# VCISwang/STCD

Measured on AMD Instinct MI355X. Metric: image-pairs/sec (256x256 bf16 SiamUnet_diff train), higher is better.
Workload: dtype bf16; 1 GPU; SiamUnet_diff(3,2) 256x256 full training step (fwd + cross_entropy + bwd + AdamW), 16 pairs/GPU, synthetic LEVIR-CD-shaped pairs resident in HBM; global_batch=16, image=256, parallelism=dp1

## Files before the change

include/stcd_hip.h:

```cpp
#ifndef STCD_HIP_H
#define STCD_HIP_H

#include <stdint.h>

#ifdef __cplusplus
extern "C" {
#endif

#define STCD_ABI_VERSION 2

#define STCD_ARCH_DIFF 0
#define STCD_ARCH_CONC 1
#define STCD_ARCH_SUB 2
#define STCD_ARCH_SNUNET 3
#define STCD_ARCH_SEGCD 4
#define STCD_ARCH_SEGCD_R18 5
#define STCD_ARCH_SEGCD_R34 6
#define STCD_ARCH_SEGCD_R101 7
#define STCD_ARCH_SEGCD_R152 8
#define STCD_ARCH_FCEF 9
#define STCD_ARCH_XCONC 10
#define STCD_ARCH_SNUNET_CONC 11
#define STCD_ARCH_SNUNET_CONC_DS 12
#define STCD_ARCH_UNETSEG 16
// ... 168 lines not shown
int stcd_mask_close(const uint8_t* in, int height, int width, int radius, int mask_value, uint8_t* out, void* hip_stream);

typedef struct stcd_conv_geom {
    int32_t n, hi, wi, ci, ldi;
    int32_t hm, wm, in_stride;
    int32_t ho, wo, out_stride, oy0, ox0;
    int32_t co, ldo;
    int32_t ntaps;
    int8_t dy[9], dx[9];
    int8_t pad_[2];
} stcd_conv_geom;

int stcd_op_conv(int dtype, int impl, const stcd_conv_geom* g, const void* in, const float* w, const float* bias,
                 void* out, void* scratch, int64_t scratch_bytes, void* hip_stream);
enum { STCD_CONV_SMALL = 0, STCD_CONV_RES = 1, STCD_CONV_TILE = 2, STCD_CONV_GEMM = 3, STCD_CONV_HALO = 4, STCD_CONV_DMA = 5 };
typedef struct stcd_conv_fused {
    int32_t kernel;
    int32_t groups;
    void* sum_acc;
    int32_t sum_c0, sum_c;
    float sum_scale1, sum_scale2;
    int32_t use_epi, relu;
    const void* gate;
    const void* res;
    int32_t ldg, ldr;
    float alpha, beta;
    const void* bw_y;
    const float* bw_stat;
    const float* bw_mask;
    void* bw_acc;
    int32_t bw_ldy;
    int32_t blocks, tiles_per_group, blocks_per_group, bn_rep;
    int32_t tile_m;
} stcd_conv_fused;
int stcd_op_conv_fused(const stcd_conv_geom* g, stcd_conv_fused* f, const void* in, const float* w, const float* bias, void* out,
                       void* scratch, int64_t scratch_bytes, void* hip_stream);
int stcd_op_wgrad(int dtype, int impl, const stcd_conv_geom* g, const void* in, const void* dout, float* dw,
                  void* scratch, int64_t scratch_bytes, void* hip_stream);
int64_t stcd_op_scratch_bytes(const stcd_conv_geom* g);

typedef struct stcd_map_geom {
    int32_t n, h, w, c, groups;
} stcd_map_geom;
int64_t stcd_op_ew_scratch_bytes(const stcd_map_geom* g);
int stcd_op_bn_act(int dtype, const stcd_map_geom* g, const void* y, int ldy, const float* gamma, const float* beta,
                   float* running_mean, float* running_var, const float* mask, int relu, int training, void* a, int lda,
                   void* pool, int ldp, float* stat, void* scratch, int64_t scratch_bytes, void* hip_stream);
int stcd_op_bn_act_pair(int dtype, const stcd_map_geom* g, const void* y, int ldy, const float* gamma, const float* beta,
                        float* running_mean, float* running_var, const float* mask, int fuse_mode, void* a, int lda, void* pool,
                        int ldp, void* fused, int ldf, float* stat, void* scratch, int64_t scratch_bytes, void* hip_stream);
int stcd_op_bn_act_bwd(int dtype, const stcd_map_geom* g, const void* da, int ldda, const void* y, int ldy, const float* stat,
                       const float* mask, int relu, void* dy, int lddy, float* dgamma, float* dbeta, void* scratch,
                       int64_t scratch_bytes, void* hip_stream);
int stcd_op_maxpool(int dtype, const stcd_map_geom* g, const void* a, int lda, void* pool, int ldp, void* hip_stream);
int stcd_op_maxpool_bwd(int dtype, const stcd_map_geom* g, const void* a, int lda, const void* dpool, int ldp, void* da, int ldda,
                        int accumulate, void* hip_stream);
int stcd_op_maxpool3(int dtype, const stcd_map_geom* g, const void* a, int lda, void* pool, int ldp, void* idx, void* hip_stream);
int stcd_op_maxpool3_bwd(int dtype, const stcd_map_geom* g, const void* idx, const void* dpool, int ldp, void* da, int ldda, void* hip_stream);
int64_t stcd_op_pairdw_scratch_bytes(const stcd_map_geom* g);
int stcd_op_pairdw(int dtype, const stcd_map_geom* g, const void* a, int lda, const float* w, const float* b, void* out, int ldo,
                   void* hip_stream);
int stcd_op_pairdw_bwd(int dtype, const stcd_map_geom* g, const void* a, int lda, const void* dout, int lddo, const float* w, void* da,
                       int ldda, float* dw, void* scratch, int64_t scratch_bytes, void* hip_stream);
int stcd_op_fuse(int dtype, int mode, const stcd_map_geom* g, const void* a, int lda, void* d, int ldd, void* hip_stream);
int stcd_op_fuse_bwd(int dtype, int mode, const stcd_map_geom* g, const void* a, int lda, const void* dd, int ldd, void* da, int ldda,
                     void* hip_stream);
int stcd_op_rep_pad(int dtype, const stcd_map_geom* g, void* d, int ld, int h0, int w0, void* hip_stream);
int stcd_op_rep_pad_bwd(int dtype, const stcd_map_geom* g, void* dd, int ld, int h0, int w0, void* hip_stream);
int stcd_op_skip_bwd(int dtype, int mode, const stcd_map_geom* g, const void* a, int lda, const void* y, int ldy, const void* dd,
                     int ldd, const void* dpool, int ldp, const float* stat, const float* mask, void* da, int ldda, void* dy,
                     int lddy, float* dgamma, float* dbeta, void* scratch, int64_t scratch_bytes, void* hip_stream);

int64_t stcd_op_cf_scratch_bytes(int64_t rows, int channels, int n, int q_tokens, int kv_tokens);
int stcd_op_cf_im2col(int dtype, const void* x, void* col, int ldc, int n, int h, int w, int c, int k, int stride, int pad, void* hip_stream);
int stcd_op_cf_col2im(int dtype, const void* dcol, int ldc, void* dx, int n, int h, int w, int c, int k, int stride, int pad, int accumulate,
                      void* hip_stream);
int stcd_op_cf_layernorm(int dtype, const void* x, void* y, const float* gamma, const float* beta, float* stats, int64_t rows, int c, float eps,
                         void* hip_stream);
int stcd_op_cf_layernorm_bwd(int dtype, const void* dy, const void* dy2, const void* x, const float* stats, const float* gamma, const void* add,
                             void* dx, float* dgamma, float* dbeta, void* scratch, int64_t rows, int c, void* hip_stream);
int stcd_op_cf_colsum(int dtype, const void* x, int64_t rows, int c, float* out, void* scratch, void* hip_stream);
int stcd_op_cf_attention(int dtype, const void* q, const void* kv, void* out, float* lse, int n, int q_tokens, int kv_tokens, int heads, int d,
                         float p, uint64_t seed, void* hip_stream);
int64_t stcd_op_cf_attention_scratch_bytes(int n, int q_tokens, int kv_tokens, int heads, int d);
int stcd_op_cf_attention_bwd(int dtype, const void* q, const void* kv, const void* out, const void* dout, const float* lse, void* dq, void* dkv,
                             void* scratch, int n, int q_tokens, int kv_tokens, int heads, int d, float p, uint64_t seed, void* hip_stream);
int stcd_op_cf_dwgelu(int dtype, const void* h, void* u, void* a, const float* w, const float* b, int n, int height, int width, int ch, float p,
                      uint64_t seed, void* hip_stream);
int64_t stcd_op_cf_dwgelu_scratch_bytes(int n, int height, int width, int ch);
int stcd_op_cf_dwgelu_bwd(int dtype, const void* h, const void* u, void* da, void* dh, const float* w, float* dw, float* db, void* scratch, int n,
                          int height, int width, int ch, float p, uint64_t seed, void* hip_stream);
int stcd_op_cf_resid_drop(int dtype, const void* x, const void* y, void* out, int n, int64_t rows_per_img, int c, float p, float path_p,
                          uint64_t seed, int backward, void* hip_stream);
int stcd_op_cf_bilinear(int dtype, const void* src, void* dst, int n, int h, int w, int out_h, int out_w, int c, int accumulate, int backward,
                        void* hip_stream);
int stcd_op_cf_elementwise(int dtype, int op, const void* x, const void* y, void* out, int64_t rows, int c, const float* alpha, float alpha_f,
                           float beta_f, float p, uint64_t seed, void* hip_stream);
int stcd_op_cf_prelu_bwd(int dtype, const void* dz, const void* y, void* dy, const float* alpha, float* dalpha, void* scratch, int64_t rows, int c,
                         void* hip_stream);

#ifdef __cplusplus
}
#endif
#endif
```

stcd_amd/_lib.py:

```python
from __future__ import annotations

import ctypes as C
import os

import torch

_HERE = os.path.dirname(os.path.abspath(__file__))
LIB_PATH = os.environ.get("STCD_LIB_PATH") or os.path.join(_HERE, "libstcd_hip.so")

ARCH_DIFF, ARCH_CONC, ARCH_SUB, ARCH_SNUNET, ARCH_SEGCD = 0, 1, 2, 3, 4
ARCH_SEGCD_R18, ARCH_SEGCD_R34, ARCH_SEGCD_R101, ARCH_SEGCD_R152 = 5, 6, 7, 8
ARCH_FCEF = 9
ARCH_XCONC = 10
ARCH_SNUNET_CONC = 11
ARCH_SNUNET_CONC_DS = 12
ARCH_UNETSEG = 16
ARCH_FFCTLCD = 32
ARCH_BASE_RESNET = 48
ARCH_BIT = 52
ARCH_CHANGEFORMER = 64
DTYPE_F32, DTYPE_BF16 = 0, 1
ARCH_IDS = {"diff": ARCH_DIFF, "conc": ARCH_CONC, "sub": ARCH_SUB, "fcef": ARCH_FCEF, "xconc": ARCH_XCONC, "snunet": ARCH_SNUNET, "snunet_conc": ARCH_SNUNET_CONC, "snunet_conc_ds": ARCH_SNUNET_CONC_DS, "segcd": ARCH_SEGCD,
            "segcd_resnet50": ARCH_SEGCD, "segcd_resnet18": ARCH_SEGCD_R18, "segcd_resnet34": ARCH_SEGCD_R34,
            "segcd_resnet101": ARCH_SEGCD_R101, "segcd_resnet152": ARCH_SEGCD_R152,
# ... 85 lines not shown
    "stcd_num_bn": (_i, [_vp]),
    "stcd_bn_info_get": (_i, [_vp, _i, C.POINTER(BnInfo)]),
    "stcd_bn_floats": (_i64, [_vp]),
    "stcd_configure": (_i, [_vp, _i, _i, _i]),
    "stcd_workspace_bytes": (_i64, [_vp]),
    "stcd_num_dropout": (_i, [_vp]),
    "stcd_dropout_info_get": (_i, [_vp, _i, C.POINTER(DropoutInfo)]),
    "stcd_dropout_floats": (_i64, [_vp]),
    "stcd_set_dropout_p": (_i, [_vp, _f]),
    "stcd_forward": (_i, [_vp, _vp, _vp, _vp, _vp, _vp, C.c_uint64, _i, _vp, _vp, _vp]),
    "stcd_backward": (_i, [_vp, _vp, _vp, _vp, _vp, _i, _vp]),
    "stcd_grad_stage_range": (_i, [_vp, _i, C.POINTER(_i64), C.POINTER(_i64)]),
    "stcd_set_weights_tag": (_i, [_vp, C.c_uint64]),
    "stcd_set_debug": (_i, [_vp, _i]),
    "stcd_ws_tensor_count": (_i, [_vp]),
    "stcd_ws_tensor_get": (_i, [_vp, _i, C.POINTER(WsTensor)]),
    "stcd_profile_enable": (_i, [_vp, _i]),
    "stcd_profile_read": (_i, [_vp, _i, C.POINTER(C.c_double), C.POINTER(_i64), C.POINTER(C.c_double), C.POINTER(C.c_double)]),
    "stcd_profile_num_kernels": (_i, [_vp]),
    "stcd_profile_kernel": (_i, [_vp, _i, C.c_char_p, _i, C.POINTER(C.c_double), C.POINTER(_i64), C.POINTER(C.c_double), C.POINTER(C.c_double)]),
    "stcd_loss_scratch_bytes": (_i64, []),
    "stcd_loss_ce": (_i, [_vp, _vp, _i, _i, _i64, _i, _vp, _vp, _vp, _vp]),
    "stcd_loss_bce_dice": (_i, [_vp, _vp, _i64, _i, _vp, _vp, _vp, _vp]),
    "stcd_loss_contrastive": (_i, [_vp, _vp, _vp, _i64, _vp, _vp, _vp, _vp]),
    "stcd_loss_focal": (_i, [_vp, _vp, _i, _i, _i64, _vp, _f, _f, _i, _vp, _vp, _vp, _vp]),
    "stcd_loss_iou_scratch_bytes": (_i64, [_i, _i, _i64]),
    "stcd_loss_iou": (_i, [_vp, _vp, _i, _i, _i64, _vp, _i, _vp, _vp, _vp, _vp]),
    "stcd_confusion_update": (_i, [_vp, _vp, _i, _i, _i64, _vp, _vp]),
    "stcd_adam_step": (_i, [_vp, _vp, _vp, _vp, _i64, _i64, _d, _d, _d, _d, _d, _i, _vp]),
    "stcd_adam_hyper": (_i, [_i64, _d, _d, _d, _d, _d, C.POINTER(_f)]),
    "stcd_adam_step_dev": (_i, [_vp, _vp, _vp, _vp, _i64, _vp, _i, _vp]),
    "stcd_pseudo_pair": (_i, [_vp, _vp, _vp, _vp, _vp, _vp, C.c_uint64, _i, _i, _i, C.POINTER(_f), C.POINTER(_f), _vp, _vp, _vp, _vp, _vp, _vp]),
    "stcd_augment_scratch_bytes": (_i64, [_i, _i, _i]),
    "stcd_augment": (_i, [_vp, _vp, _i, _i, _i, C.POINTER(_f), C.POINTER(_f), _vp, _vp, _i64, _vp]),
    "stcd_scene_gather": (_i, [_vp, _vp, _i, _i, _i, _i, _i, _i, _i, C.POINTER(_f), C.POINTER(_f), _vp, _vp, _vp]),
    "stcd_scene_stitch": (_i, [_vp, _i, _i, _i, _i, _i, _i, _i, _i, _i, _vp, _vp, _vp, _vp]),
    "stcd_scene_finalize": (_i, [_vp, _vp, _i, _i, _i, _f, _vp, _vp, _vp, _vp, _vp]),
    "stcd_scene_gather_d4": (_i, [_vp, _vp, _i, _i, _i, _i, _i, _i, _i, C.POINTER(_f), C.POINTER(_f), _vp, _vp, _i, _vp]),
    "stcd_scene_stitch_d4": (_i, [_vp, _i, _i, _i, _i, _i, _i, _i, _i, _i, _vp, _vp, _vp, _i, _vp]),
    "stcd_scene_gather_one_d4": (_i, [_vp, _i, _i, _i, _i, _i, _i, _i, C.POINTER(_f), C.POINTER(_f), _vp, _i, _vp]),
    "stcd_scene_stitch_heads_d4": (_i, [C.POINTER(_vp), _i, _i, _i, _i, _i, _i, _i, _i, _i, _i, _vp, _vp, _vp, _i, _vp]),
    "stcd_scene_finalize_seg": (_i, [_vp, _vp, _i, _i, _i, _f, _f, _vp, _vp, _vp, _vp, _vp, _vp, _vp, _vp, _vp, _vp]),
    "stcd_selftrain_score": (_i, [C.POINTER(_vp), _i, _i, _i, _i64, _f, _vp, _i, _vp, _vp, _vp, _vp]),
    "stcd_scene_cell_agree": (_i, [C.POINTER(_vp), _i, _i, _i, _i, _i, _i, _vp, _vp, _vp, _vp]),
    "stcd_mask_close": (_i, [_vp, _i, _i, _i, _i, _vp, _vp]),
    "stcd_op_conv": (_i, [_i, _i, C.POINTER(ConvGeom), _vp, _vp, _vp, _vp, _vp, _i64, _vp]),
    "stcd_op_conv_fused": (_i, [C.POINTER(ConvGeom), C.POINTER(ConvFused), _vp, _vp, _vp, _vp, _vp, _i64, _vp]),
    "stcd_op_wgrad": (_i, [_i, _i, C.POINTER(ConvGeom), _vp, _vp, _vp, _vp, _i64, _vp]),
    "stcd_op_scratch_bytes": (_i64, [C.POINTER(ConvGeom)]),
    "stcd_op_ew_scratch_bytes": (_i64, [C.POINTER(MapGeom)]),
    "stcd_op_bn_act": (_i, [_i, C.POINTER(MapGeom), _vp, _i, _vp, _vp, _vp, _vp, _vp, _i, _i, _vp, _i, _vp, _i, _vp, _vp, _i64, _vp]),
    "stcd_op_bn_act_pair": (_i, [_i, C.POINTER(MapGeom), _vp, _i, _vp, _vp, _vp, _vp, _vp, _i, _vp, _i, _vp, _i, _vp, _i, _vp, _vp, _i64, _vp]),
    "stcd_op_bn_act_bwd": (_i, [_i, C.POINTER(MapGeom), _vp, _i, _vp, _i, _vp, _vp, _i, _vp, _i, _vp, _vp, _vp, _i64, _vp]),
    "stcd_op_maxpool": (_i, [_i, C.POINTER(MapGeom), _vp, _i, _vp, _i, _vp]),
    "stcd_op_maxpool_bwd": (_i, [_i, C.POINTER(MapGeom), _vp, _i, _vp, _i, _vp, _i, _i, _vp]),
    "stcd_op_maxpool3": (_i, [_i, C.POINTER(MapGeom), _vp, _i, _vp, _i, _vp, _vp]),
    "stcd_op_maxpool3_bwd": (_i, [_i, C.POINTER(MapGeom), _vp, _vp, _i, _vp, _i, _vp]),
    "stcd_op_pairdw_scratch_bytes": (_i64, [C.POINTER(MapGeom)]),
    "stcd_op_pairdw": (_i, [_i, C.POINTER(MapGeom), _vp, _i, _vp, _vp, _vp, _i, _vp]),
    "stcd_op_pairdw_bwd": (_i, [_i, C.POINTER(MapGeom), _vp, _i, _vp, _i, _vp, _vp, _i, _vp, _vp, _i64, _vp]),
    "stcd_op_fuse": (_i, [_i, _i, C.POINTER(MapGeom), _vp, _i, _vp, _i, _vp]),
    "stcd_op_fuse_bwd": (_i, [_i, _i, C.POINTER(MapGeom), _vp, _i, _vp, _i, _vp, _i, _vp]),
    "stcd_op_rep_pad": (_i, [_i, C.POINTER(MapGeom), _vp, _i, _i, _i, _vp]),
    "stcd_op_rep_pad_bwd": (_i, [_i, C.POINTER(MapGeom), _vp, _i, _i, _i, _vp]),
    "stcd_op_skip_bwd": (_i, [_i, _i, C.POINTER(MapGeom), _vp, _i, _vp, _i, _vp, _i, _vp, _i, _vp, _vp, _vp, _i, _vp, _i, _vp, _vp, _vp, _i64, _vp]),
    "stcd_op_cf_scratch_bytes": (_i64, [_i64, _i, _i, _i, _i]),
    "stcd_op_cf_im2col": (_i, [_i, _vp, _vp, _i, _i, _i, _i, _i, _i, _i, _i, _vp]),
    "stcd_op_cf_col2im": (_i, [_i, _vp, _i, _vp, _i, _i, _i, _i, _i, _i, _i, _i, _vp]),
    "stcd_op_cf_layernorm": (_i, [_i, _vp, _vp, _vp, _vp, _vp, _i64, _i, _f, _vp]),
    "stcd_op_cf_layernorm_bwd": (_i, [_i, _vp, _vp, _vp, _vp, _vp, _vp, _vp, _vp, _vp, _vp, _i64, _i, _vp]),
    "stcd_op_cf_colsum": (_i, [_i, _vp, _i64, _i, _vp, _vp, _vp]),
    "stcd_op_cf_attention": (_i, [_i, _vp, _vp, _vp, _vp, _i, _i, _i, _i, _i, _f, C.c_uint64, _vp]),
    "stcd_op_cf_attention_scratch_bytes": (_i64, [_i, _i, _i, _i, _i]),
    "stcd_op_cf_attention_bwd": (_i, [_i, _vp, _vp, _vp, _vp, _vp, _vp, _vp, _vp, _i, _i, _i, _i, _i, _f, C.c_uint64, _vp]),
    "stcd_op_cf_dwgelu": (_i, [_i, _vp, _vp, _vp, _vp, _vp, _i, _i, _i, _i, _f, C.c_uint64, _vp]),
    "stcd_op_cf_dwgelu_scratch_bytes": (_i64, [_i, _i, _i, _i]),
    "stcd_op_cf_dwgelu_bwd": (_i, [_i, _vp, _vp, _vp, _vp, _vp, _vp, _vp, _vp, _i, _i, _i, _i, _f, C.c_uint64, _vp]),
    "stcd_op_cf_resid_drop": (_i, [_i, _vp, _vp, _vp, _i, _i64, _i, _f, _f, C.c_uint64, _i, _vp]),
    "stcd_op_cf_bilinear": (_i, [_i, _vp, _vp, _i, _i, _i, _i, _i, _i, _i, _i, _vp]),
    "stcd_op_cf_elementwise": (_i, [_i, _i, _vp, _vp, _vp, _i64, _i, _vp, _f, _f, _f, C.c_uint64, _vp]),
    "stcd_op_cf_prelu_bwd": (_i, [_i, _vp, _vp, _vp, _vp, _vp, _vp, _i64, _i, _vp]),
}
EXPORTS = tuple(_PROTOS)

_lib = None


class StcdError(RuntimeError):
    pass


def lib():
    global _lib
    if _lib is None:
        if not os.path.exists(LIB_PATH):
            raise StcdError(
                f"{LIB_PATH} is missing: build it with `python -c 'import __graft_entry__ as g; g.build()'` "
                "or `make -C stcd_amd/csrc`.  The engine has no CPU fallback.")
        l = C.CDLL(LIB_PATH)
        for name, (res, args) in _PROTOS.items():
            fn = getattr(l, name)
            fn.restype, fn.argtypes = res, args
        if l.stcd_abi_version() != 2:
            raise StcdError("libstcd_hip.so ABI version mismatch")
        _lib = l
    return _lib
# ... 6 lines not shown
```

stcd_amd/csrc/common.h:

```cpp
#pragma once
#include <hip/hip_runtime.h>
#include <stdint.h>
#include <stdio.h>
#include <stdlib.h>
#include <string>
#include <string.h>

#include "../../include/stcd_hip.h"

namespace stcd {

typedef __bf16 bf16;

enum DType { F32 = STCD_DTYPE_F32, BF16 = STCD_DTYPE_BF16 };
inline size_t dsize(int dt) { return dt == BF16 ? 2 : 4; }

void set_error(const std::string& msg);

static inline int env_int(const char* name, int dflt) { const char* v = getenv(name); return v ? atoi(v) : dflt; }
static inline bool env_flag(const char* name, bool dflt) { const char* v = getenv(name); return v && v[0] == (dflt ? '0' : '1') ? !dflt : dflt; }

#define STCD_CHECK(cond, msg)                                              \
    do {                                                                   \
        if (!(cond)) {                                                     \
// ... 80 lines not shown
    double y = (double)__frsqrt_rn((float)x);
    y = y * (1.5 - 0.5 * x * y * y);
    return y * (1.5 - 0.5 * x * y * y);
}

__device__ __forceinline__ void bn_fwd_table(float* tab, const long long* __restrict__ facc, const float* __restrict__ gamma,
                                             const float* __restrict__ beta, float* __restrict__ rmean, float* __restrict__ rvar,
                                             float* __restrict__ stat, int C, int groups, int64_t ppg, float momentum, float eps,
                                             bool publish, int cbase = 0, int CS = 0, int g_first = 0) {
    if (CS == 0) CS = C;
    const double inv_n = 1.0 / (double)ppg;
    for (int cl = threadIdx.x; cl < CS; cl += blockDim.x) {
        const int c = cbase + cl;
        if (facc) {
            const float gam = gamma[c], bet = beta[c];
            float rm = (publish && rmean) ? rmean[c] : 0.f, rv = (publish && rvar) ? rvar[c] : 0.f;
            for (int gi = 0; gi < groups; ++gi) {
                int g = gi + g_first;
                if (g >= groups) g -= groups;
                const double s1 = bn_acc_get(facc, groups, C, g, 0, c, BN_FS1), s2 = bn_acc_get(facc, groups, C, g, 1, c, BN_FS2);
                const double mean = s1 * inv_n;
                double var = s2 * inv_n - mean * mean;
                if (var < 0.0) var = 0.0;
                const double invstd = bn_rsqrt(var + (double)eps);
                const float sc = (float)(gam * invstd), sh = (float)(bet - mean * gam * invstd);
                tab[(g * 2 + 0) * CS + cl] = sc;
                tab[(g * 2 + 1) * CS + cl] = sh;
                if (publish) {
                    float* st = stat + (int64_t)g * 4 * C;
                    st[c] = (float)mean; st[C + c] = (float)invstd; st[2 * C + c] = sc; st[3 * C + c] = sh;
                    const double unb = ppg > 1 ? var * ((double)ppg / (double)(ppg - 1)) : var;
                    rm = (float)((1.0 - momentum) * rm + momentum * mean);
                    rv = (float)((1.0 - momentum) * rv + momentum * unb);
                }
            }
            if (publish && rmean) rmean[c] = rm;
            if (publish && rvar) rvar[c] = rv;
        } else if (gamma) {
            const float invstd = 1.f / sqrtf(rvar[c] + eps);
            const float sc = gamma[c] * invstd, sh = beta[c] - rmean[c] * gamma[c] * invstd;
            for (int g = 0; g < groups; ++g) {
                tab[(g * 2 + 0) * CS + cl] = sc;
                tab[(g * 2 + 1) * CS + cl] = sh;
            }
        } else {
            for (int g = 0; g < groups; ++g) {
                tab[(g * 2 + 0) * CS + cl] = stat[(int64_t)g * 4 * C + 2 * C + c];
                tab[(g * 2 + 1) * CS + cl] = stat[(int64_t)g * 4 * C + 3 * C + c];
            }
        }
    }
}

struct XfSrc {
    const long long* facc = nullptr;
    const float* gamma = nullptr;
    const float* beta = nullptr;
    float* rmean = nullptr; float* rvar = nullptr;
    float* stat = nullptr;
    const float* mask = nullptr;
    int C = 0, groups = 1, npg = 0, publish = 0;
    long long ppg = 0;
    float momentum = 0.1f, eps = 1e-5f;
    int on = 0;
};
__device__ __forceinline__ uint4 xf_act8(const uint4 raw, const float (&sc)[8], const float (&sh)[8], const unsigned okm) {
    typedef short s16x2 __attribute__((ext_vector_type(2)));
    const uint32_t w[4] = {raw.x, raw.y, raw.z, raw.w};
    uint32_t o[4];
#pragma unroll
    for (int i = 0; i < 4; ++i) {
        const float lo = fmaf(__uint_as_float(w[i] << 16), sc[2 * i], sh[2 * i]);
        const float hi = fmaf(__uint_as_float(w[i] & 0xffff0000u), sc[2 * i + 1], sh[2 * i + 1]);
        const s16x2 p = __builtin_bit_cast(s16x2, pack_bf16x2(lo, hi));
        o[i] = __builtin_bit_cast(uint32_t, __builtin_elementwise_max(p, s16x2{0, 0})) & okm;
    }
    return make_uint4(o[0], o[1], o[2], o[3]);
}
__device__ __forceinline__ void xf_fold8(const float* __restrict__ tab_sc, const float* __restrict__ tab_sh, const float4 m0, const float4 m1,
                                         float (&sc)[8], float (&sh)[8]) {
    const float mk[8] = {m0.x, m0.y, m0.z, m0.w, m1.x, m1.y, m1.z, m1.w};
#pragma unroll
    for (int j = 0; j < 8; ++j) { sc[j] = tab_sc[j] * mk[j]; sh[j] = tab_sh[j] * mk[j]; }
}


void launch_in_pack(int dt, const float* x1, const float* x2, void* X, int B, int cin, int H, int W, hipStream_t s, int dates = 2);
void launch_gout_pack(int dt, const float* g, void* G, int B, int L, int H, int W, hipStream_t s, long long* bias_acc = nullptr);
struct BiasJob { int64_t acc_off; int64_t out_off; int C, valid; float scale; int pad_; };
void launch_bias_finish(const BiasJob* jobs_dev, int njobs, const char* ws, float* grads, hipStream_t s);

void launch_conv_ref(int dt, const stcd_conv_geom& g, const void* in, const float* w, int kpad, int wld,
                     const float* bias, void* out, bool out_nchw_f32, hipStream_t s);
void launch_wgrad_ref(int dt, const stcd_conv_geom& g, const void* in, const void* dout, float* dw, int kpad, int wld,
                      hipStream_t s);
void launch_wgrad_ref_f64(int dt, const stcd_conv_geom& g, const void* in, const void* dout, double* dw, int kpad, int wld,
                          hipStream_t s);

struct ConvMfmaPlan {
    int CiB = 0, nchunks = 0, KS = 0, modeB = 0, NT = 0, NTtot = 0;
    int64_t wf_elems = 0;
    bool ok = false;
};
ConvMfmaPlan conv_mfma_plan(const stcd_conv_geom& g);
void launch_pack_frag(const stcd_conv_geom& g, const ConvMfmaPlan& p, const float* w, int kpad, int wld, void* dst,
                      hipStream_t s);
// ... 49 lines not shown
struct ConvHaloPlan {
    int NH = 0;
    int nslices = 0, P = 0, blocks = 0, lds_bytes = 0;
    bool ok = false;
};
ConvHaloPlan conv_halo_plan(const stcd_conv_geom& g, const ConvMfmaPlan& p);
int launch_conv_halo(const stcd_conv_geom& g, const ConvMfmaPlan& p, const ConvHaloPlan& hp, const void* in, const void* wf,
                     const float* bias, void* out, hipStream_t s, const ConvEpi* epi = nullptr);

struct ConvDmaPlan {
    int tiles_m = 0, tiles_n = 0, blocks = 0, lds_bytes = 0;
    bool ok = false;
};
ConvDmaPlan conv_dma_plan(const stcd_conv_geom& g, const ConvMfmaPlan& p);
int launch_conv_dma(const stcd_conv_geom& g, const ConvMfmaPlan& p, const ConvDmaPlan& dp, const void* in, const void* wf,
                    const float* bias, void* out, hipStream_t s, const ConvEpi* epi = nullptr);

bool conv_small_ok(const stcd_conv_geom& g, const ConvMfmaPlan& p);
int conv_small_blocks(const stcd_conv_geom& g, int groups);
int launch_conv_small(const stcd_conv_geom& g, const void* in, const void* wf_modeB, const float* bias, void* out,
                      bool out_nchw_f32, int groups, long long* stat_acc, int cpad, hipStream_t s, const XfSrc* xf = nullptr,
                      const BwdSum* bs = nullptr);
bool conv_small_call_ok(const stcd_conv_geom& g, int groups, const XfSrc* xf);
bool conv_small_bwdsum_ok(const stcd_conv_geom& g);
struct WgradMfmaPlan {
    int WCI = 1, NTW = 1, gx = 1, gy = 1, gz = 1;
    int64_t slab_floats = 0;
    int wi_valid = 0;
    int gemm = 0;
    int dma = 0;
    bool ok = false;
};
WgradMfmaPlan wgrad_mfma_plan(const stcd_conv_geom& g, int kpad, int wld, bool allow_wide = false, int force_co64 = -1);
int launch_wgrad_mfma(const stcd_conv_geom& g, const WgradMfmaPlan& p, const void* in, const void* dout, float* slab,
                      int kpad, int wld, hipStream_t s);
struct WgradJob {
    stcd_conv_geom g;
    int64_t in_off, dout_off, slab_off;
    int kpad, wld;
    int dymin, dxmin, HH, HWp;
    int tiles_x, tiles_y, ntiles;
    int xrow_bytes;
    int x_bytes, y_bytes;
    int co_valid;
    unsigned in_bytes, dout_bytes;
    int gx, gy, gz;
    int start;
    int lds_bytes;
    int wi_valid;
    int dma_L, dma_nk;
    int pad_;
    int64_t xf_stat_off, xf_mask_off;
    int xf_C, xf_groups, xf_npg, pad2_;
};
WgradMfmaPlan wgrad_gemm_plan(const stcd_conv_geom& g, int kpad, int wld);
WgradJob wgrad_gemm_make_job(const stcd_conv_geom& g, const WgradMfmaPlan& p, int64_t in_off, int64_t dout_off, int64_t slab_off,
                             int kpad, int wld);
int launch_wgrad_gemm_group(int W, const WgradJob* jobs_dev, int njobs, int total_blocks, const char* base, hipStream_t s);
WgradMfmaPlan wgrad_dma_plan(const stcd_conv_geom& g, int kpad, int wld);
void wgrad_dma_set_split(WgradMfmaPlan& p, const stcd_conv_geom& g, int S, int kpad, int wld);
WgradJob wgrad_dma_make_job(const stcd_conv_geom& g, const WgradMfmaPlan& p, int64_t in_off, int64_t dout_off, int64_t slab_off,
                            int kpad, int wld);
int launch_wgrad_dma_group(const WgradJob* jobs_dev, int njobs, int total_blocks, const char* base, hipStream_t s);
WgradJob wgrad_make_job(const stcd_conv_geom& g, const WgradMfmaPlan& p, int64_t in_off, int64_t dout_off, int64_t slab_off,
                        int kpad, int wld);
void wgrad_job_set_xf(WgradJob& a, int64_t stat_off, int64_t mask_off, int C, int groups, int npg);
int wgrad_variant_slots(int WCI, int NTW, bool t9, int lds_bytes);
int launch_wgrad_group(int WCI, int NTW, bool t9, const WgradJob* jobs_dev, int njobs, int total_blocks, int lds_bytes,
                       const char* base, hipStream_t s, bool xf = false);
struct PackSpec;
struct ReduceJob {
    int64_t start, count;
    int64_t slab_off;
    int64_t out_off;
    int64_t slab_stride;
    int gx, ntaps, K, N, kpad, wld;
    int ks, kn_major;
    int8_t ky[9], kx[9];
    int8_t tiled, parts, pad_[4];
};
void launch_reduce_jobs(const ReduceJob* jobs_dev, int njobs, int64_t total, const char* ws, float* grads, hipStream_t s);
void launch_reduce_dw(const float* slab, int gx, const stcd_conv_geom& g, int K, int N, int kpad, int wld,
                      const PackSpec* ps, float* out, hipStream_t s);

struct PackSpec {
    int ks;
    int kn_major;
    int K, N, wld;
    int kpad;
    int ntaps;
    int8_t ky[9], kx[9];
};
void launch_pack_w(const PackSpec& ps, const float* src, float* dst, hipStream_t s);
void launch_unpack_dw(const PackSpec& ps, const double* dwe, float* gsrc, hipStream_t s);

struct PackJob {
    int64_t start, count;
    int64_t src_off;
    int64_t dst_off;
    int kind;
    PackSpec ps;
    int Ci, Co, CiB, nchunks, KS, NTtot, modeB;
    int aux;
};
void launch_pack_jobs(const PackJob* jobs_dev, int njobs, int64_t total, const float* params, char* ws, hipStream_t s);

int bn_stats_chunks(int64_t pixels_per_group, int C);
void launch_bn_stats(int dt, const void* Y, int ld, int C, int groups, int64_t pixels_per_group, long long* acc, hipStream_t s);
void launch_bn_eval_prepare(int C, int groups, const float* gamma, const float* beta, const float* running_mean,
                            const float* running_var, float* stat, float eps, hipStream_t s);
constexpr int MAX_VIEWS = 6;
struct SliceViews {
    int n = 0;
    void* p[MAX_VIEWS]; int ld[MAX_VIEWS]; int64_t goff[MAX_VIEWS]; int gmask[MAX_VIEWS];
};
struct BnActArgs {
    const void* Y; int ldy;
    void* A; int lda; int64_t a_group_off;
    void* P; int ldp;
    float* stat;
    const float* mask;
    int C, groups, npg, H, W;
// ... 234 lines not shown
```

stcd_amd/csrc/engine.hip:

```cpp
#include <algorithm>
#include <climits>
#include <cstdint>
#include <array>
#include <cstring>
#include <memory>
#include <vector>

#include "common.h"

namespace stcd {

static thread_local std::string g_err;
void set_error(const std::string& msg) { g_err = msg; }

enum ConvKind { K_CONV3 = 0, K_CONVT3_S1 = 1, K_UPCONV = 2, K_CONV1 = 3, K_CONVT2 = 4, K_CONV3_S2 = 5, K_CONV1_S2 = 6, K_STEM7 = 7 };

struct TRef { int64_t off = -1; int ld = 0; };
struct GRef { int64_t off = -1; int ld = 0; int64_t goff = 0; };

static inline int round8(int c) { return (c + 7) & ~7; }

struct ConvW {
    std::string name;
    int kind = 0, cin = 0, cout = 0;
    int kin_p = 0, nout_p = 0;
    int64_t w_off = 0, b_off = 0;
    PackSpec fwd{}, dgrad{};
    int64_t wpk_fwd = -1, wpk_dgrad = -1, dwe = -1;
    int64_t dwe_floats = 0;
};
struct BnP {
    std::string name;
    int C = 0, calls = 1;
    int64_t g_off = 0, b_off = 0;
    int64_t run_off = 0;
};
struct DropP { std::string name; int rows = 0, C = 0; int64_t off = 0; };

struct ConvOp {
    stcd_conv_geom g{};
    int conv = -1; bool dgrad = false;
    int tap0 = 0;
    int kreal = 0, nreal = 0;
    ConvMfmaPlan plan; int64_t wf = -1;
    bool small = false;
    ConvResPlan res; int res_groups = 1;
    ConvGemmPlan gemm;
    ConvDmaPlan dma;
    ConvHaloPlan halo;
    ConvTilePlan tile;
};
struct WgradOp {
    stcd_conv_geom g{};
    int conv = -1, tap0 = 0, kreal = 0, nreal = 0;
    WgradMfmaPlan plan;
    int64_t slab = -1;
    int stage = 0;
    int64_t in_off = -1, dout_off = -1;
    bool grouped = false;
    int group = -1;
    int64_t xf_stat_off = -1, xf_mask_off = -1; int xf_C = 0, xf_groups = 1, xf_npg = 1;
    bool own_taps = false;
    int8_t oky[9] = {0}, okx[9] = {0};
};
struct WgradGroup {
    int WCI = 1, NTW = 1; bool t9 = false;
    bool xf = false;
    int gemm = 0;
    int dma = 0;
    std::vector<WgradJob> jobs;
    int total_blocks = 0, lds_bytes = 0;
    int64_t table_off = -1;
    double flops = 0.0, bytes = 0.0;
    int seen = 0; bool launched = false;
};

struct Cbrd {
    ConvOp fwd, dgr; WgradOp wg;
    int conv = -1, bn = -1, drop = -1;
    int N = 0, H = 0, W = 0, groups = 1, npg = 0;
    TRef in; int K = 0;
    TRef Y; GRef A; TRef P; TRef dPool; bool pool = false;
    GRef dA; TRef dY; TRef dIn; bool has_dIn = false;
    int64_t stat = -1;
    int64_t facc = -1, bacc = -1;
    const Cbrd* dgr_bwd = nullptr;
    bool bwd_sums_fused = false;
    int64_t dgr_sum_acc = -1; int dgr_sum_c0 = 0, dgr_sum_C = 0;
    TRef fuse_dst;
    bool virt = false; const Cbrd* xsrc = nullptr;
};
struct XConc {
    int level = 0, C = 0;
    int64_t w_off = 0, b_off = 0;
    int bn1 = -1;
    TRef G, dG, R, dR;
    int64_t stat1 = -1, facc1 = -1, bacc1 = -1, part = -1;
    Cbrd res;
};
struct UpConv {
    int conv = -1, level = 0;
    int N = 0, h = 0, w = 0, Ho = 0, Wo = 0, C = 0;
    TRef in, out, dOut, dIn;
    ConvOp fwd[4], dgr; WgradOp wg[4];
    int64_t bias_acc = -1; bool bias_fused = false;
};

enum ProfClass { PC_CONV = 0, PC_WGRAD = 1, PC_BN_STATS = 2, PC_BN_ACT = 3, PC_BN_BWD_REDUCE = 4, PC_BN_BWD_APPLY = 5,
                 PC_POOL_FUSE = 6, PC_PACK = 7, PC_COUNT = 8 };
struct ProfRec { hipEvent_t a, b; int klass; int name_id; double flops, bytes; };
struct Prof {
    bool on = false;
    std::vector<ProfRec> recs;
    std::vector<hipEvent_t> pool;
    std::vector<std::string> names;
    size_t used = 0;
    int intern(const std::string& n) {
        for (size_t i = 0; i < names.size(); ++i)
            if (names[i] == n) return (int)i;
        names.push_back(n);
        return (int)names.size() - 1;
    }
    hipEvent_t get() {
        if (used == pool.size()) { hipEvent_t ev; (void)hipEventCreate(&ev); pool.push_back(ev); }
        return pool[used++];
    }
    ~Prof() { for (auto ev : pool) (void)hipEventDestroy(ev); }
};

struct ViewRef { int64_t off = 0; int ld = 0; int64_t goff = 0; int gmask = 1; };
struct GLayer {
    std::string name;
    int conv = -1, bn = -1, kind = K_CONV3;
    int N = 0, Hi = 0, Wi = 0, Ho = 0, Wo = 0, K = 0, C = 0, groups = 2, npg = 0;
    bool relu = true;
    TRef in, Y, A, res;
    TRef dA, dIn, dRes;
    bool has_dIn = true;
    std::vector<ViewRef> extra_dst;
    std::vector<ViewRef> grad_src;
    bool grad_base = true;
    ConvOp fwd, dgr[4]; int ndgr = 0; WgradOp wg[8]; int nwg = 0;
    int64_t stat = -1, coef = -1, facc = -1, bacc = -1;
// ... 42 lines not shown
    int64_t sn_pool = -1, sn_argm = -1, sn_att = -1, sn_hid = -1, sn_sums = -1, sn_dpool = -1, sn_part = -1;
    int64_t sn_dout_begin = -1, sn_dout_end = -1;
    ConvOp sn_final_fwd, sn_final_dgr; WgradOp sn_final_wg;
    int64_t snc_w[5] = {0, 0, 0, 0, 0}, snc_b[5] = {0, 0, 0, 0, 0}, snc_scratch = -1;
    std::vector<GLayer> g_layers;
    std::vector<GStep> g_fwd;
    int g_stem = -1, g_head_conv = -1;
    int debug_flags = 0;
    std::vector<stcd_ws_tensor> ws_tensors;
    std::vector<std::array<int, 4>> g_blocks;
    int seg_x = 4, seg_layers[4] = {3, 4, 6, 3};
    int seg_dates = 2;
    bool seg_ffc = false;
    TRef g_pool_idc;
    std::vector<std::array<int, 2>> g_dec;
    TRef gP0, gdP0, gX3, gdX3, gFuseTmp;
    int64_t g_pool_idx = -1;
    int64_t g_stem_part = -1;
    int64_t g_raw3 = -1, g_draw3 = -1;
    ConvOp g_head_fwd, g_head_dgr; WgradOp g_head_wg;
    bool bres = false; int seg_nstage = 4;
    int g_head_c = 16;
    int g_cls = -1, g_pred_conv = -1;
    ConvOp g_pred_fwd, g_pred_dgr; WgradOp g_pred_wg;
    int64_t g_pred_bias_acc = -1;
    struct BitPlan {
        bool on = false; int L = 1, dh = 64;
        int64_t pos_off = 0, wa_off = 0, enc_off = 0, dec_off = 0;
        int64_t tok_in = -1, tok_out = -1, dtok_out = -1, dtok_in = -1, stat = -1, AP = -1, dAP = -1, xs = -1, dG = -1, dec_part = -1,
                dmh = -1, dm = -1, enc_part = -1, tok_part = -1;
        TRef dec_din;
    } bit;
    int arch = 0, in_ch = 3, label = 2, dt = F32;
    int64_t min_bn_count = 0;
    float drop_p = 0.2f;
    std::vector<stcd_tensor_info> params;
    int64_t param_floats = 0, enc_param_end = 0;
    std::vector<ConvW> convs;
    std::vector<BnP> bns;
    int64_t bn_floats = 0;
    bool configured = false, fwd_training = false;
    int B = 0, H = 0, W = 0;
    std::vector<DropP> drops;
    int64_t drop_floats = 0;
    int64_t ws_bytes = 0;
    std::vector<Cbrd> enc, dec;
    std::vector<UpConv> ups;
    int final_conv = -1;
    ConvOp final_fwd, final_dgr; WgradOp final_wg;
    const Cbrd* final_dgr_bwd = nullptr;
    const Cbrd* final_xsrc = nullptr;
    int use_virt = 0;
    int fc_virt_layers = 0;
    std::vector<ConvOp*> conv_ops;
    int64_t slab = -1, slab_floats = 0;
    std::vector<WgradOp*> wgrad_ops;
    std::vector<WgradGroup> wgroups[2];
    std::vector<ReduceJob> rjobs[2];
    int64_t rjobs_total[2] = {0, 0}, rjobs_off[2] = {-1, -1};
    std::vector<PackJob> jobs[2];
    int64_t jobs_total[2] = {0, 0}, jobs_off[2] = {-1, -1};
    const void* jobs_uploaded_ws = nullptr;
    uint64_t weights_tag = 0, packed_tag = 0;
    const void* packed_ws = nullptr; const void* packed_params = nullptr; int packed_level = -1;
    TRef X0, G, finalIn, dFinalIn;
    int Hs[5] = {0}, Ws[5] = {0};
    TRef D[4], dD[4], P[4], dP[4];
    int64_t zero_begin = -1, zero_end = -1;
    int64_t final_bias_acc = -1;
    std::vector<BiasJob> bias_jobs; int64_t bias_jobs_off = -1;
    int64_t masks = -1, dwe_begin = -1, dwe_end = -1, scratch8 = -1;
    int use_mfma = 1, use_small = 1, use_wgroup = 1, use_res = 1, use_skip_fused = 1, use_act_fuse = 1, use_gemm = 1, use_skip_recompute = 1, use_bwdsum = 1, use_bwdsum_res = 0, use_tile = 1, use_halo = 0;
    int wg_side_on = 1;
    static constexpr int WG_SIDE_DIV = 4;
    static constexpr int WGROUP_ROUNDS = 1, WGROUP_MIN_TILES = 8;
    bool wg_early = false; hipStream_t wg_cur_side = nullptr;
    hipStream_t wg_side = nullptr; hipEvent_t wg_fork = nullptr, wg_join = nullptr; int wg_side_dev = -1;
};

}

using namespace stcd;
struct stcd_engine : stcd_engine_impl {};

namespace stcd {

static const int ENC_STAGE_CONVS[4] = {2, 2, 3, 3};
static const int ENC_C[4] = {16, 32, 64, 128};
static const int SKIP_IDX[4] = {1, 3, 6, 9};

static void add_param(stcd_engine& e, const std::string& name, std::initializer_list<int64_t> shape, int64_t* off_out) {
    stcd_tensor_info ti;
    memset(&ti, 0, sizeof(ti));
    snprintf(ti.name, sizeof(ti.name), "%s", name.c_str());
    ti.ndim = (int)shape.size();
    int64_t n = 1;
    int i = 0;
    for (auto s : shape) { ti.shape[i++] = s; n *= s; }
    ti.numel = n;
    ti.offset = e.param_floats;
    *off_out = ti.offset;
    e.param_floats += (n + 3) & ~(int64_t)3;
    e.params.push_back(ti);
}

static void make_specs(ConvW& c, bool need_dgrad) {
// ... 248 lines not shown
    op.small = conv_small_ok(op.g, op.plan);
    if (e.use_res && !op.small) op.res = conv_res_plan(op.g, op.plan, groups);
    pick_gemm_or_res(e, op, op.g, groups);
    if (with_tile) pick_tile(e, op, op.g, groups);
}
static bool conv_on_ref(bool mfma, const ConvOp& op) { return !(mfma && op.plan.ok && op.wf >= 0); }
struct Binder {
    stcd_engine& e; Bump& ws;
    bool with_tile = false;
    void conv(ConvOp& op, const stcd_conv_geom& g, int conv, bool dgrad, int tap0, int kreal, int nreal, int groups = 1) const {
        op = ConvOp();
        op.g = g; op.conv = conv; op.dgrad = dgrad; op.tap0 = tap0; op.kreal = kreal; op.nreal = nreal; op.res_groups = groups;
        if (e.dt == BF16) plan_conv(e, op, groups, with_tile);
        if (op.plan.ok) op.wf = ws.take(op.plan.wf_elems * 2);
        e.conv_ops.push_back(&op);
    }
    void stem(ConvOp& op, const stcd_conv_geom& g, int conv, int groups) const {
        op = ConvOp();
        op.g = g; op.conv = conv; op.kreal = e.convs[conv].cin; op.nreal = g.co; op.res_groups = groups;
        op.plan = conv_mfma_plan(g);
        if (g.ldi == 8 && g.co % 64 == 0) op.gemm = conv_gemm_plan(g, op.plan, groups);
        op.gemm.pix_chunks = 1;
        if (!op.gemm.ok) return;
        op.wf = ws.take(op.plan.wf_elems * 2);
        e.conv_ops.push_back(&op);
    }
    void wgrad(WgradOp& op, const stcd_conv_geom& g, int conv, int64_t in_off, int64_t dout_off, int stage = 0, int tap0 = 0,
               int wi_valid = 0, const int8_t* own_ky = nullptr, const int8_t* own_kx = nullptr) const {
        const ConvW& cv = e.convs[conv];
        op = WgradOp();
        op.g = g; op.conv = conv; op.tap0 = tap0; op.kreal = cv.cin; op.nreal = cv.cout;
        op.in_off = in_off; op.dout_off = dout_off; op.stage = stage;
        op.own_taps = own_ky != nullptr;
        for (int t = 0; t < g.ntaps && op.own_taps; ++t) { op.oky[t] = own_ky[t]; op.okx[t] = own_kx[t]; }
        if (e.dt == BF16) { op.plan = pick_wgrad_plan(e, g, cv.fwd.kpad, cv.fwd.wld); op.plan.wi_valid = wi_valid; }
        e.wgrad_ops.push_back(&op);
    }
};
static void take_ref_images(stcd_engine& e, Bump& ws, bool with_dwe = true) {
    for (auto& c : e.convs) {
        c.wpk_fwd = ws.take((int64_t)c.fwd.ntaps * c.fwd.kpad * c.fwd.wld * 4);
        if (c.dgrad.ntaps) c.wpk_dgrad = ws.take((int64_t)c.dgrad.ntaps * c.dgrad.kpad * c.dgrad.wld * 4);
    }
    e.dwe_begin = ws.cur;
    for (auto& c : e.convs) {
        c.dwe_floats = (int64_t)c.fwd.ntaps * c.fwd.kpad * c.fwd.wld;
        c.dwe = with_dwe ? ws.take(c.dwe_floats * 8) : -1;
    }
    e.dwe_end = ws.cur;
}

static bool same_group(const WgradGroup& G, const WgradOp& op) {
    const bool t9 = !op.plan.dma && op.g.ntaps == 9;
    return G.gemm == op.plan.gemm && G.dma == op.plan.dma && G.WCI == op.plan.WCI && G.NTW == op.plan.NTW && G.t9 == t9 && G.xf == (op.xf_C > 0);
}

static bool cf_side_on() { static const bool on = env_flag("STCD_CF_SIDE", true); return on; }

static void build_pack_jobs(stcd_engine& e, Bump& ws) {
    for (int st = 0; st < 2; ++st) { e.rjobs[st].clear(); e.rjobs_total[st] = 0; }
    for (int st = 0; st < 2; ++st) e.wgroups[st].clear();
    if (e.dt == BF16 && e.use_mfma) {
        if (e.use_wgroup) {
            for (WgradOp* op : e.wgrad_ops) {
                if (!op->plan.ok) continue;
                const bool t9 = !op->plan.dma && op->g.ntaps == 9;
                std::vector<WgradGroup>& gs = e.wgroups[op->stage];
                size_t gi = 0;
                while (gi < gs.size() && !same_group(gs[gi], *op)) ++gi;
                if (gi == gs.size()) { WgradGroup g; g.WCI = op->plan.WCI; g.NTW = op->plan.NTW; g.t9 = t9; g.gemm = op->plan.gemm; g.dma = op->plan.dma; g.xf = op->xf_C > 0; gs.push_back(g); }
                op->grouped = true;
            }
            for (int st = 0; st < 2; ++st)
                for (WgradGroup& G : e.wgroups[st]) {
                    if (G.gemm) { G.lds_bytes = 2 * 2 * G.gemm * (64 * 64 + 8 * 32); continue; }
                    if (G.dma) {
                        G.lds_bytes = 128 * 1024;
                        std::vector<WgradOp*> dops;
                        for (WgradOp* op : e.wgrad_ops)
                            if (op->grouped && op->stage == st && op->plan.dma) dops.push_back(op);
                        auto blocks_at = [&](int64_t kt) {
                            int64_t b = 0;
                            for (WgradOp* op : dops) {
                                const int64_t M = (int64_t)op->g.n * op->g.hi * op->g.wi;
                                b += ((M + kt * 64 - 1) / (kt * 64)) * op->plan.gy * op->plan.gz;
                            }
                            return b;
                        };
                        int64_t lo = 1, hi = 1;
                        const int dma_blocks = e.wg_side_on && cf_side_on() ? 192 : 256;
                        while (blocks_at(hi) > dma_blocks) hi *= 2;
                        while (lo < hi) { const int64_t mid = (lo + hi) / 2; if (blocks_at(mid) <= dma_blocks) hi = mid; else lo = mid + 1; }
                        for (WgradOp* op : dops) {
                            const ConvW& cv = e.convs[op->conv];
                            const int64_t M = (int64_t)op->g.n * op->g.hi * op->g.wi;
                            int64_t S = (M + lo * 64 - 1) / (lo * 64);
                            const int64_t slab_bytes = (int64_t)op->g.ntaps * cv.fwd.kpad * cv.fwd.wld * 4;
                            S = std::min<int64_t>(S, std::max<int64_t>(1, ((int64_t)64 << 20) / slab_bytes));
                            wgrad_dma_set_split(op->plan, op->g, (int)S, cv.fwd.kpad, cv.fwd.wld);
                        }
                        continue;
                    }
                    std::vector<WgradOp*> ops;
                    int64_t W = 0;
                    for (WgradOp* op : e.wgrad_ops)
                        if (op->grouped && op->stage == st && same_group(G, *op)) {
                            ops.push_back(op);
                            const int64_t ntiles = (int64_t)op->g.n * ((op->g.wm + 15) / 16) * ((op->g.hm + 7) / 8);
                            W += ntiles * op->plan.gy * op->plan.gz;
                        }
                    for (WgradOp* op : ops) {
                        const ConvW& cv = e.convs[op->conv];
                        WgradJob j = wgrad_make_job(op->g, op->plan, 0, 0, 0, cv.fwd.kpad, cv.fwd.wld);
                        if (op->xf_C > 0) wgrad_job_set_xf(j, op->xf_stat_off, op->xf_mask_off, op->xf_C, op->xf_groups, op->xf_npg);
                        G.lds_bytes = std::max(G.lds_bytes, j.lds_bytes);
                    }
                    int slots = wgrad_variant_slots(G.WCI, G.NTW, G.t9, G.lds_bytes);
                    if (st == 0 && e.wg_side_on && fc_family(e)) slots = std::max(64, slots / stcd_engine_impl::WG_SIDE_DIV);
                    const int64_t rounds = stcd_engine_impl::WGROUP_ROUNDS;
                    const int64_t tpb = std::max<int64_t>(stcd_engine_impl::WGROUP_MIN_TILES, (W + rounds * slots - 1) / (rounds * slots));
                    for (WgradOp* op : ops) {
                        const ConvW& cv = e.convs[op->conv];
                        const int64_t ntiles = (int64_t)op->g.n * ((op->g.wm + 15) / 16) * ((op->g.hm + 7) / 8);
                        const int64_t slab_bytes = (int64_t)op->g.ntaps * cv.fwd.kpad * cv.fwd.wld * 4;
                        int64_t gx = std::max<int64_t>(1, (ntiles + tpb - 1) / tpb);
                        gx = std::min<int64_t>(gx, std::max<int64_t>(1, ((int64_t)32 << 20) / slab_bytes));
                        op->plan.gx = (int)gx;
                        op->plan.slab_floats = gx * op->g.ntaps * cv.fwd.kpad * cv.fwd.wld;
                    }
                }
        }
        int64_t cur[2] = {0, 0};
        for (WgradOp* op : e.wgrad_ops) {
            if (!op->plan.ok) continue;
            const ConvW& cv = e.convs[op->conv];
            op->slab = ws.take(op->plan.slab_floats * 4);
            if (op->grouped) {
                for (WgradGroup& G : e.wgroups[op->stage])
                    if (same_group(G, *op)) {
                        op->group = (int)(&G - e.wgroups[op->stage].data());
                        WgradJob j = op->plan.dma ? wgrad_dma_make_job(op->g, op->plan, op->in_off, op->dout_off, op->slab, cv.fwd.kpad, cv.fwd.wld)
                                   : op->plan.gemm ? wgrad_gemm_make_job(op->g, op->plan, op->in_off, op->dout_off, op->slab, cv.fwd.kpad, cv.fwd.wld)
                                                   : wgrad_make_job(op->g, op->plan, op->in_off, op->dout_off, op->slab, cv.fwd.kpad, cv.fwd.wld);
                        if (op->xf_C > 0 && !op->plan.dma && !op->plan.gemm) wgrad_job_set_xf(j, op->xf_stat_off, op->xf_mask_off, op->xf_C, op->xf_groups, op->xf_npg);
                        j.start = G.total_blocks;
                        G.total_blocks += j.gx * j.gy * j.gz;
                        G.jobs.push_back(j);
                        double fl, by;
                        conv_work(e, op->g, op->kreal, op->nreal, &fl, &by);
                        G.flops += fl; G.bytes += by;
                    }
            }
            ReduceJob j{};
            j.slab_off = op->slab; j.out_off = cv.w_off;
            j.slab_stride = (int64_t)op->g.ntaps * cv.fwd.kpad * cv.fwd.wld;
            j.gx = op->plan.gx; j.ntaps = op->g.ntaps; j.K = cv.cin; j.N = cv.cout; j.kpad = cv.fwd.kpad; j.wld = cv.fwd.wld;
            j.ks = cv.fwd.ks; j.kn_major = cv.fwd.kn_major;
            for (int t = 0; t < op->g.ntaps; ++t) {
                j.ky[t] = op->own_taps ? op->oky[t] : cv.fwd.ky[op->tap0 + t];
                j.kx[t] = op->own_taps ? op->okx[t] : cv.fwd.kx[op->tap0 + t];
            }
            j.tiled = (int64_t)j.ntaps * j.K * j.N >= 512 * 1024;
            if (!j.tiled) {
                const int64_t outs = (int64_t)j.ntaps * j.K * j.N;
                int parts = 1;
                while (parts < 64 && parts * 32 < j.gx) parts *= 2;
                j.parts = (int8_t)parts;
                const int64_t OUTS = 256 / parts;
                j.count = ((outs + OUTS - 1) / OUTS) * 256;
            } else {
                const int TK = j.ntaps == 1 ? 32 : 16;
                const int64_t ntiles = (int64_t)((j.N + 31) / 32) * ((j.K + TK - 1) / TK);
                j.parts = 1;
                j.count = ntiles * 256;
            }
            j.start = cur[op->stage];
            cur[op->stage] += (j.count + 255) & ~(int64_t)255;
            e.rjobs[op->stage].push_back(j);
        }
        for (int st = 0; st < 2; ++st) {
            e.rjobs_total[st] = cur[st];
            e.rjobs_off[st] = ws.take((int64_t)e.rjobs[st].size() * sizeof(ReduceJob) + 16);
            for (WgradGroup& G : e.wgroups[st]) G.table_off = ws.take((int64_t)G.jobs.size() * sizeof(WgradJob) + 16);
        }
    }
    for (int with_dgrad = 0; with_dgrad < 2; ++with_dgrad) {
        std::vector<PackJob>& jobs = e.jobs[with_dgrad];
        jobs.clear();
        int64_t cur = 0;
        auto push = [&](PackJob j) { j.start = cur; cur += (j.count + 255) & ~(int64_t)255; jobs.push_back(j); };
        const bool mfma = e.dt == BF16 && e.use_mfma;
        if (!mfma) {
            for (auto& cv : e.convs)
                for (int d = 0; d <= with_dgrad; ++d) {
                    const PackSpec& ps = d ? cv.dgrad : cv.fwd;
                    if (!ps.ntaps) continue;
                    PackJob j{};
                    j.kind = 0; j.ps = ps; j.src_off = cv.w_off; j.dst_off = d ? cv.wpk_dgrad : cv.wpk_fwd;
                    j.count = (int64_t)ps.ntaps * ps.kpad * ps.wld;
                    push(j);
                }
        } else {
            for (const ConvOp* op : e.conv_ops) {
                if (op->dgrad && !with_dgrad) continue;
                const ConvW& cv = e.convs[op->conv];
                const PackSpec& full = op->dgrad ? cv.dgrad : cv.fwd;
                PackJob j{};
                j.ps = full;
                j.ps.ntaps = op->g.ntaps;
                for (int t = 0; t < op->g.ntaps; ++t) { j.ps.ky[t] = full.ky[op->tap0 + t]; j.ps.kx[t] = full.kx[op->tap0 + t]; }
                j.src_off = cv.w_off;
                if (cv.kind == K_STEM7) {
                    j.kind = 2; j.dst_off = op->wf; j.count = op->plan.wf_elems;
                    j.Co = cv.cout; j.NTtot = op->plan.NTtot; j.aux = cv.cin;
                    push(j);
                    continue;
                }
                if (!conv_on_ref(true, *op)) {
                    j.kind = 1; j.dst_off = op->wf;
                    j.count = op->plan.modeB ? op->plan.wf_elems : op->plan.wf_elems / op->g.ntaps;
                    j.Ci = op->g.ci; j.Co = op->g.co; j.CiB = op->plan.CiB; j.nchunks = op->plan.nchunks; j.KS = op->plan.KS;
                    j.NTtot = op->plan.NTtot; j.modeB = op->plan.modeB;
                } else {
                    j.kind = 0;
                    j.dst_off = (op->dgrad ? cv.wpk_dgrad : cv.wpk_fwd) + (int64_t)op->tap0 * full.kpad * full.wld * 4;
                    j.count = (int64_t)j.ps.ntaps * full.kpad * full.wld;
                }
                push(j);
            }
        }
        e.jobs_total[with_dgrad] = cur;
        e.jobs_off[with_dgrad] = ws.take((int64_t)jobs.size() * sizeof(PackJob) + 16);
    }
}

// ... 154 lines not shown
    for (auto& L : e.dec) bind_cbrd(L);
    for (auto& X : e.xc) bind_cbrd(X.res);
    for (auto& U : e.ups) {
        const ConvW& cv = e.convs[U.conv];
        for (int ph = 0; ph < 4; ++ph) {
            int tap0;
            stcd_conv_geom g = geom_up_phase(U, ph >> 1, ph & 1, U.in.ld, U.out.ld, &tap0);
            bind.conv(U.fwd[ph], g, U.conv, false, tap0, U.C, U.C);
            bind.wgrad(U.wg[ph], g, U.conv, U.in.off, U.dOut.off, wg_stage(U.conv), tap0);
        }
        stcd_conv_geom gd;
        memset(&gd, 0, sizeof(gd));
        gd.n = U.N; gd.hi = U.Ho; gd.wi = U.Wo; gd.ci = cv.dgrad.kpad; gd.ldi = U.dOut.ld;
        gd.hm = U.h; gd.wm = U.w; gd.in_stride = 2;
        gd.ho = U.h; gd.wo = U.w; gd.out_stride = 1;
        gd.co = U.C; gd.ldo = U.dIn.ld;
        gd.ntaps = 9;
        for (int t = 0; t < 9; ++t) { gd.dy[t] = (int8_t)(t / 3 - 1); gd.dx[t] = (int8_t)(t % 3 - 1); }
        bind.conv(U.dgr, gd, U.conv, true, 0, U.C, U.C);
    }
    {
        const ConvW& cv = e.convs[e.final_conv];
        bind.conv(e.final_fwd, geom3(B, H, W, cv.kin_p, e.finalIn.ld, e.label, e.label), e.final_conv, false, 0, cv.cin, e.label);
        bind.wgrad(e.final_wg, geom3(B, H, W, cv.kin_p, e.finalIn.ld, e.label, 8), e.final_conv, e.finalIn.off, e.G.off, wg_stage(e.final_conv));
        bind.conv(e.final_dgr, geom3(B, H, W, cv.dgrad.kpad, 8, cv.cin, e.dFinalIn.ld), e.final_conv, true, 0, e.label, cv.cin);
    }
    e.slab = ws.take(e.slab_floats * 4);

    for (auto& L : e.enc) { L.dgr_bwd = nullptr; L.bwd_sums_fused = false; }
    for (auto& L : e.dec) { L.dgr_bwd = nullptr; L.bwd_sums_fused = false; }
    e.final_dgr_bwd = nullptr;
    if (e.use_bwdsum && e.dt == BF16 && e.use_mfma && e.use_small && !e.use_virt) {
        const int res_too = e.use_bwdsum_res;
        auto dest_ok = [&](const Cbrd& P, const ConvOp& dgr, int64_t dIn_off, int dIn_ld, int N) {
            const bool kern = (dgr.small && conv_small_bwdsum_ok(dgr.g)) ||
                              (res_too && !dgr.small && !dgr.gemm.ok && e.use_res && dgr.res.ok && dgr.res_groups == P.groups &&
                               conv_res_bwdsum_ok(dgr.g, dgr.res));
            return !P.pool && P.fuse_dst.off < 0 && !P.virt && kern && dgr.wf >= 0 && dIn_off == P.dA.off && dIn_ld == P.dA.ld &&
                   e.convs[P.conv].cout == dgr.g.co && P.N == N && N % P.groups == 0 &&
                   (P.groups == 1 || P.dA.goff == (int64_t)P.npg * P.H * P.W * P.dA.ld);
        };
        auto scan = [&](std::vector<Cbrd>& v) {
            for (size_t i = 1; i < v.size(); ++i) {
                Cbrd& N = v[i]; Cbrd& P = v[i - 1];
                if (N.has_dIn && N.dgr_sum_acc < 0 && dest_ok(P, N.dgr, N.dIn.off, N.dIn.ld, N.N)) { N.dgr_bwd = &P; P.bwd_sums_fused = true; }
            }
        };
        scan(e.enc); scan(e.dec);
        if (!e.dec.empty() && dest_ok(e.dec.back(), e.final_dgr, e.dFinalIn.off, e.dFinalIn.ld, e.dec.back().N)) {
            e.final_dgr_bwd = &e.dec.back(); e.dec.back().bwd_sums_fused = true;
        }
    }

    e.final_xsrc = nullptr; e.fc_virt_layers = 0;
    for (auto& L : e.enc) { L.virt = false; L.xsrc = nullptr; }
    for (auto& L : e.dec) { L.virt = false; L.xsrc = nullptr; }
    if (e.use_virt && e.dt == BF16 && e.use_mfma && e.use_wgroup && !fc_cross(e)) {
        auto fwd_ok = [&](const ConvOp& op, bool nchw) {
            if (op.wf < 0 || (op.gemm.ok && !nchw)) return false;
            if (op.small && e.use_small) return true;
            return op.res.ok && !nchw && !op.res.single_halo;
        };
        auto wg_ok = [&](const WgradOp& op) { return op.plan.ok && !op.plan.gemm && !op.plan.dma && op.plan.WCI < 4 && op.plan.NTW < 4; };
        auto link = [&](Cbrd& P, ConvOp& cf, WgradOp& cw, bool nchw) {
            if (P.pool || P.fuse_dst.off >= 0) return false;
            if (!fwd_ok(cf, nchw) || !wg_ok(cw)) return false;
            P.virt = true; ++e.fc_virt_layers;
            cw.in_off = P.Y.off;
            cw.xf_stat_off = P.stat;
            cw.xf_mask_off = (P.drop >= 0) ? e.masks + e.drops[P.drop].off * 4 : -1;
            cw.xf_C = e.convs[P.conv].cout; cw.xf_groups = P.groups; cw.xf_npg = P.npg;
            return true;
        };
        for (size_t i = 0; i + 1 < e.enc.size(); ++i) {
            Cbrd& P = e.enc[i]; Cbrd& Cn = e.enc[i + 1];
            if (Cn.in.off != P.A.off) continue;
            if (link(P, Cn.fwd, Cn.wg, false)) { Cn.xsrc = &P; Cn.in.off = P.Y.off; Cn.in.ld = P.Y.ld; }
        }
        for (size_t i = 0; i < e.dec.size(); ++i) {
            Cbrd& P = e.dec[i];
            if (i + 1 < e.dec.size() && e.dec[i + 1].in.off == P.A.off) {
                Cbrd& Cn = e.dec[i + 1];
                if (link(P, Cn.fwd, Cn.wg, false)) { Cn.xsrc = &P; Cn.in.off = P.Y.off; Cn.in.ld = P.Y.ld; }
            } else if (e.finalIn.off == P.A.off) {
                if (link(P, e.final_fwd, e.final_wg, true)) { e.final_xsrc = &P; e.finalIn.off = P.Y.off; e.finalIn.ld = P.Y.ld; }
            }
        }
    }

    e.bias_jobs.clear();
    {
        size_t di = 0;
        for (int k = 0; k < 4; ++k) {
            UpConv& U = e.ups[k];
            Cbrd& L = e.dec[di];
            int nb = 0;
            for (int j = 0; j < DEC[k].n; ++j) nb += DEC[k].cout[j] >= 0;
            di += nb;
            U.bias_fused = false;
            const bool even = 2 * U.h == U.Ho && 2 * U.w == U.Wo;
            if (e.dt == BF16 && e.use_mfma && nb > 0 && L.has_dIn && L.dIn.off == U.dOut.off && L.dgr.res.ok && L.dgr.wf >= 0 && even) {
                U.bias_fused = true;
                L.dgr_sum_acc = U.bias_acc; L.dgr_sum_c0 = 0; L.dgr_sum_C = U.C;
            }
            if (e.dt == BF16) {
                BiasJob jb{}; jb.acc_off = U.bias_acc; jb.out_off = e.convs[U.conv].b_off; jb.C = U.C; jb.valid = U.C; jb.scale = BN_BS;
                e.bias_jobs.push_back(jb);
            }
        }
        BiasJob jb{}; jb.acc_off = e.final_bias_acc; jb.out_off = e.convs[e.final_conv].b_off; jb.C = 8; jb.valid = e.label; jb.scale = BN_BS;
        e.bias_jobs.push_back(jb);
        e.bias_jobs_off = ws.take((int64_t)e.bias_jobs.size() * sizeof(BiasJob) + 16);
    }

    e.ws_tensors.clear();
    auto rec_layer = [&](const Cbrd& L) {
        const ConvW& cv = e.convs[L.conv];
        auto rec = [&](const char* sfx, int64_t off, int ld, int n, int ch) {
            if (off < 0) return;
            stcd_ws_tensor r;
            memset(&r, 0, sizeof(r));
            snprintf(r.name, sizeof(r.name), "%s.%s", cv.name.c_str(), sfx);
            r.offset_bytes = off; r.n = n; r.h = L.H; r.w = L.W; r.c = ch; r.ld = ld; r.dtype = e.dt;
            e.ws_tensors.push_back(r);
        };
        rec(L.xsrc ? "in.virt" : "in", L.in.off, L.in.ld, L.N, L.K);
        rec("Y", L.Y.off, L.Y.ld, L.N, cv.cout);
        for (int g = 0; g < L.groups && !L.virt && !skip_recomputed(e, L); ++g) {
            char sfx[8];
            snprintf(sfx, sizeof(sfx), "A.g%d", g);
            rec(sfx, L.A.off + g * L.A.goff * T, L.A.ld, L.npg, cv.cout);
        }
        rec("dY", L.dY.off, L.dY.ld, L.N, cv.cout);
    };
    for (const Cbrd& L : e.enc) rec_layer(L);
    for (const Cbrd& L : e.dec) rec_layer(L);
    for (const XConc& X : e.xc) {
        auto rec = [&](const char* sfx, const TRef& t) {
            stcd_ws_tensor r;
            memset(&r, 0, sizeof(r));
            snprintf(r.name, sizeof(r.name), "cross_conc%d.diff.0.%s", X.level + 1, sfx);
            r.offset_bytes = t.off; r.n = X.res.N; r.h = X.res.H; r.w = X.res.W; r.c = X.C; r.ld = t.ld; r.dtype = e.dt;
            e.ws_tensors.push_back(r);
        };
        rec("Y", X.G); rec("A.g0", X.R); rec("dY", X.dG);
        rec_layer(X.res);
    }

    build_pack_jobs(e, ws);
    e.jobs_uploaded_ws = nullptr;
    e.ws_bytes = ws.cur;
    return 0;
}

struct Ctx {
    stcd_engine& e;
    char* ws;
    const float* params;
    float* grads;
    hipStream_t s;
    template <typename P = void> P* at(int64_t off) const { return (P*)(ws + off); }
};

struct ProfScope {
    Prof& p; hipStream_t s; bool on; hipEvent_t b;
    ProfScope(const Ctx& c, int klass, double flops, double bytes, const char* kernel = nullptr);
    ~ProfScope() { if (on) (void)hipEventRecord(b, s); }
};

ProfScope::ProfScope(const Ctx& c, int klass, double flops, double bytes, const char* kernel)
    : p(c.e.prof), s(c.s), on(c.e.prof.on), b(nullptr) {
    if (!on) return;
    static const char* DEF[PC_COUNT] = {"k_conv", "k_wgrad", "k_bn_reduce<T, 0>", "k_bn_act", "k_bn_reduce<T, 1>", "k_bn_bwd_apply",
                                        "k_pool_bwd|k_fuse|k_slice", "k_pack_jobs|k_reduce_dw"};
    ProfRec r;
    r.a = p.get(); r.b = p.get(); r.klass = klass; r.flops = flops; r.bytes = bytes;
    r.name_id = p.intern(kernel ? kernel : DEF[klass]);
    b = r.b;
    p.recs.push_back(r);
    (void)hipEventRecord(r.a, s);
}

static void conv_work(const stcd_engine& e, const stcd_conv_geom& g, int kreal, int nreal, double* flops, double* bytes) {
    double pos = (double)g.n * g.hm * g.wm;
    *flops = 2.0 * pos * g.ntaps * kreal * nreal;
    double in_px = g.in_stride == 1 ? pos : (double)g.n * (2.0 * g.hm) * (2.0 * g.wm);
// ... 147 lines not shown
    char kname[64];
    snprintf(kname, sizeof(kname), "k_conv_mfma_x4<%d>", p[0].NT);
    ProfScope prof(c, PC_CONV, fl, by, kname);
    if (launch_conv_mfma_x4(g, p, in, wf, bias, out, c.s) != 0) set_error(std::string("internal: ") + kname + " rejected the launch it was chosen for");
    return true;
}

static void wgroup_member_ready(const Ctx& c, const WgradOp& op);
static void exec_wgrad(const Ctx& c, const WgradOp& op, const void* in, const void* dout) {
    const ConvW& cv = c.e.convs[op.conv];
    PackSpec sub = cv.fwd;
    sub.ntaps = op.g.ntaps;
    for (int t = 0; t < op.g.ntaps; ++t) {
        sub.ky[t] = op.own_taps ? op.oky[t] : cv.fwd.ky[op.tap0 + t];
        sub.kx[t] = op.own_taps ? op.okx[t] : cv.fwd.kx[op.tap0 + t];
    }
    double fl, by;
    conv_work(c.e, op.g, op.kreal, op.nreal, &fl, &by);
    if (mfma_on(c.e) && op.plan.ok && op.grouped) {
        if (c.e.wg_early) wgroup_member_ready(c, op);
        return;
    }
    if (mfma_on(c.e) && op.plan.ok) {
        int rc;
        {
            char kname[64];
            snprintf(kname, sizeof(kname), "k_wgrad_mfma<%d, %d>", op.plan.WCI, op.plan.NTW);
            ProfScope prof(c, PC_WGRAD, fl, by, kname);
            rc = launch_wgrad_mfma(op.g, op.plan, in, dout, c.at<float>(op.slab), sub.kpad, sub.wld, c.s);
        }
        if (rc == 0) return;
    }
    if (op.own_taps) { set_error("internal: no reference fallback for a launch with its own tap table"); return; }
    double* dwe = c.at<double>(cv.dwe) + (int64_t)op.tap0 * sub.kpad * sub.wld;
    if (mfma_on(c.e))
        (void)hipMemsetAsync(dwe, 0, (size_t)sub.ntaps * sub.kpad * sub.wld * 8, c.s);
    {
        ProfScope prof(c, PC_WGRAD, fl, by, "k_wgrad_ref");
        launch_wgrad_ref_f64(c.e.dt, op.g, in, dout, dwe, sub.kpad, sub.wld, c.s);
    }
    launch_unpack_dw(sub, dwe, c.grads + cv.w_off, c.s);
}

static int pack_all_weights(const Ctx& c, bool with_dgrad) {
    stcd_engine& e = c.e;
    if (e.jobs_uploaded_ws != (const void*)c.ws) {
        for (int k = 0; k < 2; ++k) {
            if (!e.jobs[k].empty())
                STCD_HIP(hipMemcpyAsync(c.at(e.jobs_off[k]), e.jobs[k].data(), e.jobs[k].size() * sizeof(PackJob),
                                        hipMemcpyHostToDevice, c.s));
            if (!e.rjobs[k].empty())
                STCD_HIP(hipMemcpyAsync(c.at(e.rjobs_off[k]), e.rjobs[k].data(), e.rjobs[k].size() * sizeof(ReduceJob),
                                        hipMemcpyHostToDevice, c.s));
            for (WgradGroup& G : e.wgroups[k])
                STCD_HIP(hipMemcpyAsync(c.at(G.table_off), G.jobs.data(), G.jobs.size() * sizeof(WgradJob), hipMemcpyHostToDevice, c.s));
        }
        if (!e.bias_jobs.empty())
            STCD_HIP(hipMemcpyAsync(c.at(e.bias_jobs_off), e.bias_jobs.data(), e.bias_jobs.size() * sizeof(BiasJob), hipMemcpyHostToDevice, c.s));
        e.jobs_uploaded_ws = c.ws;
    }
    const int k = with_dgrad ? 1 : 0;
    if (k == 0 && e.weights_tag != 0 && e.weights_tag == e.packed_tag && e.packed_ws == (const void*)c.ws && e.packed_params == (const void*)c.params)
        return 0;
    ProfScope prof(c, PC_PACK, 0.0, 0.0);
    launch_pack_jobs(c.at<PackJob>(e.jobs_off[k]), (int)e.jobs[k].size(), e.jobs_total[k], c.params, c.ws, c.s);
    e.packed_tag = k == 0 ? e.weights_tag : 0; e.packed_ws = c.ws; e.packed_params = c.params; e.packed_level = k;
    return 0;
}

static void launch_wgroup(const Ctx& c, WgradGroup& G) {
    {
        char kname[64];
        if (G.dma) snprintf(kname, sizeof(kname), "k_wgrad_dma");
        else if (G.gemm) snprintf(kname, sizeof(kname), "k_wgrad_gemm<%d>", G.gemm);
        else snprintf(kname, sizeof(kname), "k_wgrad_group<%d, %d, %s>", G.WCI, G.NTW, G.t9 ? "true" : "false");
        ProfScope prof(c, PC_WGRAD, G.flops, G.bytes, kname);
        G.launched = true;
        if (G.dma) {
            launch_wgrad_dma_group(c.at<WgradJob>(G.table_off), (int)G.jobs.size(), G.total_blocks, c.ws, c.s);
            return;
        }
        if (G.gemm) {
            launch_wgrad_gemm_group(G.gemm, c.at<WgradJob>(G.table_off), (int)G.jobs.size(), G.total_blocks, c.ws, c.s);
            return;
        }
        if (launch_wgrad_group(G.WCI, G.NTW, G.t9, c.at<WgradJob>(G.table_off), (int)G.jobs.size(), G.total_blocks, G.lds_bytes,
                               c.ws, c.s, G.xf) != 0)
            set_error("grouped weight-gradient launch exceeds the LDS budget");
    }
}

static void wgroup_member_ready(const Ctx& c, const WgradOp& op) {
    stcd_engine& e = c.e;
    if (op.group < 0 || op.group >= (int)e.wgroups[op.stage].size()) return;
    WgradGroup& G = e.wgroups[op.stage][op.group];
    if (++G.seen < (int)G.jobs.size() || G.launched) return;
    if (e.wg_cur_side) {
        if (hipEventRecord(e.wg_fork, c.s) != hipSuccess || hipStreamWaitEvent(e.wg_cur_side, e.wg_fork, 0) != hipSuccess) { set_error("side-stream fork failed"); return; }
        Ctx cs{e, c.ws, c.params, c.grads, e.wg_cur_side};
        launch_wgroup(cs, G);
    } else {
        launch_wgroup(c, G);
    }
}

static void reduce_stage(const Ctx& c, int stage) {
    stcd_engine& e = c.e;
    for (WgradGroup& G : e.wgroups[stage]) {
        if (!G.launched) launch_wgroup(c, G);
        G.launched = false; G.seen = 0;
    }
    if (e.rjobs[stage].empty()) return;
    ProfScope prof(c, PC_PACK, 0.0, 0.0, "k_reduce_jobs");
    launch_reduce_jobs(c.at<ReduceJob>(e.rjobs_off[stage]), (int)e.rjobs[stage].size(), e.rjobs_total[stage], c.ws, c.grads, c.s);
}

static XfSrc xf_source(const Ctx& c, const Cbrd& P, float* bn_running, bool training) {
    stcd_engine& e = c.e;
    const BnP& bn = e.bns[P.bn];
    XfSrc x;
    x.C = e.convs[P.conv].cout; x.groups = P.groups; x.npg = P.npg; x.ppg = (long long)P.npg * P.H * P.W;
    x.facc = training ? c.at<long long>(P.facc) : nullptr;
    x.gamma = c.params + bn.g_off; x.beta = c.params + bn.b_off;
    x.rmean = bn_running + bn.run_off; x.rvar = bn_running + bn.run_off + x.C;
    x.stat = c.at<float>(P.stat);
    x.mask = (training && e.drop_p > 0.f && P.drop >= 0) ? c.at<float>(e.masks) + e.drops[P.drop].off : nullptr;
    x.publish = training ? 1 : 0;
    x.on = 1;
    return x;
}

static void cbrd_forward(const Ctx& c, const Cbrd& L, float* bn_running, bool training) {
    stcd_engine& e = c.e;
    const ConvW& cv = e.convs[L.conv];
    const BnP& bn = e.bns[L.bn];
    const int C = cv.cout;
    int fused_chunks = 0;
    StatReq sr; sr.acc = training ? c.at<long long>(L.facc) : nullptr; sr.groups = L.groups; sr.C = C;
    XfSrc xf;
    if (L.xsrc) xf = xf_source(c, *L.xsrc, bn_running, training);
    exec_conv(c, L.fwd, c.at(L.in.off), c.params + cv.b_off, c.at(L.Y.off), false, &sr, &fused_chunks, nullptr, nullptr, L.xsrc ? &xf : nullptr);
    const int64_t ppg = (int64_t)L.npg * L.H * L.W;
    const double act_bytes = (double)L.N * L.H * L.W * C * (double)dsize(e.dt);
    float* stat = c.at<float>(L.stat);
    if (training) {
        if (!fused_chunks) {
            ProfScope ps(c, PC_BN_STATS, 0.0, act_bytes);
            launch_bn_stats(e.dt, c.at(L.Y.off), L.Y.ld, C, L.groups, ppg, c.at<long long>(L.facc), c.s);
        }
    }
    if (L.virt) return;
    BnActArgs a;
    a.Y = c.at(L.Y.off); a.ldy = L.Y.ld;
    a.A = skip_recomputed(e, L) ? nullptr : c.at(L.A.off); a.lda = L.A.ld; a.a_group_off = L.A.goff;
    a.P = L.pool ? c.at(L.P.off) : nullptr; a.ldp = L.P.ld;
    a.stat = stat;
    a.mask = (training && e.drop_p > 0.f && L.drop >= 0) ? c.at<float>(e.masks) + e.drops[L.drop].off : nullptr;
    a.C = C; a.groups = L.groups; a.npg = L.npg; a.H = L.H; a.W = L.W; a.relu = 1;
    a.facc = training ? c.at<long long>(L.facc) : nullptr;
    a.gamma = c.params + bn.g_off; a.beta = c.params + bn.b_off;
    a.running_mean = bn_running + bn.run_off; a.running_var = bn_running + bn.run_off + C;
    if (L.fuse_dst.off >= 0 && e.use_act_fuse && L.groups == 2) {
        ProfScope ps(c, PC_BN_ACT, 0.0, act_bytes * (a.A ? 2.75 : 1.75), "k_bn_act_pair");
        launch_bn_act_pair(e.dt, a, c.at(L.fuse_dst.off), L.fuse_dst.ld, e.arch == STCD_ARCH_DIFF ? 0 : 1, c.s);
        return;
    }
    ProfScope ps(c, PC_BN_ACT, 0.0, act_bytes * (L.pool ? 2.25 : 2.0));
    launch_bn_act(e.dt, a, c.s);
}

static BwdSum bwd_sum_of(const Ctx& c, const Cbrd& P) {
    stcd_engine& e = c.e;
    BwdSum b;
    b.Y = c.at(P.Y.off); b.ldy = P.Y.ld; b.stat = c.at<float>(P.stat);
    b.mask = (e.drop_p > 0.f && P.drop >= 0) ? c.at<float>(e.masks) + e.drops[P.drop].off : nullptr;
    b.acc = c.at<long long>(P.bacc); b.groups = P.groups;
    return b;
}

static void cbrd_backward(const Ctx& c, const Cbrd& L, int skip_chunks = 0) {
    stcd_engine& e = c.e;
    const ConvW& cv = e.convs[L.conv];
    const BnP& bn = e.bns[L.bn];
    const int C = cv.cout;
    const int64_t HW = (int64_t)L.H * L.W, ppg = (int64_t)L.npg * HW;
    const float* stat = c.at<float>(L.stat);
    const float* mask = (e.drop_p > 0.f && L.drop >= 0) ? c.at<float>(e.masks) + e.drops[L.drop].off : nullptr;
    long long* bacc = c.at<long long>(L.bacc);
    const double act_bytes = (double)L.N * HW * C * (double)dsize(e.dt);
    (void)ppg;
    if (!skip_chunks && !L.bwd_sums_fused) {
        ProfScope ps(c, PC_BN_BWD_REDUCE, 0.0, 2.0 * act_bytes);
        launch_bn_bwd_reduce(e.dt, c.at(L.dA.off), L.dA.ld, L.dA.goff, c.at(L.Y.off), L.Y.ld, stat, mask, C, L.groups, L.npg, HW, 1,
                             bacc, c.s);
    }
    {
        ProfScope ps(c, PC_BN_BWD_APPLY, 0.0, 3.0 * act_bytes);
        launch_bn_bwd_apply(e.dt, c.at(L.dA.off), L.dA.ld, L.dA.goff, c.at(L.dY.off), L.dY.ld, c.at(L.Y.off), L.Y.ld, stat, bacc,
                            c.grads + bn.g_off, c.grads + bn.b_off, mask, C, L.groups, L.npg, HW, 1, c.s);
    }
    exec_wgrad(c, L.wg, c.at(L.in.off), c.at(L.dY.off));
    if (L.has_dIn) {
        StatReq sr;
        if (L.dgr_sum_acc >= 0) { sr.acc = c.at<long long>(L.dgr_sum_acc); sr.groups = 1; sr.c0 = L.dgr_sum_c0; sr.C = L.dgr_sum_C; sr.s1 = sr.s2 = BN_BS; }
        BwdSum bs;
        if (L.dgr_bwd) bs = bwd_sum_of(c, *L.dgr_bwd);
        exec_conv(c, L.dgr, c.at(L.dY.off), nullptr, c.at(L.dIn.off), false, L.dgr_sum_acc >= 0 ? &sr : nullptr, nullptr, nullptr, nullptr, nullptr,
                  L.dgr_bwd ? &bs : nullptr);
    }
}

static void upconv_forward(const Ctx& c, const UpConv& U) {
    stcd_engine& e = c.e;
    const ConvW& cv = e.convs[U.conv];
    if (!exec_conv_x4(c, U.fwd, c.at(U.in.off), c.params + cv.b_off, c.at(U.out.off)))
        for (int ph = 0; ph < 4; ++ph) exec_conv(c, U.fwd[ph], c.at(U.in.off), c.params + cv.b_off, c.at(U.out.off), false);
    launch_rep_pad(e.dt, c.at(U.out.off), U.out.ld, U.N, U.Ho, U.Wo, 2 * U.h, 2 * U.w, U.C, c.s);
}

static void upconv_backward(const Ctx& c, const UpConv& U) {
    stcd_engine& e = c.e;
    const ConvW& cv = e.convs[U.conv];
    launch_rep_pad_bwd(e.dt, c.at(U.dOut.off), U.dOut.ld, U.N, U.Ho, U.Wo, 2 * U.h, 2 * U.w, U.C, c.s);
    if (U.bias_fused && mfma_on(e)) {
    } else if (2 * U.h == U.Ho && 2 * U.w == U.Wo) {
        launch_bias_grad(e.dt, c.at(U.dOut.off), U.dOut.ld, (int64_t)U.N * U.Ho * U.Wo, U.C, c.grads + cv.b_off, c.s,
                         e.dt == BF16 ? c.at<long long>(U.bias_acc) : nullptr);
    } else {
        const int64_t T = (int64_t)dsize(e.dt);
        for (int n = 0; n < U.N; ++n)
            for (int y = 0; y < 2 * U.h; ++y)
                launch_bias_grad(e.dt, c.at<char>(U.dOut.off) + ((int64_t)(n * U.Ho + y) * U.Wo) * U.dOut.ld * T, U.dOut.ld,
                                 2 * U.w, U.C, c.grads + cv.b_off, c.s, e.dt == BF16 ? c.at<long long>(U.bias_acc) : nullptr);
    }
    for (int ph = 0; ph < 4; ++ph) exec_wgrad(c, U.wg[ph], c.at(U.in.off), c.at(U.dOut.off));
    exec_conv(c, U.dgr, c.at(U.dOut.off), nullptr, c.at(U.dIn.off), false);
}

static void xconc_forward(const Ctx& c, const XConc& X, const Cbrd& skip, float* bn_running, bool training) {
    stcd_engine& e = c.e;
    const BnP& bn = e.bns[X.bn1];
    const int C = X.C, B = X.res.N, h = X.res.H, w = X.res.W;
    {
        ProfScope ps(c, PC_POOL_FUSE, 0.0, 3.0 * B * h * w * C * (double)dsize(e.dt), "k_pairdw_fwd");
        launch_pairdw_fwd(e.dt, c.at(skip.A.off), skip.A.ld, skip.A.goff, c.at(X.G.off), X.G.ld, c.params + X.w_off, c.params + X.b_off, B, h, w, C, c.s);
    }
    if (training) launch_bn_stats(e.dt, c.at(X.G.off), X.G.ld, C, 1, (int64_t)B * h * w, c.at<long long>(X.facc1), c.s);
    BnActArgs a;
    a.Y = c.at(X.G.off); a.ldy = X.G.ld;
    a.A = c.at(X.R.off); a.lda = X.R.ld; a.a_group_off = 0;
    a.P = nullptr; a.ldp = 0;
    a.stat = c.at<float>(X.stat1);
    a.mask = nullptr;
    a.C = C; a.groups = 1; a.npg = B; a.H = h; a.W = w; a.relu = 1;
    a.facc = training ? c.at<long long>(X.facc1) : nullptr;
    a.gamma = c.params + bn.g_off; a.beta = c.params + bn.b_off;
    a.running_mean = bn_running + bn.run_off; a.running_var = bn_running + bn.run_off + C;
    launch_bn_act(e.dt, a, c.s);
    cbrd_forward(c, X.res, bn_running, training);
}
static void xconc_backward(const Ctx& c, const XConc& X, const Cbrd& skip) {
    stcd_engine& e = c.e;
    const BnP& bn = e.bns[X.bn1];
    const int C = X.C, B = X.res.N, h = X.res.H, w = X.res.W;
    const int64_t HW = (int64_t)h * w;
    cbrd_backward(c, X.res);
    launch_bn_bwd_reduce(e.dt, c.at(X.dR.off), X.dR.ld, 0, c.at(X.G.off), X.G.ld, c.at<float>(X.stat1), nullptr, C, 1, B, HW, 1,
                         c.at<long long>(X.bacc1), c.s);
    launch_bn_bwd_apply(e.dt, c.at(X.dR.off), X.dR.ld, 0, c.at(X.dG.off), X.dG.ld, c.at(X.G.off), X.G.ld, c.at<float>(X.stat1),
                        c.at<long long>(X.bacc1), c.grads + bn.g_off, c.grads + bn.b_off, nullptr, C, 1, B, HW, 1, c.s);
    ProfScope ps(c, PC_POOL_FUSE, 0.0, 6.0 * B * h * w * C * (double)dsize(e.dt), "k_pairdw_bwd");
    launch_pairdw_bwd_data(e.dt, c.at(X.dG.off), X.dG.ld, c.at(skip.dA.off), skip.dA.ld, skip.dA.goff, c.params + X.w_off, B, h, w, C, c.s);
    launch_pairdw_bwd_filter(e.dt, c.at(skip.A.off), skip.A.ld, skip.A.goff, c.at(X.dG.off), X.dG.ld, c.grads + X.w_off, c.at<float>(X.part),
                             B, h, w, C, c.s);
}

static int forward_fcsiam(stcd_engine& e, const float* x1, const float* x2, const float* params, float* bn_running,
                          const float* masks, uint64_t seed, int training, float* logits, void* workspace, hipStream_t s) {
    Ctx c{e, (char*)workspace, params, nullptr, s};
    const int B = e.B, dt = e.dt;
    const int64_t T = (int64_t)dsize(dt);
    if (training && e.drop_p > 0.f) {
        if (masks) STCD_HIP(hipMemcpyAsync(c.at(e.masks), masks, e.drop_floats * 4, hipMemcpyDeviceToDevice, s));
        else launch_dropout_gen(c.at<float>(e.masks), e.drop_floats, seed, e.drop_p, s);
    } else if (training && e.fc_virt_layers > 0) {
        launch_dropout_gen(c.at<float>(e.masks), e.drop_floats, seed, 0.f, s);
    }
    if (pack_all_weights(c, training != 0)) return 1;
    if (training) STCD_HIP(hipMemsetAsync(c.at(e.zero_begin), 0, e.zero_end - e.zero_begin, s));
    launch_in_pack(dt, x1, x2, c.at(e.X0.off), B, e.in_ch, e.H, e.W, s, e.arch == STCD_ARCH_FCEF ? 0 : 2);
    for (auto& L : e.enc) cbrd_forward(c, L, bn_running, training != 0);
    size_t di = 0;
    for (int k = 0; k < 4; ++k) {
        const UpConv& U = e.ups[k];
        const int s_ = U.level, C = ENC_C[s_];
        upconv_forward(c, U);
        const Cbrd& skip = e.enc[SKIP_IDX[s_]];
        if (fc_cross(e)) xconc_forward(c, e.xc[s_], skip, bn_running, training != 0);
        else if (!fc_concat_skips(e) && !(e.use_act_fuse && skip.fuse_dst.off >= 0)) {
            ProfScope ps(c, PC_POOL_FUSE, 0.0, 3.0 * B * e.Hs[s_] * e.Ws[s_] * C * (double)T);
            launch_fuse(dt, e.arch == STCD_ARCH_DIFF ? 0 : 1, c.at(skip.A.off), skip.A.ld, skip.A.goff,
                        c.at<char>(e.D[s_].off) + C * T, e.D[s_].ld, B, (int64_t)e.Hs[s_] * e.Ws[s_], C, s);
        }
        for (int j = 0; j < DEC[k].n; ++j) {
            if (DEC[k].cout[j] < 0) break;
            cbrd_forward(c, e.dec[di++], bn_running, training != 0);
        }
    }
    {
        XfSrc xf;
        if (e.final_xsrc) xf = xf_source(c, *e.final_xsrc, bn_running, training != 0);
        exec_conv(c, e.final_fwd, c.at(e.finalIn.off), params + e.convs[e.final_conv].b_off, logits, true, nullptr, nullptr, nullptr, nullptr,
                  e.final_xsrc ? &xf : nullptr);
    }
    STCD_HIP(hipGetLastError());
    return 0;
}

static hipStream_t wgrad_side_stream(stcd_engine& e, hipStream_t s) {
    if (!e.wg_side_on || !e.use_wgroup || !mfma_on(e)) return nullptr;
    if (e.prof.on) return nullptr;
    hipStreamCaptureStatus cap = hipStreamCaptureStatusNone;
    if (hipStreamIsCapturing(s, &cap) != hipSuccess) { (void)hipGetLastError(); return nullptr; }
    if (cap != hipStreamCaptureStatusNone) return nullptr;
    int dev = 0;
    if (hipGetDevice(&dev) != hipSuccess) { (void)hipGetLastError(); return nullptr; }
    if (e.wg_side && e.wg_side_dev == dev) return e.wg_side;
    if (e.wg_side) return nullptr;
    int prio_lo = 0, prio_hi = 0;
    (void)hipDeviceGetStreamPriorityRange(&prio_lo, &prio_hi);
    hipStream_t st = nullptr;
    if (hipStreamCreateWithPriority(&st, hipStreamNonBlocking, prio_lo) != hipSuccess) { (void)hipGetLastError(); e.wg_side_on = 0; return nullptr; }
    if (hipEventCreateWithFlags(&e.wg_fork, hipEventDisableTiming) != hipSuccess || hipEventCreateWithFlags(&e.wg_join, hipEventDisableTiming) != hipSuccess) {
        (void)hipGetLastError(); (void)hipStreamDestroy(st); e.wg_side_on = 0; return nullptr;
    }
    e.wg_side = st; e.wg_side_dev = dev;
    return st;
}

static void finish_biases(const Ctx& c) {
    launch_bias_finish(c.at<BiasJob>(c.e.bias_jobs_off), (int)c.e.bias_jobs.size(), c.ws, c.grads, c.s);
}

template <typename Extra>
static int stage_tail(const Ctx& c, int stage, hipStream_t side, bool wait_join, Extra extra) {
    stcd_engine& e = c.e;
    if (!side) { reduce_stage(c, stage); extra(c); return 0; }
    STCD_HIP(hipEventRecord(e.wg_fork, c.s));
    STCD_HIP(hipStreamWaitEvent(side, e.wg_fork, 0));
    Ctx cs{e, c.ws, c.params, c.grads, side};
    reduce_stage(cs, stage);
    extra(cs);
    STCD_HIP(hipEventRecord(e.wg_join, side));
    if (wait_join) STCD_HIP(hipStreamWaitEvent(c.s, e.wg_join, 0));
    return 0;
}

struct EarlyScope {
    stcd_engine& e;
    EarlyScope(stcd_engine& e_, bool on, hipStream_t sd) : e(e_) { e.wg_early = on; e.wg_cur_side = sd; }
    ~EarlyScope() { e.wg_early = false; e.wg_cur_side = nullptr; }
};

static int backward_fcsiam(stcd_engine& e, const float* grad_logits, const float* params, float* grads, void* workspace,
                           int stage, hipStream_t s) {
    Ctx c{e, (char*)workspace, params, grads, s};
    hipStream_t side = stage < 0 ? wgrad_side_stream(e, s) : nullptr;
    EarlyScope early_scope(e, mfma_on(e) && e.use_wgroup, side);
    for (int st = 0; st < 2; ++st)
        if (stage < 0 || stage == st)
            for (WgradGroup& G : e.wgroups[st]) { G.seen = 0; G.launched = false; }
    const int B = e.B, dt = e.dt;
    const int64_t T = (int64_t)dsize(dt);
    if (stage <= 0) {
        STCD_HIP(hipMemsetAsync(grads, 0, e.param_floats * 4, s));
        if (!mfma_on(e)) STCD_HIP(hipMemsetAsync(c.at(e.dwe_begin), 0, e.dwe_end - e.dwe_begin, s));
        launch_gout_pack(dt, grad_logits, c.at(e.G.off), B, e.label, e.H, e.W, s, c.at<long long>(e.final_bias_acc));
        exec_wgrad(c, e.final_wg, c.at(e.finalIn.off), c.at(e.G.off));
        {
            BwdSum bs;
            if (e.final_dgr_bwd) bs = bwd_sum_of(c, *e.final_dgr_bwd);
            exec_conv(c, e.final_dgr, c.at(e.G.off), nullptr, c.at(e.dFinalIn.off), false, nullptr, nullptr, nullptr, nullptr, nullptr,
                      e.final_dgr_bwd ? &bs : nullptr);
        }
        int di = (int)e.dec.size() - 1;
        for (int k = 3; k >= 0; --k) {
            int nb = 0;
            for (int j = 0; j < DEC[k].n; ++j) nb += DEC[k].cout[j] >= 0;
            for (int j = 0; j < nb; ++j) cbrd_backward(c, e.dec[di--]);
            const UpConv& U = e.ups[k];
            const int s_ = U.level, C = ENC_C[s_];
            upconv_backward(c, U);
            const Cbrd& skip = e.enc[SKIP_IDX[s_]];
            if (fc_cross(e)) xconc_backward(c, e.xc[s_], skip);
            else if (!fc_concat_skips(e) && !e.use_skip_fused) {
                ProfScope ps(c, PC_POOL_FUSE, 0.0, (e.arch == STCD_ARCH_DIFF ? 5.0 : 3.0) * B * e.Hs[s_] * e.Ws[s_] * C * (double)T);
                launch_fuse_bwd(dt, e.arch == STCD_ARCH_DIFF ? 0 : 1, c.at(skip.A.off), skip.A.ld, skip.A.goff,
                                c.at<char>(e.dD[s_].off) + C * T, e.dD[s_].ld, c.at(skip.dA.off), skip.dA.ld, skip.dA.goff, B,
                                (int64_t)e.Hs[s_] * e.Ws[s_], C, s);
            }
        }
        if (stage_tail(c, 0, side, false, finish_biases)) return 1;
    }
    if (stage < 0 || stage == 1) {
        for (int li = (int)e.enc.size() - 1; li >= 0; --li) {
            const Cbrd& L = e.enc[li];
            int skip_chunks = 0;
            if (L.pool && !fc_concat_skips(e) && !fc_cross(e) && e.use_skip_fused) {
                const int C = e.convs[L.conv].cout;
                int lvl = 0;
                while (lvl < 4 && SKIP_IDX[lvl] != li) ++lvl;
                const float* mk = e.drop_p > 0.f ? c.at<float>(e.masks) + e.drops[L.drop].off : nullptr;
                if (skip_recomputed(e, L)) {
                    ProfScope ps(c, PC_POOL_FUSE, 0.0, 2.75 * L.N * L.H * L.W * C * (double)T, "k_skip_bwd_pair");
                    launch_skip_bwd_pair(dt, e.arch == STCD_ARCH_DIFF ? 0 : 1, c.at(L.Y.off), L.Y.ld, c.at<char>(e.dD[lvl].off) + C * T,
                                         e.dD[lvl].ld, c.at(L.dPool.off), L.dPool.ld, c.at(L.dA.off), L.dA.ld, L.dA.goff,
                                         c.at<float>(L.stat), mk, L.npg, L.H, L.W, C, c.at<long long>(L.bacc), s);
                } else {
                ProfScope ps(c, PC_POOL_FUSE, 0.0, 4.75 * L.N * L.H * L.W * C * (double)T, "k_skip_bwd");
                launch_skip_bwd(dt, e.arch == STCD_ARCH_DIFF ? 0 : 1, c.at(L.A.off), L.A.ld, L.A.goff, c.at(L.Y.off), L.Y.ld,
                                c.at<char>(e.dD[lvl].off) + C * T, e.dD[lvl].ld, c.at(L.dPool.off), L.dPool.ld, c.at(L.dA.off), L.dA.ld,
                                L.dA.goff, c.at<float>(L.stat), e.drop_p > 0.f ? c.at<float>(e.masks) + e.drops[L.drop].off : nullptr,
                                L.npg, L.H, L.W, C, c.at<long long>(L.bacc), s);
                }
// ... 1194 lines not shown
            ProfScope ps(c, PC_POOL_FUSE, 48.0 * 32 * st.N * st.h * st.w, 4.0 * st.N * st.h * st.w * 32 * (double)T, "k_bit_tok_bwd");
            launch_bit_tok_bwd(dt, c.at(st.src.off), params + b.wa_off, c.at<float>(b.stat), c.at<float>(b.dtok_in), c.at(b.dec_din.off),
                               c.at(st.dsrc.off), c.at<float>(b.tok_part), grads + b.wa_off, st.N, st.h * st.w, s);
        }
        else if (st.kind == GS_BILINEAR) {
            ProfScope ps(c, PC_POOL_FUSE, 0.0, 17.0 * st.N * st.h * st.w * st.C * (double)T, "k_bilinear_bwd");
            launch_bilinear_bwd(dt, c.at(st.ddst.off), st.ddst.ld, c.at(st.dsrc.off), st.dsrc.ld, st.N, st.h, st.w, 4 * st.h, 4 * st.w, st.C, 0, s);
        } else if (st.kind == GS_ABSPAIR) {
            const int64_t hw = (int64_t)st.h * st.w;
            ProfScope ps(c, PC_POOL_FUSE, 0.0, 5.0 * st.N * hw * st.C * (double)T, "k_fuse_bwd");
            launch_fuse_bwd(dt, 0, c.at(st.src.off), st.src.ld, (int64_t)st.N * hw * st.src.ld, c.at(st.ddst.off), st.ddst.ld,
                            c.at(st.dsrc.off), st.dsrc.ld, (int64_t)st.N * hw * st.dsrc.ld, st.N, hw, st.C, s);
        } else if (st.kind == GS_BCONV) {
            { ProfScope ps(c, PC_POOL_FUSE, 0.0, (double)st.N * st.h * st.w * 32 * (double)T, "k_bias_grad");
            launch_bias_grad(dt, c.at(st.ddst.off), st.ddst.ld, (int64_t)st.N * st.h * st.w, 32, grads + e.convs[e.g_pred_conv].b_off, s,
                             dt == BF16 ? c.at<long long>(e.g_pred_bias_acc) : nullptr); }
            exec_wgrad(c, e.g_pred_wg, c.at(st.src.off), c.at(st.ddst.off));
            exec_conv(c, e.g_pred_dgr, c.at(st.ddst.off), nullptr, c.at(st.dsrc.off), false);
        }
        else {
            launch_slice(dt, c.at(st.ddst.off), st.ddst.ld, c.at(e.g_pool_idc.off), e.g_pool_idc.ld, (int64_t)st.N * (st.h / 2) * (st.w / 2), st.C, 1, s);
            launch_maxpool3_bwd(dt, c.at<unsigned char>(e.g_pool_idx), c.at(st.ddst.off), st.ddst.ld, c.at(st.dsrc.off), st.dsrc.ld, st.N, st.h, st.w, st.C, s);
        }
    }
    reduce_stage(c, 0);
    launch_bias_finish(c.at<BiasJob>(e.bias_jobs_off), (int)e.bias_jobs.size(), c.ws, c.grads, s);
    STCD_HIP(hipGetLastError());
    return 0;
}

#include "engine_cf.inl"

}

extern "C" {

const char* stcd_last_error(void) { return stcd::g_err.c_str(); }
int stcd_abi_version(void) { return STCD_ABI_VERSION; }

static void engine_env_switches(stcd_engine* e) {
    e->use_mfma = !env_flag("STCD_FORCE_REF_KERNELS", false);
    e->use_small = !env_flag("STCD_NO_SMALL_KERNEL", false);
    e->use_gemm = !env_flag("STCD_NO_GEMM_KERNEL", false);
    e->use_res = !env_flag("STCD_NO_RES_KERNEL", false);
    e->use_halo = env_flag("STCD_HALO_KERNEL", false);
    e->use_tile = !env_flag("STCD_NO_TILE_KERNEL", false);
    e->use_wgroup = !env_flag("STCD_NO_WGRAD_GROUPS", false);
    e->use_act_fuse = !env_flag("STCD_NO_ACT_FUSE", false);
    e->use_skip_fused = !env_flag("STCD_NO_SKIP_FUSED", false);
    e->use_skip_recompute = !env_flag("STCD_NO_SKIP_RECOMPUTE", false);
    e->use_bwdsum = !env_flag("STCD_NO_BWDSUM_FUSE", false);
    e->use_bwdsum_res = env_flag("STCD_BWDSUM_RES", false);
    e->use_virt = env_int("STCD_VIRT_ACT", e->use_virt) != 0;
    e->wg_side_on = env_int("STCD_WGRAD_SIDE", e->wg_side_on) != 0;
}

int stcd_cf_default_config(stcd_cf_config* cfg) {
    STCD_CHECK(cfg != nullptr, "cfg is null");
    static const int E[4] = {64, 128, 320, 512}, DP[4] = {3, 3, 4, 3}, HD[4] = {1, 2, 4, 8}, SR[4] = {8, 4, 2, 1};
    memset(cfg, 0, sizeof(*cfg));
    cfg->in_ch = 3; cfg->out_ch = 2;
    for (int i = 0; i < 4; ++i) { cfg->embed_dims[i] = E[i]; cfg->depths[i] = DP[i]; cfg->num_heads[i] = HD[i]; cfg->sr_ratios[i] = SR[i]; }
    cfg->mlp_ratio = 4; cfg->embedding_dim = 256; cfg->patch1 = 7; cfg->patch = 7;
    cfg->drop_rate = 0.1f; cfg->attn_drop = 0.1f; cfg->drop_path_rate = 0.1f; cfg->diff_drop = 0.6f;
    return 0;
}

int stcd_create_changeformer(const stcd_cf_config* cfg, int dtype, stcd_engine** out) {
    STCD_CHECK(out != nullptr && cfg != nullptr, "null argument");
    STCD_CHECK(cfg->in_ch >= 1 && cfg->in_ch <= 8, "in_ch must be in [1,8]");
    STCD_CHECK(cfg->out_ch >= 1 && cfg->out_ch <= 8, "out_ch must be in [1,8]");
    STCD_CHECK(dtype == STCD_DTYPE_F32 || dtype == STCD_DTYPE_BF16, "unknown dtype");
    STCD_CHECK(cfg->mlp_ratio >= 1 && cfg->embedding_dim >= 8 && cfg->embedding_dim % 8 == 0, "embedding_dim must be a positive multiple of 8");
    STCD_CHECK((cfg->embedding_dim & (cfg->embedding_dim - 1)) == 0, "embedding_dim must be a power of two (BatchNorm kernels)");
    STCD_CHECK((cfg->patch1 & 1) && (cfg->patch & 1) && cfg->patch1 >= 3 && cfg->patch >= 3, "patch sizes must be odd and >= 3");
    for (int i = 0; i < 4; ++i) {
        STCD_CHECK(cfg->embed_dims[i] >= 8 && cfg->embed_dims[i] % 8 == 0 && cfg->embed_dims[i] <= 1024, "embed_dims must be multiples of 8, <= 1024");
        STCD_CHECK(cfg->depths[i] >= 1 && cfg->num_heads[i] >= 1 && cfg->sr_ratios[i] >= 1, "depths, num_heads and sr_ratios must be >= 1");
        STCD_CHECK(cfg->embed_dims[i] % cfg->num_heads[i] == 0, "embed_dims must be divisible by num_heads");
    }
    for (float p : {cfg->drop_rate, cfg->attn_drop, cfg->drop_path_rate, cfg->diff_drop}) STCD_CHECK(p >= 0.f && p < 1.f, "drop rates must be in [0,1)");
    std::unique_ptr<stcd_engine> e(new stcd_engine());
    e->arch = STCD_ARCH_CHANGEFORMER; e->in_ch = cfg->in_ch; e->label = cfg->out_ch; e->dt = dtype;
    engine_env_switches(e.get());
    e->cf = std::make_shared<CfPlan>();
    CfPlan& P = *e->cf;
    for (int i = 0; i < 4; ++i) { P.E[i] = cfg->embed_dims[i]; P.depths[i] = cfg->depths[i]; P.heads[i] = cfg->num_heads[i]; P.srs[i] = cfg->sr_ratios[i]; }
    P.mlp_ratio = cfg->mlp_ratio; P.D = cfg->embedding_dim; P.patch1 = cfg->patch1; P.patch = cfg->patch;
    P.drop = cfg->drop_rate; P.attn_drop = cfg->attn_drop; P.drop_path = cfg->drop_path_rate; P.diff_drop = cfg->diff_drop;
    build_cf_tables(*e);
    *out = e.release();
    return 0;
}

int stcd_cf_num_sites(const stcd_engine* e) { return e && e->cf && e->configured ? (int)e->cf->sites.size() : 0; }
int stcd_cf_site_get(const stcd_engine* e, int i, stcd_cf_site* out) {
    STCD_CHECK(e && e->cf && e->configured && out && i >= 0 && i < (int)e->cf->sites.size(), "bad argument");
    memset(out, 0, sizeof(*out));
    const CfPlan::Site& s = e->cf->sites[i];
    snprintf(out->name, sizeof(out->name), "%s", s.name.c_str());
    out->ndim = s.nd;
    for (int k = 0; k < s.nd; ++k) out->dims[k] = s.dims[k];
    out->p = s.p;
    return 0;
}
uint32_t stcd_cf_site_seed(uint64_t seed, int site) { return cf_site_seed(seed, site); }
// ... 656 lines not shown
```

stcd_amd/csrc/kernels_conv_mfma.hip:

```cpp
#include "common.h"

namespace stcd {

typedef __attribute__((ext_vector_type(8))) __bf16 bf16x8;
typedef __attribute__((ext_vector_type(4))) float f32x4;
typedef __attribute__((ext_vector_type(4))) unsigned u32x4;

struct ConvMfmaArgs {
    stcd_conv_geom g;
    const bf16* in;
    const bf16* wf;
    const float* bias;
    void* out;
    int out_nchw;
    int CiB, nchunks, KS;
    int modeB;
    int NTtot;
    int dymin, dxmin, HH, HWp, swmask;
    int tiles_x, tiles_y;
    int halo_bytes, wbuf_bytes;
    int tap[9];
};

static inline void fill_taps(const stcd_conv_geom& g, int* tap) {
// ... 367 lines not shown
#undef LAUNCH_NT
    return 0;
}

bool conv_mfma_x4_ok(const stcd_conv_geom g[4], const ConvMfmaPlan p[4]) {
    for (int k = 0; k < 4; ++k)
        if (!p[k].ok || p[k].NT != p[0].NT || p[k].NTtot != p[0].NTtot || g[k].n != g[0].n || g[k].hm != g[0].hm || g[k].wm != g[0].wm)
            return false;
    return true;
}
int launch_conv_mfma_x4(const stcd_conv_geom g[4], const ConvMfmaPlan p[4], const void* in, const void* const wf[4],
                        const float* bias, void* out, hipStream_t s) {
    if (!conv_mfma_x4_ok(g, p)) return 1;
    ConvMfmaArgs4 j;
    size_t lds = 0;
    for (int k = 0; k < 4; ++k) lds = std::max(lds, conv_mfma_args(g[k], p[k], in, wf[k], bias, out, false, j.a[k]));
    if (lds > 160 * 1024) return 1;
    dim3 grid((unsigned)(j.a[0].tiles_x * j.a[0].tiles_y * g[0].n), (unsigned)(p[0].NTtot / p[0].NT), 4);
#define LAUNCH_X4(N_)                                                                                             \
    do {                                                                                                          \
        static bool attr_set = false;                                                                             \
        if (!attr_set) {                                                                                          \
            (void)hipFuncSetAttribute((const void*)k_conv_mfma_x4<N_>, hipFuncAttributeMaxDynamicSharedMemorySize, 160 * 1024); \
            attr_set = true;                                                                                      \
        }                                                                                                         \
        k_conv_mfma_x4<N_><<<grid, 256, lds, s>>>(j);                                                             \
    } while (0)
    switch (p[0].NT) {
        case 1: LAUNCH_X4(1); break;
        case 2: LAUNCH_X4(2); break;
        case 4: LAUNCH_X4(4); break;
        default: LAUNCH_X4(8); break;
    }
#undef LAUNCH_X4
    return 0;
}



__device__ __forceinline__ bf16x8 tr_frag(const char* base0, const char* base1) {
    typedef __attribute__((ext_vector_type(4))) __bf16 bf16x4;
    typedef __attribute__((address_space(3))) bf16x4 lds_bf16x4;
    const bf16x4 lo = __builtin_amdgcn_ds_read_tr16_b64_v4bf16((lds_bf16x4*)base0);
    const bf16x4 hi = __builtin_amdgcn_ds_read_tr16_b64_v4bf16((lds_bf16x4*)base1);
    bf16x8 f;
    f[0] = lo[0]; f[1] = lo[1]; f[2] = lo[2]; f[3] = lo[3];
    f[4] = hi[0]; f[5] = hi[1]; f[6] = hi[2]; f[7] = hi[3];
    return f;
}

template <int C>
__device__ __forceinline__ int px_off(int x) { return x * (2 * C) + (x >> 3) * (C == 16 ? 128 : 32); }

template <int WCI, int NTW, bool T9, bool XF = false>
__device__ __forceinline__ void wgrad_body(const WgradJob& a, const char* base, const int bx, const int by, const int bz) {
    extern __shared__ __attribute__((aligned(16))) char smem[];
    const bf16* a_in = reinterpret_cast<const bf16*>(base + a.in_off);
    const bf16* a_dout = reinterpret_cast<const bf16*>(base + a.dout_off);
    float* a_slab = reinterpret_cast<float*>(const_cast<char*>(base) + a.slab_off);
    constexpr int WK = 4 / WCI, CIB = WCI * 16, COB = NTW * 16;
    constexpr int XCH = CIB / 8, YCH = COB / 8;
    constexpr int SCX = CIB > 32 ? 32 : CIB, NSX = CIB / SCX;
    const int xsub = a.x_bytes / NSX;
    constexpr int SCY = COB > 32 ? 32 : COB, NSY = COB / SCY;
    const int ysub = a.y_bytes / NSY;
    constexpr int YROW = 16 * 2 * SCY + 2 * (SCY == 16 ? 128 : 32);
    const int tid = threadIdx.x, lane = tid & 63, wid = tid >> 6;
    const int wci = wid % WCI, wk = wid / WCI;
    const int grp = lane >> 4, li = lane & 15, qrow = li >> 2, pcol = li & 3;
    const int HWp = a.HWp;
    const int ci0 = by * CIB, co0 = bz * COB;
    const int buf_bytes = a.x_bytes + a.y_bytes;
    const int ntaps = T9 ? 9 : a.g.ntaps;

    f32x4 acc[9][NTW];
#pragma unroll
    for (int t = 0; t < 9; ++t)
#pragma unroll
        for (int n_ = 0; n_ < NTW; ++n_) acc[t][n_] = f32x4{0.f, 0.f, 0.f, 0.f};

    const int nx = a.HH * HWp * XCH;
    constexpr int MAXX = WCI == 4 ? 6 : 3;
    int xg[MAXX], xl[MAXX], xa[MAXX], xb[MAXX];
#pragma unroll
    for (int p = 0; p < MAXX; ++p) {
        const int i = min(tid + p * 256, nx - 1);
        const int ch = i % XCH, pix = i / XCH, hx = pix % HWp, hy = pix / HWp;
        xa[p] = hy + a.dymin; xb[p] = hx + a.dxmin;
        xg[p] = ((hy * a.g.wi + hx) * a.g.ldi + ci0 + ch * 8) * 2;
        xl[p] = (ch / (SCX / 8)) * xsub + hy * a.xrow_bytes + px_off<SCX>(hx) + (ch % (SCX / 8)) * 16;
        if (ci0 + ch * 8 >= a.g.ci) xa[p] = 1 << 28;
    }
    int yg[NTW], yl[NTW], ya[NTW], yb[NTW];
#pragma unroll
    for (int q = 0; q < NTW; ++q) {
        const int j = tid + q * 256, ch = j % YCH, pix = j / YCH, py = pix >> 4, pxx = pix & 15;
        ya[q] = py; yb[q] = pxx;
        yg[q] = (((py * a.g.out_stride) * a.g.wo + pxx * a.g.out_stride) * a.g.ldo + co0 + ch * 8) * 2;
        yl[q] = a.x_bytes + (ch / (SCY / 8)) * ysub + py * YROW + px_off<SCY>(pxx) + (ch % (SCY / 8)) * 16;
        if (co0 + ch * 8 >= a.co_valid) ya[q] = 1 << 28;
    }
    const int npx = (nx + 255) >> 8;

    const int tiles_img = a.tiles_x * a.tiles_y;
    const int step = a.gx;
    const int dn = step / tiles_img, drem = step - dn * tiles_img, dty = drem / a.tiles_x, dtx = drem - dty * a.tiles_x;
    int tile = bx;
    int tn = tile / tiles_img, trem = tile - tn * tiles_img, tty = trem / a.tiles_x, ttx = trem - tty * a.tiles_x;

    const int64_t lead = ((int64_t)(-a.dymin) * a.g.wi + (-a.dxmin)) * a.g.ldi * 2;
    const __amdgpu_buffer_rsrc_t xrs = __builtin_amdgcn_make_buffer_rsrc(
        const_cast<char*>(reinterpret_cast<const char*>(a_in)) - lead, (short)0, (int)(a.in_bytes + (unsigned)lead), 0x00020000);
    const __amdgpu_buffer_rsrc_t yrs = __builtin_amdgcn_make_buffer_rsrc(
        const_cast<char*>(reinterpret_cast<const char*>(a_dout)), (short)0, (int)a.dout_bytes, 0x00020000);
    uint4 prex[MAXX], prey[NTW];
    constexpr bool xf_on = XF;
    float* const xf_tab = reinterpret_cast<float*>(smem + 2 * buf_bytes);
    const int xf_ch = min(ci0 + (tid % XCH) * 8, max(a.xf_C - 8, 0));
    unsigned xf_ok = 0; int xf_g = 0;
    float4 xf_m0 = make_float4(1.f, 1.f, 1.f, 1.f), xf_m1 = xf_m0;
    if constexpr (xf_on) {
        const float* st = reinterpret_cast<const float*>(base + a.xf_stat_off);
        for (int i = tid; i < a.xf_groups * 2 * a.xf_C; i += 256) {
            const int c = i % a.xf_C, w = (i / a.xf_C) & 1, g_ = i / (2 * a.xf_C);
            xf_tab[i] = st[((int64_t)g_ * 4 + 2 + w) * a.xf_C + c];
        }
        __syncthreads();
    }
#define WG_FETCH(N_, Y_, X_)                                                                                          \
    do {                                                                                                              \
        const int my0_ = (Y_) * 8, mx0_ = (X_) * 16;                                                                   \
        if constexpr (xf_on) {                                                                                        \
            xf_ok = 0; xf_g = (N_) / a.xf_npg;                                                                        \
            if (a.xf_mask_off >= 0) {                                                                                 \
                const float4* mp_ = reinterpret_cast<const float4*>(reinterpret_cast<const float*>(base + a.xf_mask_off) + (int64_t)(N_) * a.xf_C + xf_ch); \
                xf_m0 = mp_[0]; xf_m1 = mp_[1];                                                                       \
            }                                                                                                         \
        }                                                                                                             \
        const unsigned xs_ = (unsigned)(((((int64_t)(N_) * a.g.hi + my0_) * a.g.wi + mx0_) * a.g.ldi) * 2);            \
        const unsigned ys_ = (unsigned)(((((int64_t)(N_) * a.g.ho + my0_ * a.g.out_stride + a.g.oy0) * a.g.wo +        \
                                          mx0_ * a.g.out_stride + a.g.ox0) * a.g.ldo) * 2);                            \
        _Pragma("unroll") for (int p = 0; p < MAXX; ++p) {                                                            \
            if (p < npx) {                                                                                            \
                const bool ok_ = (unsigned)(my0_ + xa[p]) < (unsigned)a.g.hi && (unsigned)(mx0_ + xb[p]) < (unsigned)a.wi_valid; \
                const u32x4 v_ = __builtin_amdgcn_raw_buffer_load_b128(xrs, ok_ ? (unsigned)xg[p] : 0x80000000u, xs_, 0); \
                prex[p] = make_uint4(v_[0], v_[1], v_[2], v_[3]);                                                     \
                if constexpr (xf_on) xf_ok |= ok_ ? (1u << p) : 0u;                                                   \
            }                                                                                                         \
        }                                                                                                             \
        _Pragma("unroll") for (int q = 0; q < NTW; ++q) {                                                             \
            const bool ok_ = (unsigned)(my0_ + ya[q]) < (unsigned)a.g.hm && mx0_ + yb[q] < a.g.wm;                     \
            const u32x4 v_ = __builtin_amdgcn_raw_buffer_load_b128(yrs, ok_ ? (unsigned)yg[q] : 0x80000000u, ys_, 0); \
            prey[q] = make_uint4(v_[0], v_[1], v_[2], v_[3]);                                                         \
        }                                                                                                             \
    } while (0)
#define WG_STASH(BUF_)                                                                                                \
    do {                                                                                                              \
        if constexpr (xf_on) {                                                                                        \
            float sc_[8], sh_[8];                                                                                     \
            const float* tb_ = xf_tab + (xf_g * 2) * a.xf_C + xf_ch;                                                  \
            xf_fold8(tb_, tb_ + a.xf_C, xf_m0, xf_m1, sc_, sh_);                                                      \
            _Pragma("unroll") for (int p = 0; p < MAXX; ++p)                                                          \
                if (p < npx) prex[p] = xf_act8(prex[p], sc_, sh_, 0u - ((xf_ok >> p) & 1u));                          \
        }                                                                                                             \
        _Pragma("unroll") for (int p = 0; p < MAXX; ++p)                                                              \
            if (p < npx && tid + p * 256 < nx) *reinterpret_cast<uint4*>(smem + (BUF_) * buf_bytes + xl[p]) = prex[p]; \
        _Pragma("unroll") for (int q = 0; q < NTW; ++q)                                                               \
            *reinterpret_cast<uint4*>(smem + (BUF_) * buf_bytes + yl[q]) = prey[q];                                   \
    } while (0)

    const int frow = grp >> 1;
    const int fx0 = 8 * (grp & 1) + qrow, fx1 = fx0 + 4;
    const int yb0 = frow * YROW + px_off<SCY>(fx0) + 8 * pcol, yb1 = frow * YROW + px_off<SCY>(fx1) + 8 * pcol;
    int xoff0[9], xoff1[9];
#pragma unroll
    for (int t = 0; t < 9; ++t) {
        const int tdy = t < ntaps ? a.g.dy[t] - a.dymin : 0, tdx = t < ntaps ? a.g.dx[t] - a.dxmin : 0;
        const int csub = (wci * 16 / SCX) * xsub + (wci * 16 % SCX) * 2;
        xoff0[t] = (tdy + frow) * a.xrow_bytes + px_off<SCX>(fx0 + tdx) + csub + 8 * pcol;
        xoff1[t] = (tdy + frow) * a.xrow_bytes + px_off<SCX>(fx1 + tdx) + csub + 8 * pcol;
    }

    int buf = 0;
    if (tile < a.ntiles) { WG_FETCH(tn, tty, ttx); WG_STASH(0); }
    __syncthreads();
    for (; tile < a.ntiles; tile += step, buf ^= 1) {
        int nn = tn, nyy = tty, nxx = ttx;
        nxx += dtx; if (nxx >= a.tiles_x) { nxx -= a.tiles_x; ++nyy; }
        nyy += dty; if (nyy >= a.tiles_y) { nyy -= a.tiles_y; ++nn; }
        nn += dn;
        const bool have_next = tile + step < a.ntiles;
        if (have_next) WG_FETCH(nn, nyy, nxx);
        const char* xs = smem + buf * buf_bytes;
        const char* ys = xs + a.x_bytes;
#pragma unroll
        for (int ks = wk; ks < 4; ks += WK) {
            bf16x8 bfr[NTW];
#pragma unroll
            for (int n_ = 0; n_ < NTW; ++n_) {
                const int yo = ((n_ * 16) / SCY) * ysub + ((n_ * 16) % SCY) * 2;
                bfr[n_] = tr_frag(ys + ks * 2 * YROW + yb0 + yo, ys + ks * 2 * YROW + yb1 + yo);
            }
            const char* xr = xs + ks * 2 * a.xrow_bytes;
            if constexpr (T9) {
                bf16x8 afr[9];
#pragma unroll
                for (int t = 0; t < 9; ++t) afr[t] = tr_frag(xr + xoff0[t], xr + xoff1[t]);
#pragma unroll
                for (int t = 0; t < 9; ++t)
#pragma unroll
                    for (int n_ = 0; n_ < NTW; ++n_)
                        acc[t][n_] = __builtin_amdgcn_mfma_f32_16x16x32_bf16(afr[t], bfr[n_], acc[t][n_], 0, 0, 0);
            } else {
#pragma unroll
                for (int t = 0; t < 9; ++t) {
                    if (t < ntaps) {
// ... 20 lines not shown
        for (int t = 0; t < 9; ++t)
#pragma unroll
            for (int n_ = 0; n_ < NTW; ++n_)
#pragma unroll
                for (int j = 0; j < 4; ++j) dst[((t * NTW + n_) * 4 + j) * 64] = acc[t][n_][j];
    }
    __syncthreads();
    if (wk == 0) {
#pragma unroll 1
        for (int w = 1; w < WK; ++w) {
            const float* src = red + ((w - 1) * WCI + wci) * PERW + lane;
#pragma unroll
            for (int t = 0; t < 9; ++t)
#pragma unroll
                for (int n_ = 0; n_ < NTW; ++n_)
#pragma unroll
                    for (int j = 0; j < 4; ++j) acc[t][n_][j] += src[((t * NTW + n_) * 4 + j) * 64];
        }
        float* slab = a_slab + (int64_t)bx * ntaps * a.kpad * a.wld;
#pragma unroll
        for (int t = 0; t < 9; ++t)
            if (t < ntaps)
#pragma unroll
                for (int n_ = 0; n_ < NTW; ++n_)
#pragma unroll
                    for (int j = 0; j < 4; ++j) {
                        const int ci = ci0 + wci * 16 + 4 * grp + j, co = co0 + n_ * 16 + li;
                        if (ci < a.kpad && co < a.wld) slab[((int64_t)t * a.kpad + ci) * a.wld + co] = acc[t][n_][j];
                    }
    }
}

template <int WCI, int NTW, bool T9>
__global__ void __launch_bounds__(256, NTW == 4 ? 1 : 2)
k_wgrad_mfma(const WgradJob a) {
    wgrad_body<WCI, NTW, T9>(a, nullptr, blockIdx.x, blockIdx.y, blockIdx.z);
}

template <int WCI, int NTW, bool T9, bool XF = false>
__global__ void __launch_bounds__(256, (WCI == 2 && NTW == 2 && !XF) ? 3 : NTW == 4 ? 1 : 2)
k_wgrad_group(const WgradJob* __restrict__ jobs, int njobs, const char* base) {
    int lo = 0, hi = njobs - 1;
    while (lo < hi) {
        const int mid = (lo + hi + 1) >> 1;
        if (jobs[mid].start <= (int)blockIdx.x) lo = mid; else hi = mid - 1;
    }
    const WgradJob& a = jobs[lo];
    const int lb = blockIdx.x - a.start;
    const int G = a.gy * a.gz, full = (a.gx >> 3) << 3;
    int bx, r;
    if (lb < full * G) { const int rem = lb % (8 * G); bx = (lb / (8 * G)) * 8 + (rem & 7); r = rem >> 3; }
    else { const int l2 = lb - full * G, tail = a.gx - full; bx = full + l2 % tail; r = l2 / tail; }
    wgrad_body<WCI, NTW, T9, XF>(a, base, bx, r % a.gy, r / a.gy);
}

template <int PARTS>
__global__ void __launch_bounds__(256)
k_reduce_dw(const float* __restrict__ slab, int gx, int64_t slab_stride, int ntaps, int K, int N, int kpad, int wld,
            PackSpec ps, int use_ps, float* __restrict__ out) {
    constexpr int OUTS = 256 / PARTS;
    __shared__ float red[256];
    const int o = blockIdx.x * OUTS + (threadIdx.x % OUTS), part = threadIdx.x / OUTS;
    const int total = ntaps * K * N;
    float acc = 0.f;
    int n = 0, k = 0, t = 0;
    if (o < total) {
        n = o % N; k = (o / N) % K; t = o / (N * K);
        const float* p = slab + ((int64_t)t * kpad + k) * wld + n;
        for (int b = part; b < gx; b += PARTS) acc += p[(int64_t)b * slab_stride];
    }
    red[threadIdx.x] = acc;
    __syncthreads();
    if (part == 0 && o < total) {
        acc = 0.f;
#pragma unroll
        for (int q = 0; q < PARTS; ++q) acc += red[q * OUTS + threadIdx.x];
        if (use_ps) {
            const int64_t a_ = ps.kn_major ? ((int64_t)k * ps.N + n) : ((int64_t)n * ps.K + k);
            out[(a_ * ps.ks + ps.ky[t]) * ps.ks + ps.kx[t]] = acc;
        } else {
            out[((int64_t)t * kpad + k) * wld + n] = acc;
        }
    }
}

__global__ void __launch_bounds__(256)
k_reduce_jobs(const ReduceJob* __restrict__ jobs, int njobs, int64_t total, const char* __restrict__ ws, float* __restrict__ grads) {
    __shared__ float tile[9 * 16 * 33];
    const int64_t i0 = (int64_t)blockIdx.x * blockDim.x;
    int lo = 0, hi = njobs - 1;
    while (lo < hi) {
        const int mid = (lo + hi + 1) >> 1;
        if (jobs[mid].start <= i0) lo = mid; else hi = mid - 1;
    }
    const ReduceJob& jb = jobs[lo];
    if (!jb.tiled) {
        const int parts = jb.parts, OUTS = 256 / parts;
        const int lb = (int)((i0 - jb.start) >> 8);
        const int ol = threadIdx.x % OUTS, part = threadIdx.x / OUTS;
        const int outs = jb.ntaps * jb.K * jb.N;
        const int o = lb * OUTS + ol;
        const int chunk = (jb.gx + parts - 1) / parts;
        const int b0 = part * chunk, b1 = min(jb.gx, b0 + chunk);
        int n = 0, k = 0, t = 0;
        float acc = 0.f;
        if (o < outs) {
// ... 77 lines not shown
    p.NTW = co64 ? 4 : g.co >= 32 ? 2 : 1;
    p.WCI = (co64 || (wide_ok && g.ci >= 64 && p.NTW == 2 && HH * HWp * 8 <= 6 * 256)) ? 4 : g.ci >= 32 ? 2 : 1;
    p.gy = (g.ci + p.WCI * 16 - 1) / (p.WCI * 16);
    p.gz = (g.co + p.NTW * 16 - 1) / (p.NTW * 16);
    const int64_t slab_bytes = (int64_t)g.ntaps * kpad * wld * 4;
    constexpr int target_blocks = 1536;
    int64_t gx = std::max<int64_t>(1, target_blocks / (p.gy * p.gz));
    gx = std::min<int64_t>(gx, std::max<int64_t>(1, ((int64_t)24 << 20) / slab_bytes));
    gx = std::min<int64_t>(gx, ntiles);
    p.gx = (int)gx;
    p.slab_floats = (int64_t)p.gx * g.ntaps * kpad * wld;
    const int xpieces = HH * HWp * (p.WCI * 2);
    p.ok = g.ci % 8 == 0 && g.ldi % 8 == 0 && g.ldo % 8 == 0 && g.in_stride == 1 && xpieces <= (p.WCI == 4 ? 6 : 3) * 256 && g.hm <= g.hi && g.wm <= g.wi &&
           ((int64_t)g.n * g.hi + 4) * g.wi * g.ldi * 2 < ((int64_t)1 << 31) && (int64_t)g.n * g.ho * g.wo * g.ldo * 2 < ((int64_t)1 << 31);
    return p;
}

WgradJob wgrad_make_job(const stcd_conv_geom& g, const WgradMfmaPlan& p, int64_t in_off, int64_t dout_off, int64_t slab_off,
                        int kpad, int wld) {
    WgradJob a;
    memset(&a, 0, sizeof(a));
    a.g = g;
    a.in_off = in_off; a.dout_off = dout_off; a.slab_off = slab_off; a.kpad = kpad; a.wld = wld;
    int dymax, dxmax;
    taps_extent(g, &a.dymin, &dymax, &a.dxmin, &dxmax);
    a.HH = 7 * g.in_stride + (dymax - a.dymin) + 1;
    a.HWp = 15 * g.in_stride + (dxmax - a.dxmin) + 1;
    a.tiles_x = (g.wm + 15) / 16;
    a.tiles_y = (g.hm + 7) / 8;
    a.ntiles = g.n * a.tiles_x * a.tiles_y;
    const int CIB = p.WCI * 16, COB = p.NTW * 16;
    const int SCX = CIB > 32 ? 32 : CIB, NSX = CIB / SCX;
    const int SCY = COB > 32 ? 32 : COB, NSY = COB / SCY;
    const int xpad = SCX == 16 ? 128 : 32, ypad = SCY == 16 ? 128 : 32;
    a.xrow_bytes = (a.HWp * 2 * SCX + ((a.HWp + 7) / 8) * xpad + 15) & ~15;
    a.x_bytes = NSX * ((a.HH * a.xrow_bytes + 255) & ~255);
    a.y_bytes = NSY * ((8 * (16 * 2 * SCY + 2 * ypad) + 255) & ~255);
    a.co_valid = (g.co + 7) & ~7;
    a.in_bytes = (unsigned)((int64_t)g.n * g.hi * g.wi * g.ldi * 2);
    a.dout_bytes = (unsigned)((int64_t)g.n * g.ho * g.wo * g.ldo * 2);
    a.gx = p.gx; a.gy = p.gy; a.gz = p.gz; a.start = 0;
    a.wi_valid = p.wi_valid > 0 ? p.wi_valid : g.wi; a.pad_ = 0;
    const int WK = 4 / p.WCI;
    a.lds_bytes = (int)std::max<size_t>(2 * (size_t)(a.x_bytes + a.y_bytes), (size_t)(WK - 1) * p.WCI * 9 * p.NTW * 4 * 64 * 4);
    a.xf_stat_off = -1; a.xf_mask_off = -1; a.xf_C = 0; a.xf_groups = 1; a.xf_npg = 1; a.pad2_ = 0;
    return a;
}

void wgrad_job_set_xf(WgradJob& a, int64_t stat_off, int64_t mask_off, int C, int groups, int npg) {
    a.xf_stat_off = stat_off; a.xf_mask_off = mask_off; a.xf_C = C; a.xf_groups = groups; a.xf_npg = npg;
    a.lds_bytes = std::max(a.lds_bytes, 2 * (a.x_bytes + a.y_bytes) + groups * 2 * C * 4);
}

#define WG_DISPATCH(W_, N_, T_, WHAT)                                       \
    do {                                                                    \
        if ((W_) == 4 && (N_) == 4) { if (T_) { WHAT(4, 4, true); } else { WHAT(4, 4, false); } }   \
        else if ((W_) == 4) { if (T_) { WHAT(4, 2, true); } else { WHAT(4, 2, false); } }           \
        else if ((W_) == 1 && (N_) == 1) { if (T_) { WHAT(1, 1, true); } else { WHAT(1, 1, false); } }   \
        else if ((W_) == 1) { if (T_) { WHAT(1, 2, true); } else { WHAT(1, 2, false); } }           \
        else if ((N_) == 1) { if (T_) { WHAT(2, 1, true); } else { WHAT(2, 1, false); } }           \
        else { if (T_) { WHAT(2, 2, true); } else { WHAT(2, 2, false); } }                          \
    } while (0)

int wgrad_variant_slots(int WCI, int NTW, bool t9, int lds_bytes) {
    int dev = 0, cus = 256, per_cu = 2;
    if (hipGetDevice(&dev) != hipSuccess) { (void)hipGetLastError(); return 512; }
    hipDeviceProp_t prop;
    if (hipGetDeviceProperties(&prop, dev) == hipSuccess) cus = prop.multiProcessorCount;
#define WG_OCC(W_, N_, T_) \
    if (hipOccupancyMaxActiveBlocksPerMultiprocessor(&per_cu, k_wgrad_group<W_, N_, T_>, 256, (size_t)lds_bytes) != hipSuccess) per_cu = 2
    WG_DISPATCH(WCI, NTW, t9, WG_OCC);
#undef WG_OCC
    (void)hipGetLastError();
    return std::max(1, per_cu) * cus;
}

int launch_wgrad_group(int WCI, int NTW, bool t9, const WgradJob* jobs_dev, int njobs, int total_blocks, int lds_bytes,
                       const char* base, hipStream_t s, bool xf) {
    if (njobs <= 0 || total_blocks <= 0) return 0;
    if (lds_bytes > 128 * 1024) return 1;
    if (lds_bytes > 64 * 1024) {
        static bool attr_set = false;
        if (!attr_set) {
            (void)hipFuncSetAttribute((const void*)k_wgrad_group<4, 2, true>, hipFuncAttributeMaxDynamicSharedMemorySize, 160 * 1024);
            (void)hipFuncSetAttribute((const void*)k_wgrad_group<4, 2, false>, hipFuncAttributeMaxDynamicSharedMemorySize, 160 * 1024);
            (void)hipFuncSetAttribute((const void*)k_wgrad_group<4, 4, true>, hipFuncAttributeMaxDynamicSharedMemorySize, 160 * 1024);
            (void)hipFuncSetAttribute((const void*)k_wgrad_group<4, 4, false>, hipFuncAttributeMaxDynamicSharedMemorySize, 160 * 1024);
            attr_set = true;
        }
    }
    if (xf) {
#define WG_GROUP_XF(W_, N_, T_) k_wgrad_group<W_, N_, T_, true><<<(unsigned)total_blocks, 256, (size_t)lds_bytes, s>>>(jobs_dev, njobs, base)
        if (WCI == 4 || NTW == 4) return 1;
        WG_DISPATCH(WCI, NTW, t9, WG_GROUP_XF);
#undef WG_GROUP_XF
        return 0;
    }
#define WG_GROUP(W_, N_, T_) k_wgrad_group<W_, N_, T_><<<(unsigned)total_blocks, 256, (size_t)lds_bytes, s>>>(jobs_dev, njobs, base)
    WG_DISPATCH(WCI, NTW, t9, WG_GROUP);
#undef WG_GROUP
    return 0;
}

int launch_wgrad_mfma(const stcd_conv_geom& g, const WgradMfmaPlan& p, const void* in, const void* dout, float* slab,
                      int kpad, int wld, hipStream_t s) {
    if (!p.ok) return 1;
    const WgradJob a = wgrad_make_job(g, p, (int64_t)(intptr_t)in, (int64_t)(intptr_t)dout, (int64_t)(intptr_t)slab, kpad, wld);
// ... 1398 lines not shown
```

stcd_amd/csrc/kernels_ew.hip:

```cpp
#include <cstdlib>

#include "common.h"

namespace stcd {

__device__ __forceinline__ void ld8f(const float* p, float (&v)[8]) {
    float4 a = *reinterpret_cast<const float4*>(p), b = *reinterpret_cast<const float4*>(p + 4);
    v[0] = a.x; v[1] = a.y; v[2] = a.z; v[3] = a.w; v[4] = b.x; v[5] = b.y; v[6] = b.z; v[7] = b.w;
}


template <typename T> struct Raw8;
template <> struct Raw8<bf16> {
    uint4 v;
    __device__ __forceinline__ void opaque() { asm volatile("" : "+v"(v.x), "+v"(v.y), "+v"(v.z), "+v"(v.w)); }
    __device__ __forceinline__ void ld(const bf16* p) { v = *reinterpret_cast<const uint4*>(p); }
    __device__ __forceinline__ void get(float (&o)[8]) const {
        const uint32_t w[4] = {v.x, v.y, v.z, v.w};
#pragma unroll
        for (int i = 0; i < 4; ++i) { o[2 * i] = __uint_as_float(w[i] << 16); o[2 * i + 1] = __uint_as_float(w[i] & 0xffff0000u); }
    }
};
template <> struct Raw8<float> {
    float4 a, b;
// ... 251 lines not shown
                for (int k = 0; k < NS; ++k) {
                    const bool on = k < xs.n && ((xs.gmask[k] >> g) & 1);
#pragma unroll
                    for (int j = 0; j < 8; ++j) d[u][j] += on ? ex[u][k][j] : 0.f;
                }
#pragma unroll
                for (int j = 0; j < 8; ++j) d[u][j] = round_as<T>(d[u][j]);
                if (ok[u]) {
                    const int64_t pu = p + (int64_t)u * lanes;
                    store8<T>(dA_sum + g * dav.goff + pu * dav.ld + cofs, d[u]);
                }
            }
        }
#pragma unroll
        for (int u = 0; u < U; ++u) {
            if (!ok[u]) continue;
            if (MODE == 0) {
#pragma unroll
                for (int j = 0; j < 8; ++j) { s1[j] += y[u][j]; s2[j] += y[u][j] * y[u][j]; }
            } else {
#pragma unroll
                for (int j = 0; j < 8; ++j) {
                    float z = y[u][j] * scale[j] + shift[j];
                    if constexpr (RES) z += rs[u][j];
                    float dz = d[u][j] * (MASK ? mk[u][j] : 1.f);
                    if (relu && !(z > 0.f)) dz = 0.f;
                    s1[j] += dz;
                    s2[j] += dz * (y[u][j] - mean[j]) * invstd[j];
                }
            }
        }
    }
    const int nred = block_reduce16(s1, s2, cb, red);
    __syncthreads();
    for (int o = threadIdx.x; o < 2 * CS; o += 256) {
        int which = o / CS, c = o - which * CS;
        const float a_ = block_reduce16_get(red, nred, cb, which, c);
        bn_acc_add(acc, chunk, gridDim.y, C, g, which, cbase + c, a_, MODE == 0 ? (which ? BN_FS2 : BN_FS1) : BN_BS);
    }
}

void launch_bn_stats(int dt, const void* Y, int ld, int C, int groups, int64_t ppg, long long* acc, hipStream_t s) {
    const int nslab = bn_slabs(C);
    int nchunk = bn_stats_chunks(ppg, C / nslab);
    dim3 grid(nchunk * nslab, groups);
    GV z{0, 0};
    if (dt == BF16)
        k_bn_reduce<bf16, 0><<<grid, 256, 0, s>>>((const bf16*)Y, ld, nullptr, z, nullptr, nullptr, nullptr, 0, C, 0, 1, 0, ppg, nchunk, acc, SliceViews(), 1, nullptr, nslab);
    else
        k_bn_reduce<float, 0><<<grid, 256, 0, s>>>((const float*)Y, ld, nullptr, z, nullptr, nullptr, nullptr, 0, C, 0, 1, 0, ppg, nchunk, acc, SliceViews(), 1, nullptr, nslab);
}


__device__ __forceinline__ void bn_bwd_table(float* tab, const long long* __restrict__ bacc, const float* __restrict__ stat,
                                             float* __restrict__ dgamma, float* __restrict__ dbeta, int C, int groups, int64_t ppg,
                                             bool publish, int cbase = 0, int CS = 0, float* __restrict__ dbeta_copy = nullptr) {
    if (CS == 0) CS = C;
    const double inv_n = 1.0 / (double)ppg;
    for (int cl = threadIdx.x; cl < CS; cl += blockDim.x) {
        const int c = cbase + cl;
        double tg = 0.0, tb = 0.0;
        for (int g = 0; g < groups; ++g) {
            const double s1 = bn_acc_get(bacc, groups, C, g, 0, c, BN_BS), s2 = bn_acc_get(bacc, groups, C, g, 1, c, BN_BS);
            const float* st = stat + (int64_t)g * 4 * C;
            const double mean = st[c], invstd = st[C + c], scale = st[2 * C + c];
            const double k1 = s1 * inv_n, k2 = s2 * inv_n;
            float* bw = tab + (int64_t)g * 5 * CS;
            bw[cl] = (float)scale;
            bw[CS + cl] = st[3 * C + c];
            bw[2 * CS + cl] = (float)(-scale * k2 * invstd);
            bw[3 * CS + cl] = (float)mean;
            bw[4 * CS + cl] = (float)(-scale * k1);
            tb += s1; tg += s2;
        }
        if (publish && dgamma) { dgamma[c] = (float)tg; dbeta[c] = (float)tb; if (dbeta_copy) dbeta_copy[c] = (float)tb; }
    }
}

__global__ void k_bn_eval_prepare(int C, int groups, const float* __restrict__ gamma, const float* __restrict__ beta,
                                  const float* __restrict__ rmean, const float* __restrict__ rvar, float* __restrict__ stat,
                                  float eps) {
    int c = blockIdx.x * blockDim.x + threadIdx.x;
    if (c >= C) return;
    float invstd = 1.f / sqrtf(rvar[c] + eps);
    for (int g = 0; g < groups; ++g) {
        float* st = stat + (int64_t)g * 4 * C;
        st[c] = rmean[c];
        st[C + c] = invstd;
        st[2 * C + c] = gamma[c] * invstd;
        st[3 * C + c] = beta[c] - rmean[c] * gamma[c] * invstd;
    }
}
void launch_bn_eval_prepare(int C, int groups, const float* gamma, const float* beta, const float* rmean,
                            const float* rvar, float* stat, float eps, hipStream_t s) {
    k_bn_eval_prepare<<<cdiv(C, 64), 64, 0, s>>>(C, groups, gamma, beta, rmean, rvar, stat, eps);
}

template <typename T, bool RES, bool MASK>
__global__ void __launch_bounds__(256)
k_bn_act(const T* __restrict__ Y, int ldy, T* __restrict__ A, GV av, T* __restrict__ P, int ldp,
         float* __restrict__ stat, const float* __restrict__ mask, const T* __restrict__ res, int ldres, int C, int npg,
         int H, int W, int relu, int64_t total, const long long* __restrict__ facc, const float* __restrict__ gamma,
         const float* __restrict__ beta, float* __restrict__ rmean, float* __restrict__ rvar, int groups, float momentum, float eps,
         const SliceViews xd, int nslab, int g_first) {
    extern __shared__ float bn_tab[];
    const int CS = C / nslab, slab = blockIdx.x % nslab, bi = blockIdx.x / nslab, bps = gridDim.x / nslab, cbase = slab * CS;
    bn_fwd_table(bn_tab, facc, gamma, beta, rmean, rvar, stat, C, groups, (int64_t)npg * H * W, momentum, eps, bi == 0, cbase, CS, g_first);
    __syncthreads();
    const int64_t total_s = total / nslab;
    for (int64_t i64 = (int64_t)bi * blockDim.x + threadIdx.x; i64 < total_s; i64 += (int64_t)bps * blockDim.x) {
    const int cb = CS >> 3, Hc = (H + 1) >> 1, Wc = (W + 1) >> 1, Hp = H >> 1, Wp = W >> 1;
    uint32_t r = (uint32_t)i64;
    const int c0l = (int)(r % (uint32_t)cb) * 8, c0 = cbase + c0l; r /= (uint32_t)cb;
    const int xc = (int)(r % (uint32_t)Wc); r /= (uint32_t)Wc;
    const int yc = (int)(r % (uint32_t)Hc);
    const int n = (int)(r / (uint32_t)Hc);
    const int g = n / npg, nig = n - g * npg;
    float sc[8], sh[8], mk[8];
    {
#pragma unroll
        for (int j = 0; j < 8; ++j) { sc[j] = bn_tab[(g * 2 + 0) * CS + c0l + j]; sh[j] = bn_tab[(g * 2 + 1) * CS + c0l + j]; }
        if constexpr (MASK) {
            const float4* mp = reinterpret_cast<const float4*>(mask + (int64_t)n * C + c0);
            const float4 m0 = mp[0], m1 = mp[1];
            mk[0] = m0.x; mk[1] = m0.y; mk[2] = m0.z; mk[3] = m0.w; mk[4] = m1.x; mk[5] = m1.y; mk[6] = m1.z; mk[7] = m1.w;
#pragma unroll
            for (int j = 0; j < 8; ++j) { sc[j] *= mk[j]; sh[j] *= mk[j]; }
        }
    }
    float v[4][8], rs[4][8];
// ... 486 lines not shown
    int n = (int)(r / h0);
    bool ey = (y == h0 - 1) && H > h0, ex = (x == w0 - 1) && W > w0;
    if (!ey && !ex) return;
    float acc[8], v[8];
    load8<T>(dD + (((int64_t)n * H + y) * W + x) * ld + c0, acc);
    for (int yy = y; yy < (ey ? H : y + 1); ++yy)
        for (int xx = x; xx < (ex ? W : x + 1); ++xx) {
            if (yy == y && xx == x) continue;
            load8<T>(dD + (((int64_t)n * H + yy) * W + xx) * ld + c0, v);
#pragma unroll
            for (int j = 0; j < 8; ++j) acc[j] += v[j];
        }
    store8<T>(dD + (((int64_t)n * H + y) * W + x) * ld + c0, acc);
}

template <typename T, int PX, int OPT, bool MASK>
__global__ void __launch_bounds__(256)
k_bn_bwd_apply(const T* __restrict__ dA, GV dav, T* __restrict__ dY, int lddy, const T* __restrict__ Y, int ldy,
               const float* __restrict__ stat, const long long* __restrict__ bacc, float* __restrict__ dgamma, float* __restrict__ dbeta,
               int groups, const float* __restrict__ mask, const T* __restrict__ res, int ldres,
               T* __restrict__ dZout, int lddz, const T* __restrict__ extra, int ldex, int C, int npg, int64_t HW, int relu,
               int64_t total, int nslab, float* __restrict__ dbeta_copy) {
    extern __shared__ float bw_tab[];
    const int CS = C / nslab, slab = blockIdx.x % nslab, bi = blockIdx.x / nslab, bps = gridDim.x / nslab, cbase = slab * CS;
    bn_bwd_table(bw_tab, bacc, stat, dgamma, dbeta, C, groups, (int64_t)npg * HW, bi == 0, cbase, CS, dbeta_copy);
    __syncthreads();
    const int64_t total_s = total / nslab;
    for (int64_t i = (int64_t)bi * blockDim.x + threadIdx.x; i < total_s; i += (int64_t)bps * blockDim.x) {
    const int cb = CS >> 3;
    const uint32_t iu = (uint32_t)i;
    const int c0l = (int)(iu % (uint32_t)cb) * 8, c0 = cbase + c0l;
    const int64_t p0 = (int64_t)(iu / (uint32_t)cb) * PX;
    const int n = (int)((uint32_t)p0 / (uint32_t)HW);
    const int g = n / npg;
    const int64_t pig0 = p0 - (int64_t)g * npg * HW;
    float sc[8], sh[8], kb[8], mu[8], kc[8], mk[8];
    const float* w = bw_tab + (int64_t)g * 5 * CS + c0l;
#pragma unroll
    for (int j = 0; j < 8; ++j) { sc[j] = w[j]; sh[j] = w[CS + j]; kb[j] = w[2 * CS + j]; mu[j] = w[3 * CS + j]; kc[j] = w[4 * CS + j]; }
    if constexpr (MASK) ld8f(mask + (int64_t)n * C + c0, mk);
    float y[PX][8], d[PX][8], rs[PX][8], ex[PX][8];
#pragma unroll
    for (int k = 0; k < PX; ++k) {
        load8<T>(Y + (p0 + k) * ldy + c0, y[k]);
        load8<T>(dA + g * dav.goff + (pig0 + k) * dav.ld + c0, d[k]);
        if constexpr (OPT == 1) load8<T>(res + (p0 + k) * ldres + c0, rs[k]);
        if constexpr (OPT == 2) load8<T>(extra + (p0 + k) * ldex + c0, ex[k]);
    }
#pragma unroll
    for (int k = 0; k < PX; ++k) {
        float o[8], dzv[8];
#pragma unroll
        for (int j = 0; j < 8; ++j) {
            float dz = MASK ? d[k][j] * mk[j] : d[k][j];
            float z = y[k][j] * sc[j] + sh[j];
            if constexpr (OPT == 1) z += rs[k][j];
            if (relu && !(z > 0.f)) dz = 0.f;
            dzv[j] = dz;
            o[j] = sc[j] * dz + kb[j] * (y[k][j] - mu[j]) + kc[j];
            if constexpr (OPT == 2) o[j] += ex[k][j];
        }
        if (dZout) store8<T>(dZout + (p0 + k) * lddz + c0, dzv);
        store8<T>(dY + (p0 + k) * lddy + c0, o);
    }
    }
}
template <typename T>
__global__ void __launch_bounds__(256)
k_bias_grad(const T* __restrict__ dY, int ld, int64_t pixels, int C, float* __restrict__ db, long long* __restrict__ acc_i) {
    __shared__ float red[256 * 8];
    const int cb = C >> 3, lanes = 256 / cb;
    const int mycb = threadIdx.x % cb, lane = threadIdx.x / cb;
    float s[8];
#pragma unroll
    for (int j = 0; j < 8; ++j) s[j] = 0.f;
    const int64_t stride = (int64_t)gridDim.x * lanes;
    int64_t p = (int64_t)blockIdx.x * lanes + lane;
    for (; p + 3 * stride < pixels; p += 4 * stride) {
        float v[4][8];
#pragma unroll
        for (int u = 0; u < 4; ++u) load8<T>(dY + (p + u * stride) * ld + mycb * 8, v[u]);
#pragma unroll
        for (int u = 0; u < 4; ++u)
#pragma unroll
            for (int j = 0; j < 8; ++j) s[j] += v[u][j];
    }
    for (; p < pixels; p += stride) {
        float v[8];
        load8<T>(dY + p * ld + mycb * 8, v);
#pragma unroll
        for (int j = 0; j < 8; ++j) s[j] += v[j];
    }
#pragma unroll
    for (int j = 0; j < 8; ++j) red[threadIdx.x * 8 + j] = s[j];
    __syncthreads();
    for (int c = threadIdx.x; c < C; c += 256) {
        float acc = 0.f;
        for (int l = 0; l < lanes; ++l) acc += red[(l * cb + (c >> 3)) * 8 + (c & 7)];
        if (acc_i) bn_acc_add(acc_i, blockIdx.x, 1, C, 0, 0, c, acc, BN_BS);
        else atomicAdd(db + c, acc);
    }
}
__global__ void __launch_bounds__(256)
k_bias_grad_det(const float* __restrict__ dY, int ld, int64_t pixels, int C, float* __restrict__ db) {
    __shared__ double red[256];
    const int c = blockIdx.x;
    double acc = 0.0;
    for (int64_t p = threadIdx.x; p < pixels; p += 256) acc += (double)dY[p * ld + c];
    red[threadIdx.x] = acc;
    __syncthreads();
    for (int o = 128; o > 0; o >>= 1) {
        if ((int)threadIdx.x < o) red[threadIdx.x] += red[threadIdx.x + o];
// ... 775 lines not shown
```

stcd_amd/csrc/ops_abi.hip:

```cpp
#include <algorithm>

#include "common.h"

using namespace stcd;

namespace {

int check_map(const stcd_map_geom* g) {
    STCD_CHECK(g != nullptr, "geometry is null");
    STCD_CHECK(g->n >= 1 && g->h >= 1 && g->w >= 1, "bad sizes");
    STCD_CHECK(g->c >= 8 && g->c % 8 == 0 && g->c <= 2048 && (g->c & (g->c - 1)) == 0, "channels must be a power of two in [8, 2048]");
    STCD_CHECK(g->groups >= 1 && g->groups <= 2 && g->n % g->groups == 0, "groups must be 1 or 2 and divide n");
    STCD_CHECK((int64_t)g->n * g->h * g->w * (g->c / 8) < ((int64_t)1 << 31), "tensor too large for 32-bit indexing");
    return 0;
}

int64_t acc_bytes(const stcd_map_geom& g) { return bn_acc_bytes(g.groups, g.c); }

}

extern "C" {

int64_t stcd_op_ew_scratch_bytes(const stcd_map_geom* g) {
    if (!g || g->c < 8 || g->groups < 1) return 0;
// ... 18 lines not shown
        launch_bn_stats(dtype, y, ldy, g->c, g->groups, ppg, acc, s);
        aa.facc = acc; aa.gamma = gamma; aa.beta = beta; aa.running_mean = running_mean; aa.running_var = running_var;
    } else {
        launch_bn_eval_prepare(g->c, g->groups, gamma, beta, running_mean, running_var, stat, 1e-5f, s);
    }
    aa.Y = y; aa.ldy = ldy; aa.A = a; aa.lda = lda; aa.a_group_off = ppg * lda;
    aa.P = pool; aa.ldp = ldp; aa.stat = stat; aa.mask = mask;
    aa.C = g->c; aa.groups = g->groups; aa.npg = npg; aa.H = g->h; aa.W = g->w; aa.relu = relu ? 1 : 0;
    launch_bn_act(dtype, aa, s);
    STCD_HIP(hipGetLastError());
    return 0;
}

int stcd_op_bn_act_pair(int dtype, const stcd_map_geom* g, const void* y, int ldy, const float* gamma, const float* beta,
                        float* running_mean, float* running_var, const float* mask, int fuse_mode, void* a, int lda, void* pool,
                        int ldp, void* fused, int ldf, float* stat, void* scratch, int64_t scratch_bytes, void* hip_stream) {
    if (check_map(g)) return 1;
    STCD_CHECK(dtype == STCD_DTYPE_F32 || dtype == STCD_DTYPE_BF16, "unknown dtype");
    STCD_CHECK(g->groups == 2, "the pair kernel handles the two dates of a pair: groups must be 2");
    STCD_CHECK(y && gamma && beta && running_mean && running_var && fused && stat && scratch, "null pointer argument");
    STCD_CHECK(fuse_mode == 0 || fuse_mode == 1, "fuse_mode must be 0 (|a1-a2|) or 1 (a2-a1)");
    STCD_CHECK(scratch_bytes >= stcd_op_ew_scratch_bytes(g), "scratch too small");
    hipStream_t s = (hipStream_t)hip_stream;
    const int npg = g->n / 2;
    const int64_t ppg = (int64_t)npg * g->h * g->w;
    long long* acc = (long long*)scratch;
    STCD_HIP(hipMemsetAsync(acc, 0, (size_t)acc_bytes(*g), s));
    launch_bn_stats(dtype, y, ldy, g->c, 2, ppg, acc, s);
    BnActArgs aa;
    aa.facc = acc; aa.gamma = gamma; aa.beta = beta; aa.running_mean = running_mean; aa.running_var = running_var;
    aa.Y = y; aa.ldy = ldy; aa.A = a; aa.lda = lda; aa.a_group_off = ppg * lda;
    aa.P = pool; aa.ldp = ldp; aa.stat = stat; aa.mask = mask;
    aa.C = g->c; aa.groups = 2; aa.npg = npg; aa.H = g->h; aa.W = g->w; aa.relu = 1;
    launch_bn_act_pair(dtype, aa, fused, ldf, fuse_mode, s);
    STCD_HIP(hipGetLastError());
    return 0;
}

int stcd_op_bn_act_bwd(int dtype, const stcd_map_geom* g, const void* da, int ldda, const void* y, int ldy, const float* stat,
                       const float* mask, int relu, void* dy, int lddy, float* dgamma, float* dbeta, void* scratch,
                       int64_t scratch_bytes, void* hip_stream) {
    if (check_map(g)) return 1;
    STCD_CHECK(dtype == STCD_DTYPE_F32 || dtype == STCD_DTYPE_BF16, "unknown dtype");
    STCD_CHECK(da && y && stat && dy && dgamma && dbeta && scratch, "null pointer argument");
    STCD_CHECK(scratch_bytes >= stcd_op_ew_scratch_bytes(g), "scratch too small");
    hipStream_t s = (hipStream_t)hip_stream;
    const int npg = g->n / g->groups;
    const int64_t HW = (int64_t)g->h * g->w, ppg = npg * HW;
    long long* acc = (long long*)scratch;
    STCD_HIP(hipMemsetAsync(acc, 0, (size_t)acc_bytes(*g), s));
    launch_bn_bwd_reduce(dtype, da, ldda, ppg * ldda, y, ldy, stat, mask, g->c, g->groups, npg, HW, relu ? 1 : 0, acc, s);
    launch_bn_bwd_apply(dtype, da, ldda, ppg * ldda, dy, lddy, y, ldy, stat, acc, dgamma, dbeta, mask, g->c, g->groups, npg, HW,
                        relu ? 1 : 0, s);
    STCD_HIP(hipGetLastError());
    return 0;
}

int stcd_op_maxpool(int dtype, const stcd_map_geom* g, const void* a, int lda, void* pool, int ldp, void* hip_stream) {
    if (check_map(g)) return 1;
    STCD_CHECK(a && pool, "null pointer argument");
    launch_maxpool(dtype, a, lda, pool, ldp, g->n, g->h, g->w, g->c, (hipStream_t)hip_stream);
    STCD_HIP(hipGetLastError());
    return 0;
}

int stcd_op_maxpool_bwd(int dtype, const stcd_map_geom* g, const void* a, int lda, const void* dpool, int ldp, void* da, int ldda,
                        int accumulate, void* hip_stream) {
    if (check_map(g)) return 1;
    STCD_CHECK(a && dpool && da, "null pointer argument");
    const int npg = g->n / g->groups;
    const int64_t ppg = (int64_t)npg * g->h * g->w;
    launch_pool_bwd(dtype, a, lda, ppg * lda, dpool, ldp, da, ldda, ppg * ldda, g->groups, npg, g->h, g->w, g->c, accumulate ? 1 : 0,
                    (hipStream_t)hip_stream);
    STCD_HIP(hipGetLastError());
    return 0;
}

int stcd_op_maxpool3(int dtype, const stcd_map_geom* g, const void* a, int lda, void* pool, int ldp, void* idx, void* hip_stream) {
    if (check_map(g)) return 1;
    STCD_CHECK(a && pool && g->h % 2 == 0 && g->w % 2 == 0, "null pointer argument or odd size");
    launch_maxpool3(dtype, a, lda, pool, ldp, g->n, g->h, g->w, g->c, (hipStream_t)hip_stream, (unsigned char*)idx);
    STCD_HIP(hipGetLastError());
    return 0;
}
int stcd_op_maxpool3_bwd(int dtype, const stcd_map_geom* g, const void* idx, const void* dpool, int ldp, void* da, int ldda, void* hip_stream) {
    if (check_map(g)) return 1;
    STCD_CHECK(idx && dpool && da && g->h % 2 == 0 && g->w % 2 == 0, "null pointer argument or odd size");
    launch_maxpool3_bwd(dtype, (const unsigned char*)idx, dpool, ldp, da, ldda, g->n, g->h, g->w, g->c, (hipStream_t)hip_stream);
    STCD_HIP(hipGetLastError());
    return 0;
}

int stcd_op_fuse(int dtype, int mode, const stcd_map_geom* g, const void* a, int lda, void* d, int ldd, void* hip_stream) {
    if (check_map(g)) return 1;
    STCD_CHECK(g->groups == 2 && (mode == 0 || mode == 1) && a && d, "bad argument (groups must be 2, mode 0 or 1)");
    const int b = g->n / 2;
    const int64_t HW = (int64_t)g->h * g->w;
    launch_fuse(dtype, mode, a, lda, (int64_t)b * HW * lda, d, ldd, b, HW, g->c, (hipStream_t)hip_stream);
    STCD_HIP(hipGetLastError());
    return 0;
}

int64_t stcd_op_pairdw_scratch_bytes(const stcd_map_geom* g) {
    if (!g || g->n < 2 || g->c < 8) return 0;
    return pairdw_partial_floats(g->n / 2, g->h, g->w, g->c) * 4 + 256;
}
// ... 142 lines not shown
```

Measured before the change: 7947 image-pairs/sec.

## Fuse first encoder BN backward apply into its 3x3 weight-gradient kernel

For the first encoder conv layer (small Co), the BN backward apply step that writes dY is folded into the wgrad MFMA kernel. The kernel recomputes dY on the fly from dA, Y, BN stats and the reduced sums, so the dY tensor is never written to or read back from HBM. This requires a new kernel variant, separate job grouping, and a reordered dW reduce tail so these ops run after the BN reduction. It adds per-element recomputation inside wgrad and more LDS for the BN table, and it only applies to large full-map stride-1 3x3 layers.

```diff
diff --git a/include/stcd_hip.h b/include/stcd_hip.h
--- a/include/stcd_hip.h
+++ b/include/stcd_hip.h
@@ -244,6 +244,9 @@
 int stcd_op_bn_act_bwd(int dtype, const stcd_map_geom* g, const void* da, int ldda, const void* y, int ldy, const float* stat,
                        const float* mask, int relu, void* dy, int lddy, float* dgamma, float* dbeta, void* scratch,
                        int64_t scratch_bytes, void* hip_stream);
+int stcd_op_bn_bwd_wgrad(const stcd_conv_geom* g, int groups, int gx, const void* in, const void* da, int ldda, const void* y, int ldy,
+                         const float* stat, const float* mask, int relu, float* dw, float* dgamma, float* dbeta, void* scratch,
+                         int64_t scratch_bytes, void* hip_stream);
 int stcd_op_maxpool(int dtype, const stcd_map_geom* g, const void* a, int lda, void* pool, int ldp, void* hip_stream);
 int stcd_op_maxpool_bwd(int dtype, const stcd_map_geom* g, const void* a, int lda, const void* dpool, int ldp, void* da, int ldda,
                         int accumulate, void* hip_stream);
diff --git a/stcd_amd/_lib.py b/stcd_amd/_lib.py
--- a/stcd_amd/_lib.py
+++ b/stcd_amd/_lib.py
@@ -161,6 +161,7 @@
     "stcd_op_bn_act": (_i, [_i, C.POINTER(MapGeom), _vp, _i, _vp, _vp, _vp, _vp, _vp, _i, _i, _vp, _i, _vp, _i, _vp, _vp, _i64, _vp]),
     "stcd_op_bn_act_pair": (_i, [_i, C.POINTER(MapGeom), _vp, _i, _vp, _vp, _vp, _vp, _vp, _i, _vp, _i, _vp, _i, _vp, _i, _vp, _vp, _i64, _vp]),
     "stcd_op_bn_act_bwd": (_i, [_i, C.POINTER(MapGeom), _vp, _i, _vp, _i, _vp, _vp, _i, _vp, _i, _vp, _vp, _vp, _i64, _vp]),
+    "stcd_op_bn_bwd_wgrad": (_i, [C.POINTER(ConvGeom), _i, _i, _vp, _vp, _i, _vp, _i, _vp, _vp, _i, _vp, _vp, _vp, _vp, _i64, _vp]),
     "stcd_op_maxpool": (_i, [_i, C.POINTER(MapGeom), _vp, _i, _vp, _i, _vp]),
     "stcd_op_maxpool_bwd": (_i, [_i, C.POINTER(MapGeom), _vp, _i, _vp, _i, _vp, _i, _i, _vp]),
     "stcd_op_maxpool3": (_i, [_i, C.POINTER(MapGeom), _vp, _i, _vp, _i, _vp, _vp]),
diff --git a/stcd_amd/csrc/common.h b/stcd_amd/csrc/common.h
--- a/stcd_amd/csrc/common.h
+++ b/stcd_amd/csrc/common.h
@@ -156,6 +156,56 @@
     }
 }
 
+__device__ __forceinline__ void bn_bwd_table(float* tab, const long long* __restrict__ bacc, const float* __restrict__ stat,
+                                             float* __restrict__ dgamma, float* __restrict__ dbeta, int C, int groups, int64_t ppg,
+                                             bool publish, int cbase = 0, int CS = 0, float* __restrict__ dbeta_copy = nullptr) {
+    if (CS == 0) CS = C;
+    const double inv_n = 1.0 / (double)ppg;
+    for (int cl = threadIdx.x; cl < CS; cl += blockDim.x) {
+        const int c = cbase + cl;
+        double tg = 0.0, tb = 0.0;
+        for (int g = 0; g < groups; ++g) {
+            const double s1 = bn_acc_get(bacc, groups, C, g, 0, c, BN_BS), s2 = bn_acc_get(bacc, groups, C, g, 1, c, BN_BS);
+            const float* st = stat + (int64_t)g * 4 * C;
+            const double mean = st[c], invstd = st[C + c], scale = st[2 * C + c];
+            const double k1 = s1 * inv_n, k2 = s2 * inv_n;
+            float* bw = tab + (int64_t)g * 5 * CS;
+            bw[cl] = (float)scale;
+            bw[CS + cl] = st[3 * C + c];
+            bw[2 * CS + cl] = (float)(-scale * k2 * invstd);
+            bw[3 * CS + cl] = (float)mean;
+            bw[4 * CS + cl] = (float)(-scale * k1);
+            tb += s1; tg += s2;
+        }
+        if (publish && dgamma) { dgamma[c] = (float)tg; dbeta[c] = (float)tb; if (dbeta_copy) dbeta_copy[c] = (float)tb; }
+    }
+}
+template <bool MASK, bool RES>
+__device__ __forceinline__ float bn_bwd_dy1(float d, float mk, float y, float rs, float sc, float sh, float kb, float mu, float kc,
+                                            int relu, float& dz_out) {
+    float dz = MASK ? d * mk : d;
+    float z = y * sc + sh;
+    if constexpr (RES) z += rs;
+    if (relu && !(z > 0.f)) dz = 0.f;
+    dz_out = dz;
+    return sc * dz + kb * (y - mu) + kc;
+}
+__device__ __forceinline__ uint4 bn_bwd_dy8(const uint4 da, const uint4 yr, const float (&sc)[8], const float (&sh)[8], const float (&kb)[8],
+                                            const float (&mu)[8], const float (&kc)[8], const float (&mk)[8], int relu, const unsigned okm) {
+    const uint32_t dw[4] = {da.x, da.y, da.z, da.w}, yw[4] = {yr.x, yr.y, yr.z, yr.w};
+    uint32_t o[4];
+#pragma unroll
+    for (int i = 0; i < 4; ++i) {
+        float dz;
+        const float lo = bn_bwd_dy1<true, false>(__uint_as_float(dw[i] << 16), mk[2 * i], __uint_as_float(yw[i] << 16), 0.f, sc[2 * i], sh[2 * i],
+                                                 kb[2 * i], mu[2 * i], kc[2 * i], relu, dz);
+        const float hi = bn_bwd_dy1<true, false>(__uint_as_float(dw[i] & 0xffff0000u), mk[2 * i + 1], __uint_as_float(yw[i] & 0xffff0000u), 0.f,
+                                                 sc[2 * i + 1], sh[2 * i + 1], kb[2 * i + 1], mu[2 * i + 1], kc[2 * i + 1], relu, dz);
+        o[i] = pack_bf16x2(lo, hi) & okm;
+    }
+    return make_uint4(o[0], o[1], o[2], o[3]);
+}
+
 struct XfSrc {
     const long long* facc = nullptr;
     const float* gamma = nullptr;
@@ -311,6 +361,10 @@
     int pad_;
     int64_t xf_stat_off, xf_mask_off;
     int xf_C, xf_groups, xf_npg, pad2_;
+    int64_t dy_y_off, dy_stat_off, dy_mask_off, dy_bacc_off;
+    int64_t dy_dgamma_off, dy_dbeta_off;
+    unsigned dy_y_bytes;
+    int dy_C, dy_ldy, dy_groups, dy_npg, dy_relu;
 };
 WgradMfmaPlan wgrad_gemm_plan(const stcd_conv_geom& g, int kpad, int wld);
 WgradJob wgrad_gemm_make_job(const stcd_conv_geom& g, const WgradMfmaPlan& p, int64_t in_off, int64_t dout_off, int64_t slab_off,
@@ -327,6 +381,10 @@
 int wgrad_variant_slots(int WCI, int NTW, bool t9, int lds_bytes);
 int launch_wgrad_group(int WCI, int NTW, bool t9, const WgradJob* jobs_dev, int njobs, int total_blocks, int lds_bytes,
                        const char* base, hipStream_t s, bool xf = false);
+bool wgrad_dy_ok(const stcd_conv_geom& g, const WgradMfmaPlan& p);
+void wgrad_job_set_dy(WgradJob& a, int64_t y_off, int ldy, int64_t stat_off, int64_t mask_off, int64_t bacc_off, int64_t dgamma_off,
+                      int64_t dbeta_off, int C, int groups, int npg, int relu);
+int launch_wgrad_group_dy(const WgradJob* jobs_dev, int njobs, int total_blocks, int lds_bytes, const char* base, float* grads, hipStream_t s);
 struct PackSpec;
 struct ReduceJob {
     int64_t start, count;
diff --git a/stcd_amd/csrc/engine.hip b/stcd_amd/csrc/engine.hip
--- a/stcd_amd/csrc/engine.hip
+++ b/stcd_amd/csrc/engine.hip
@@ -60,18 +60,22 @@
     bool grouped = false;
     int group = -1;
     int64_t xf_stat_off = -1, xf_mask_off = -1; int xf_C = 0, xf_groups = 1, xf_npg = 1;
+    int64_t dy_y_off = -1, dy_stat_off = -1, dy_mask_off = -1, dy_bacc_off = -1, dy_dgamma_off = 0, dy_dbeta_off = 0;
+    int dy_C = 0, dy_ldy = 0, dy_groups = 1, dy_npg = 1;
     bool own_taps = false;
     int8_t oky[9] = {0}, okx[9] = {0};
 };
 struct WgradGroup {
     int WCI = 1, NTW = 1; bool t9 = false;
     bool xf = false;
+    bool dy = false;
     int gemm = 0;
     int dma = 0;
     std::vector<WgradJob> jobs;
     int total_blocks = 0, lds_bytes = 0;
     int64_t table_off = -1;
     double flops = 0.0, bytes = 0.0;
+    bool reduced = false;
     int seen = 0; bool launched = false;
 };
 
@@ -89,6 +93,7 @@
     int64_t dgr_sum_acc = -1; int dgr_sum_c0 = 0, dgr_sum_C = 0;
     TRef fuse_dst;
     bool virt = false; const Cbrd* xsrc = nullptr;
+    bool wg_dy = false;
 };
 struct XConc {
     int level = 0, C = 0;
@@ -237,6 +242,10 @@
     const Cbrd* final_xsrc = nullptr;
     int use_virt = 0;
     int fc_virt_layers = 0;
+    int use_wgrad_dy = -1;
+    int rjobs_tail[2] = {0, 0}; int64_t rjobs_head_total[2] = {0, 0}, rjobs_tail_total[2] = {0, 0}, rjobs_tail_off[2] = {-1, -1};
+    std::vector<ReduceJob> rjobs_tail_jobs[2];
+    bool wg_reduced_early[2] = {false, false};
     std::vector<ConvOp*> conv_ops;
     int64_t slab = -1, slab_floats = 0;
     std::vector<WgradOp*> wgrad_ops;
@@ -591,15 +600,20 @@
 
 static bool same_group(const WgradGroup& G, const WgradOp& op) {
     const bool t9 = !op.plan.dma && op.g.ntaps == 9;
-    return G.gemm == op.plan.gemm && G.dma == op.plan.dma && G.WCI == op.plan.WCI && G.NTW == op.plan.NTW && G.t9 == t9 && G.xf == (op.xf_C > 0);
+    return G.gemm == op.plan.gemm && G.dma == op.plan.dma && G.WCI == op.plan.WCI && G.NTW == op.plan.NTW && G.t9 == t9 && G.xf == (op.xf_C > 0) && G.dy == (op.dy_C > 0);
 }
 
 static bool cf_side_on() { static const bool on = env_flag("STCD_CF_SIDE", true); return on; }
 
 static void build_pack_jobs(stcd_engine& e, Bump& ws) {
     for (int st = 0; st < 2; ++st) { e.rjobs[st].clear(); e.rjobs_total[st] = 0; }
+    for (int st = 0; st < 2; ++st) { e.rjobs_tail[st] = 0; e.rjobs_tail_jobs[st].clear(); e.rjobs_tail_total[st] = 0; e.rjobs_tail_off[st] = -1; }
     for (int st = 0; st < 2; ++st) e.wgroups[st].clear();
     if (e.dt == BF16 && e.use_mfma) {
+        auto set_dy = [](WgradJob& j, const WgradOp& op) {
+            wgrad_job_set_dy(j, op.dy_y_off, op.dy_ldy, op.dy_stat_off, op.dy_mask_off, op.dy_bacc_off, op.dy_dgamma_off, op.dy_dbeta_off,
+                             op.dy_C, op.dy_groups, op.dy_npg, 1);
+        };
         if (e.use_wgroup) {
             for (WgradOp* op : e.wgrad_ops) {
                 if (!op->plan.ok) continue;
@@ -607,7 +621,7 @@
                 std::vector<WgradGroup>& gs = e.wgroups[op->stage];
                 size_t gi = 0;
                 while (gi < gs.size() && !same_group(gs[gi], *op)) ++gi;
-                if (gi == gs.size()) { WgradGroup g; g.WCI = op->plan.WCI; g.NTW = op->plan.NTW; g.t9 = t9; g.gemm = op->plan.gemm; g.dma = op->plan.dma; g.xf = op->xf_C > 0; gs.push_back(g); }
+                if (gi == gs.size()) { WgradGroup g; g.WCI = op->plan.WCI; g.NTW = op->plan.NTW; g.t9 = t9; g.gemm = op->plan.gemm; g.dma = op->plan.dma; g.xf = op->xf_C > 0; g.dy = op->dy_C > 0; gs.push_back(g); }
                 op->grouped = true;
             }
             for (int st = 0; st < 2; ++st)
@@ -640,21 +654,28 @@
                         }
                         continue;
                     }
+                    auto same_variant = [&](const WgradOp& op) {
+                        WgradGroup V = G;
+                        V.dy = op.dy_C > 0;
+                        return same_group(V, op);
+                    };
                     std::vector<WgradOp*> ops;
                     int64_t W = 0;
+                    int lds_plain = 0;
                     for (WgradOp* op : e.wgrad_ops)
-                        if (op->grouped && op->stage == st && same_group(G, *op)) {
-                            ops.push_back(op);
+                        if (op->grouped && op->stage == st && same_variant(*op)) {
                             const int64_t ntiles = (int64_t)op->g.n * ((op->g.wm + 15) / 16) * ((op->g.hm + 7) / 8);
                             W += ntiles * op->plan.gy * op->plan.gz;
+                            const ConvW& cv = e.convs[op->conv];
+                            WgradJob j = wgrad_make_job(op->g, op->plan, 0, 0, 0, cv.fwd.kpad, cv.fwd.wld);
+                            if (op->xf_C > 0) wgrad_job_set_xf(j, op->xf_stat_off, op->xf_mask_off, op->xf_C, op->xf_groups, op->xf_npg);
+                            lds_plain = std::max(lds_plain, j.lds_bytes);
+                            if (!same_group(G, *op)) continue;
+                            ops.push_back(op);
+                            if (op->dy_C > 0) set_dy(j, *op);
+                            G.lds_bytes = std::max(G.lds_bytes, j.lds_bytes);
                         }
-                    for (WgradOp* op : ops) {
-                        const ConvW& cv = e.convs[op->conv];
-                        WgradJob j = wgrad_make_job(op->g, op->plan, 0, 0, 0, cv.fwd.kpad, cv.fwd.wld);
-                        if (op->xf_C > 0) wgrad_job_set_xf(j, op->xf_stat_off, op->xf_mask_off, op->xf_C, op->xf_groups, op->xf_npg);
-                        G.lds_bytes = std::max(G.lds_bytes, j.lds_bytes);
-                    }
-                    int slots = wgrad_variant_slots(G.WCI, G.NTW, G.t9, G.lds_bytes);
+                    int slots = wgrad_variant_slots(G.WCI, G.NTW, G.t9, lds_plain);
                     if (st == 0 && e.wg_side_on && fc_family(e)) slots = std::max(64, slots / stcd_engine_impl::WG_SIDE_DIV);
                     const int64_t rounds = stcd_engine_impl::WGROUP_ROUNDS;
                     const int64_t tpb = std::max<int64_t>(stcd_engine_impl::WGROUP_MIN_TILES, (W + rounds * slots - 1) / (rounds * slots));
@@ -670,8 +691,10 @@
                 }
         }
         int64_t cur[2] = {0, 0};
+        for (int pass = 0; pass < 2; ++pass)
         for (WgradOp* op : e.wgrad_ops) {
             if (!op->plan.ok) continue;
+            if ((op->grouped && op->dy_C > 0) != (pass == 1)) continue;
             const ConvW& cv = e.convs[op->conv];
             op->slab = ws.take(op->plan.slab_floats * 4);
             if (op->grouped) {
@@ -682,11 +705,13 @@
                                    : op->plan.gemm ? wgrad_gemm_make_job(op->g, op->plan, op->in_off, op->dout_off, op->slab, cv.fwd.kpad, cv.fwd.wld)
                                                    : wgrad_make_job(op->g, op->plan, op->in_off, op->dout_off, op->slab, cv.fwd.kpad, cv.fwd.wld);
                         if (op->xf_C > 0 && !op->plan.dma && !op->plan.gemm) wgrad_job_set_xf(j, op->xf_stat_off, op->xf_mask_off, op->xf_C, op->xf_groups, op->xf_npg);
+                        if (op->dy_C > 0) set_dy(j, *op);
                         j.start = G.total_blocks;
                         G.total_blocks += j.gx * j.gy * j.gz;
                         G.jobs.push_back(j);
                         double fl, by;
                         conv_work(e, op->g, op->kreal, op->nreal, &fl, &by);
+                        if (op->dy_C > 0) by += (double)op->g.n * op->g.ho * op->g.wo * op->dy_C * 2.0;
                         G.flops += fl; G.bytes += by;
                     }
             }
@@ -714,12 +739,20 @@
                 j.count = ntiles * 256;
             }
             j.start = cur[op->stage];
+            if (pass == 1) {
+                ReduceJob t = j;
+                if (e.rjobs_tail[op->stage]++ == 0) e.rjobs_head_total[op->stage] = cur[op->stage];
+                t.start = j.start - e.rjobs_head_total[op->stage];
+                e.rjobs_tail_jobs[op->stage].push_back(t);
+                e.rjobs_tail_total[op->stage] = t.start + ((j.count + 255) & ~(int64_t)255);
+            }
             cur[op->stage] += (j.count + 255) & ~(int64_t)255;
             e.rjobs[op->stage].push_back(j);
         }
         for (int st = 0; st < 2; ++st) {
             e.rjobs_total[st] = cur[st];
             e.rjobs_off[st] = ws.take((int64_t)e.rjobs[st].size() * sizeof(ReduceJob) + 16);
+            if (e.rjobs_tail[st]) e.rjobs_tail_off[st] = ws.take((int64_t)e.rjobs_tail_jobs[st].size() * sizeof(ReduceJob) + 16);
             for (WgradGroup& G : e.wgroups[st]) G.table_off = ws.take((int64_t)G.jobs.size() * sizeof(WgradJob) + 16);
         }
     }
@@ -980,6 +1013,24 @@
         }
     }
 
+    for (auto& L : e.enc) { L.wg_dy = false; L.wg.dy_C = 0; }
+    if (e.use_wgrad_dy != 0 && e.dt == BF16 && e.use_mfma && e.use_wgroup && !e.use_virt && !e.enc.empty()) {
+        Cbrd& L = e.enc[0];
+        const ConvW& cv = e.convs[L.conv];
+        const BnP& bn = e.bns[L.bn];
+        const int C = cv.cout;
+        const bool contiguous = L.dA.off == L.dY.off && L.dA.ld == L.dY.ld && (L.groups == 1 || L.dA.goff == (int64_t)L.npg * L.H * L.W * L.dA.ld);
+        const bool big = e.use_wgrad_dy > 0 || (int64_t)L.N * L.H * L.W >= 131072;
+        if (big && !L.has_dIn && contiguous && wgrad_dy_ok(L.wg.g, L.wg.plan) && L.wg.g.co == C &&
+            (int64_t)L.N * L.H * L.W * L.Y.ld * 2 < ((int64_t)1 << 31)) {
+            L.wg_dy = true;
+            WgradOp& w = L.wg;
+            w.dy_C = C; w.dy_y_off = L.Y.off; w.dy_ldy = L.Y.ld; w.dy_stat_off = L.stat; w.dy_bacc_off = L.bacc;
+            w.dy_mask_off = (L.drop >= 0) ? e.masks + e.drops[L.drop].off * 4 : -1;
+            w.dy_dgamma_off = bn.g_off; w.dy_dbeta_off = bn.b_off; w.dy_groups = L.groups; w.dy_npg = L.npg;
+        }
+    }
+
     e.final_xsrc = nullptr; e.fc_virt_layers = 0;
     for (auto& L : e.enc) { L.virt = false; L.xsrc = nullptr; }
     for (auto& L : e.dec) { L.virt = false; L.xsrc = nullptr; }
@@ -1059,7 +1110,7 @@
             snprintf(sfx, sizeof(sfx), "A.g%d", g);
             rec(sfx, L.A.off + g * L.A.goff * T, L.A.ld, L.npg, cv.cout);
         }
-        rec("dY", L.dY.off, L.dY.ld, L.N, cv.cout);
+        if (!L.wg_dy) rec("dY", L.dY.off, L.dY.ld, L.N, cv.cout);
     };
     for (const Cbrd& L : e.enc) rec_layer(L);
     for (const Cbrd& L : e.dec) rec_layer(L);
@@ -1313,6 +1364,9 @@
             if (!e.rjobs[k].empty())
                 STCD_HIP(hipMemcpyAsync(c.at(e.rjobs_off[k]), e.rjobs[k].data(), e.rjobs[k].size() * sizeof(ReduceJob),
                                         hipMemcpyHostToDevice, c.s));
+            if (e.rjobs_tail[k])
+                STCD_HIP(hipMemcpyAsync(c.at(e.rjobs_tail_off[k]), e.rjobs_tail_jobs[k].data(), e.rjobs_tail_jobs[k].size() * sizeof(ReduceJob),
+                                        hipMemcpyHostToDevice, c.s));
             for (WgradGroup& G : e.wgroups[k])
                 STCD_HIP(hipMemcpyAsync(c.at(G.table_off), G.jobs.data(), G.jobs.size() * sizeof(WgradJob), hipMemcpyHostToDevice, c.s));
         }
@@ -1334,9 +1388,14 @@
         char kname[64];
         if (G.dma) snprintf(kname, sizeof(kname), "k_wgrad_dma");
         else if (G.gemm) snprintf(kname, sizeof(kname), "k_wgrad_gemm<%d>", G.gemm);
-        else snprintf(kname, sizeof(kname), "k_wgrad_group<%d, %d, %s>", G.WCI, G.NTW, G.t9 ? "true" : "false");
+        else snprintf(kname, sizeof(kname), "k_wgrad_group<%d, %d, %s%s>", G.WCI, G.NTW, G.t9 ? "true" : "false", G.dy ? ", dy" : "");
         ProfScope prof(c, PC_WGRAD, G.flops, G.bytes, kname);
         G.launched = true;
+        if (G.dy) {
+            if (launch_wgrad_group_dy(c.at<WgradJob>(G.table_off), (int)G.jobs.size(), G.total_blocks, G.lds_bytes, c.ws, c.grads, c.s) != 0)
+                set_error("grouped weight-gradient launch (dy) exceeds the LDS budget");
+            return;
+        }
         if (G.dma) {
             launch_wgrad_dma_group(c.at<WgradJob>(G.table_off), (int)G.jobs.size(), G.total_blocks, c.ws, c.s);
             return;
@@ -1356,10 +1415,29 @@
     if (op.group < 0 || op.group >= (int)e.wgroups[op.stage].size()) return;
     WgradGroup& G = e.wgroups[op.stage][op.group];
     if (++G.seen < (int)G.jobs.size() || G.launched) return;
-    if (e.wg_cur_side) {
+    const int st = op.stage;
+    if (e.wg_cur_side && G.dy && e.rjobs_tail[st] > 0) {
+        launch_wgroup(c, G);
+        ProfScope prof(c, PC_PACK, 0.0, 0.0, "k_reduce_jobs");
+        launch_reduce_jobs(c.at<ReduceJob>(e.rjobs_tail_off[st]), e.rjobs_tail[st], e.rjobs_tail_total[st], c.ws, c.grads, c.s);
+        G.reduced = true;
+    } else if (e.wg_cur_side) {
         if (hipEventRecord(e.wg_fork, c.s) != hipSuccess || hipStreamWaitEvent(e.wg_cur_side, e.wg_fork, 0) != hipSuccess) { set_error("side-stream fork failed"); return; }
         Ctx cs{e, c.ws, c.params, c.grads, e.wg_cur_side};
         launch_wgroup(cs, G);
+        if (e.rjobs_tail[st] > 0 && !e.wg_reduced_early[st]) {
+            bool all_out = true;
+            for (const WgradGroup& H : e.wgroups[st]) all_out = all_out && (H.launched || H.dy);
+            if (all_out) {
+                {
+                    ProfScope prof(cs, PC_PACK, 0.0, 0.0, "k_reduce_jobs");
+                    launch_reduce_jobs(c.at<ReduceJob>(e.rjobs_off[st]), (int)e.rjobs[st].size() - e.rjobs_tail[st], e.rjobs_head_total[st], c.ws,
+                                       c.grads, e.wg_cur_side);
+                }
+                if (hipEventRecord(e.wg_join, e.wg_cur_side) != hipSuccess) { set_error("side-stream join failed"); return; }
+                e.wg_reduced_early[st] = true;
+            }
+        }
     } else {
         launch_wgroup(c, G);
     }
@@ -1367,13 +1445,23 @@
 
 static void reduce_stage(const Ctx& c, int stage) {
     stcd_engine& e = c.e;
+    bool tail_done = e.rjobs_tail[stage] > 0;
     for (WgradGroup& G : e.wgroups[stage]) {
         if (!G.launched) launch_wgroup(c, G);
-        G.launched = false; G.seen = 0;
-    }
-    if (e.rjobs[stage].empty()) return;
+        if (G.dy && !G.reduced) tail_done = false;
+        G.launched = false; G.seen = 0; G.reduced = false;
+    }
+    const bool head_done = e.wg_reduced_early[stage];
+    e.wg_reduced_early[stage] = false;
+    if (e.rjobs[stage].empty() || (head_done && tail_done)) return;
     ProfScope prof(c, PC_PACK, 0.0, 0.0, "k_reduce_jobs");
-    launch_reduce_jobs(c.at<ReduceJob>(e.rjobs_off[stage]), (int)e.rjobs[stage].size(), e.rjobs_total[stage], c.ws, c.grads, c.s);
+    const int nhead = (int)e.rjobs[stage].size() - e.rjobs_tail[stage];
+    if (head_done)
+        launch_reduce_jobs(c.at<ReduceJob>(e.rjobs_tail_off[stage]), e.rjobs_tail[stage], e.rjobs_tail_total[stage], c.ws, c.grads, c.s);
+    else if (tail_done)
+        launch_reduce_jobs(c.at<ReduceJob>(e.rjobs_off[stage]), nhead, e.rjobs_head_total[stage], c.ws, c.grads, c.s);
+    else
+        launch_reduce_jobs(c.at<ReduceJob>(e.rjobs_off[stage]), (int)e.rjobs[stage].size(), e.rjobs_total[stage], c.ws, c.grads, c.s);
 }
 
 static XfSrc xf_source(const Ctx& c, const Cbrd& P, float* bn_running, bool training) {
@@ -1455,7 +1543,7 @@
         launch_bn_bwd_reduce(e.dt, c.at(L.dA.off), L.dA.ld, L.dA.goff, c.at(L.Y.off), L.Y.ld, stat, mask, C, L.groups, L.npg, HW, 1,
                              bacc, c.s);
     }
-    {
+    if (!L.wg_dy) {
         ProfScope ps(c, PC_BN_BWD_APPLY, 0.0, 3.0 * act_bytes);
         launch_bn_bwd_apply(e.dt, c.at(L.dA.off), L.dA.ld, L.dA.goff, c.at(L.dY.off), L.dY.ld, c.at(L.Y.off), L.Y.ld, stat, bacc,
                             c.grads + bn.g_off, c.grads + bn.b_off, mask, C, L.groups, L.npg, HW, 1, c.s);
@@ -1544,7 +1632,7 @@
     if (training && e.drop_p > 0.f) {
         if (masks) STCD_HIP(hipMemcpyAsync(c.at(e.masks), masks, e.drop_floats * 4, hipMemcpyDeviceToDevice, s));
         else launch_dropout_gen(c.at<float>(e.masks), e.drop_floats, seed, e.drop_p, s);
-    } else if (training && e.fc_virt_layers > 0) {
+    } else if (training && (e.fc_virt_layers > 0 || (!e.enc.empty() && e.enc[0].wg_dy))) {
         launch_dropout_gen(c.at<float>(e.masks), e.drop_floats, seed, 0.f, s);
     }
     if (pack_all_weights(c, training != 0)) return 1;
@@ -1607,6 +1695,14 @@
 static int stage_tail(const Ctx& c, int stage, hipStream_t side, bool wait_join, Extra extra) {
     stcd_engine& e = c.e;
     if (!side) { reduce_stage(c, stage); extra(c); return 0; }
+    bool all_early = e.wg_reduced_early[stage] && e.rjobs_tail[stage] > 0;
+    for (const WgradGroup& G : e.wgroups[stage]) all_early = all_early && G.launched && (!G.dy || G.reduced);
+    if (all_early) {
+        reduce_stage(c, stage);
+        extra(c);
+        if (wait_join) STCD_HIP(hipStreamWaitEvent(c.s, e.wg_join, 0));
+        return 0;
+    }
     STCD_HIP(hipEventRecord(e.wg_fork, c.s));
     STCD_HIP(hipStreamWaitEvent(side, e.wg_fork, 0));
     Ctx cs{e, c.ws, c.params, c.grads, side};
@@ -1629,8 +1725,10 @@
     hipStream_t side = stage < 0 ? wgrad_side_stream(e, s) : nullptr;
     EarlyScope early_scope(e, mfma_on(e) && e.use_wgroup, side);
     for (int st = 0; st < 2; ++st)
-        if (stage < 0 || stage == st)
-            for (WgradGroup& G : e.wgroups[st]) { G.seen = 0; G.launched = false; }
+        if (stage < 0 || stage == st) {
+            for (WgradGroup& G : e.wgroups[st]) { G.seen = 0; G.launched = false; G.reduced = false; }
+            e.wg_reduced_early[st] = false;
+        }
     const int B = e.B, dt = e.dt;
     const int64_t T = (int64_t)dsize(dt);
     if (stage <= 0) {
@@ -2931,6 +3029,7 @@
     e->use_bwdsum = !env_flag("STCD_NO_BWDSUM_FUSE", false);
     e->use_bwdsum_res = env_flag("STCD_BWDSUM_RES", false);
     e->use_virt = env_int("STCD_VIRT_ACT", e->use_virt) != 0;
+    e->use_wgrad_dy = env_int("STCD_WGRAD_DY", e->use_wgrad_dy);
     e->wg_side_on = env_int("STCD_WGRAD_SIDE", e->wg_side_on) != 0;
 }
 
diff --git a/stcd_amd/csrc/kernels_conv_mfma.hip b/stcd_amd/csrc/kernels_conv_mfma.hip
--- a/stcd_amd/csrc/kernels_conv_mfma.hip
+++ b/stcd_amd/csrc/kernels_conv_mfma.hip
@@ -443,8 +443,8 @@
 template <int C>
 __device__ __forceinline__ int px_off(int x) { return x * (2 * C) + (x >> 3) * (C == 16 ? 128 : 32); }
 
-template <int WCI, int NTW, bool T9, bool XF = false>
-__device__ __forceinline__ void wgrad_body(const WgradJob& a, const char* base, const int bx, const int by, const int bz) {
+template <int WCI, int NTW, bool T9, bool XF = false, bool DY = false>
+__device__ __forceinline__ void wgrad_body(const WgradJob& a, const char* base, const int bx, const int by, const int bz, float* grads = nullptr) {
     extern __shared__ __attribute__((aligned(16))) char smem[];
     const bf16* a_in = reinterpret_cast<const bf16*>(base + a.in_off);
     const bf16* a_dout = reinterpret_cast<const bf16*>(base + a.dout_off);
@@ -516,6 +516,26 @@
             const int c = i % a.xf_C, w = (i / a.xf_C) & 1, g_ = i / (2 * a.xf_C);
             xf_tab[i] = st[((int64_t)g_ * 4 + 2 + w) * a.xf_C + c];
         }
+        __syncthreads();
+    }
+    constexpr bool dy_on = DY;
+    float* const dy_tab = reinterpret_cast<float*>(smem + 2 * buf_bytes);
+    const int dy_ch = min(co0 + (tid % YCH) * 8, max(a.dy_C - 8, 0));
+    unsigned dy_ok = 0; int dy_g = 0;
+    float4 dy_m0 = make_float4(1.f, 1.f, 1.f, 1.f), dy_m1 = dy_m0;
+    uint4 prey2[NTW];
+    int yg2[NTW];
+    __amdgpu_buffer_rsrc_t y2rs = yrs;
+    if constexpr (dy_on) {
+#pragma unroll
+        for (int q = 0; q < NTW; ++q) {
+            const int j = tid + q * 256, ch = j % YCH, pix = j / YCH, py = pix >> 4, pxx = pix & 15;
+            yg2[q] = (((py * a.g.out_stride) * a.g.wo + pxx * a.g.out_stride) * a.dy_ldy + co0 + ch * 8) * 2;
+        }
+        y2rs = __builtin_amdgcn_make_buffer_rsrc(const_cast<char*>(base + a.dy_y_off), (short)0, (int)a.dy_y_bytes, 0x00020000);
+        bn_bwd_table(dy_tab, reinterpret_cast<const long long*>(base + a.dy_bacc_off), reinterpret_cast<const float*>(base + a.dy_stat_off),
+                     grads + a.dy_dgamma_off, grads + a.dy_dbeta_off, a.dy_C, a.dy_groups, (int64_t)a.dy_npg * a.g.ho * a.g.wo,
+                     bx == 0 && by == 0 && bz == 0);
         __syncthreads();
     }
 #define WG_FETCH(N_, Y_, X_)                                                                                          \
@@ -539,10 +559,25 @@
                 if constexpr (xf_on) xf_ok |= ok_ ? (1u << p) : 0u;                                                   \
             }                                                                                                         \
         }                                                                                                             \
+        unsigned ys2_ = 0;                                                                                            \
+        if constexpr (dy_on) {                                                                                        \
+            dy_ok = 0; dy_g = (N_) / a.dy_npg;                                                                        \
+            if (a.dy_mask_off >= 0) {                                                                                 \
+                const float4* mp_ = reinterpret_cast<const float4*>(reinterpret_cast<const float*>(base + a.dy_mask_off) + (int64_t)(N_) * a.dy_C + dy_ch); \
+                dy_m0 = mp_[0]; dy_m1 = mp_[1];                                                                       \
+            }                                                                                                         \
+            ys2_ = (unsigned)(((((int64_t)(N_) * a.g.ho + my0_ * a.g.out_stride + a.g.oy0) * a.g.wo +                  \
+                                mx0_ * a.g.out_stride + a.g.ox0) * a.dy_ldy) * 2);                                     \
+        }                                                                                                             \
         _Pragma("unroll") for (int q = 0; q < NTW; ++q) {                                                             \
             const bool ok_ = (unsigned)(my0_ + ya[q]) < (unsigned)a.g.hm && mx0_ + yb[q] < a.g.wm;                     \
             const u32x4 v_ = __builtin_amdgcn_raw_buffer_load_b128(yrs, ok_ ? (unsigned)yg[q] : 0x80000000u, ys_, 0); \
             prey[q] = make_uint4(v_[0], v_[1], v_[2], v_[3]);                                                         \
+            if constexpr (dy_on) {                                                                                    \
+                const u32x4 w_ = __builtin_amdgcn_raw_buffer_load_b128(y2rs, ok_ ? (unsigned)yg2[q] : 0x80000000u, ys2_, 0); \
+                prey2[q] = make_uint4(w_[0], w_[1], w_[2], w_[3]);                                                    \
+                dy_ok |= ok_ ? (1u << q) : 0u;                                                                        \
+            }                                                                                                         \
         }                                                                                                             \
     } while (0)
 #define WG_STASH(BUF_)                                                                                                \
@@ -553,6 +588,17 @@
             xf_fold8(tb_, tb_ + a.xf_C, xf_m0, xf_m1, sc_, sh_);                                                      \
             _Pragma("unroll") for (int p = 0; p < MAXX; ++p)                                                          \
                 if (p < npx) prex[p] = xf_act8(prex[p], sc_, sh_, 0u - ((xf_ok >> p) & 1u));                          \
+        }                                                                                                             \
+        if constexpr (dy_on) {                                                                                        \
+            float sc_[8], sh_[8], kb_[8], mu_[8], kc_[8];                                                             \
+            const float* tb_ = dy_tab + (dy_g * 5) * a.dy_C + dy_ch;                                                  \
+            _Pragma("unroll") for (int j_ = 0; j_ < 8; ++j_) {                                                        \
+                sc_[j_] = tb_[j_]; sh_[j_] = tb_[a.dy_C + j_]; kb_[j_] = tb_[2 * a.dy_C + j_];                         \
+                mu_[j_] = tb_[3 * a.dy_C + j_]; kc_[j_] = tb_[4 * a.dy_C + j_];                                        \
+            }                                                                                                         \
+            const float mk_[8] = {dy_m0.x, dy_m0.y, dy_m0.z, dy_m0.w, dy_m1.x, dy_m1.y, dy_m1.z, dy_m1.w};            \
+            _Pragma("unroll") for (int q = 0; q < NTW; ++q)                                                           \
+                prey[q] = bn_bwd_dy8(prey[q], prey2[q], sc_, sh_, kb_, mu_, kc_, mk_, a.dy_relu, 0u - ((dy_ok >> q) & 1u)); \
         }                                                                                                             \
         _Pragma("unroll") for (int p = 0; p < MAXX; ++p)                                                              \
             if (p < npx && tid + p * 256 < nx) *reinterpret_cast<uint4*>(smem + (BUF_) * buf_bytes + xl[p]) = prex[p]; \
@@ -679,6 +725,17 @@
     if (lb < full * G) { const int rem = lb % (8 * G); bx = (lb / (8 * G)) * 8 + (rem & 7); r = rem >> 3; }
     else { const int l2 = lb - full * G, tail = a.gx - full; bx = full + l2 % tail; r = l2 / tail; }
     wgrad_body<WCI, NTW, T9, XF>(a, base, bx, r % a.gy, r / a.gy);
+}
+
+__global__ void __launch_bounds__(256, 2)
+k_wgrad_group_dy(const WgradJob* __restrict__ jobs, int njobs, const char* base, float* grads) {
+    int lo = 0, hi = njobs - 1;
+    while (lo < hi) {
+        const int mid = (lo + hi + 1) >> 1;
+        if (jobs[mid].start <= (int)blockIdx.x) lo = mid; else hi = mid - 1;
+    }
+    const WgradJob& a = jobs[lo];
+    wgrad_body<1, 1, true, false, true>(a, base, blockIdx.x - a.start, 0, 0, grads);
 }
 
 template <int PARTS>
@@ -862,7 +919,25 @@
     a.lds_bytes = std::max(a.lds_bytes, 2 * (a.x_bytes + a.y_bytes) + groups * 2 * C * 4);
 }
 
-#define WG_DISPATCH(W_, N_, T_, WHAT)                                       \
+bool wgrad_dy_ok(const stcd_conv_geom& g, const WgradMfmaPlan& p) {
+    return p.ok && !p.gemm && !p.dma && p.WCI == 1 && p.NTW == 1 && p.gy * p.gz == 1 && g.ntaps == 9 && g.co % 8 == 0 && g.co <= 16 &&
+           g.out_stride == 1 && g.oy0 == 0 && g.ox0 == 0 && g.hm == g.ho && g.wm == g.wo;
+}
+void wgrad_job_set_dy(WgradJob& a, int64_t y_off, int ldy, int64_t stat_off, int64_t mask_off, int64_t bacc_off, int64_t dgamma_off,
+                      int64_t dbeta_off, int C, int groups, int npg, int relu) {
+    a.dy_y_off = y_off; a.dy_ldy = ldy; a.dy_stat_off = stat_off; a.dy_mask_off = mask_off; a.dy_bacc_off = bacc_off;
+    a.dy_dgamma_off = dgamma_off; a.dy_dbeta_off = dbeta_off; a.dy_C = C; a.dy_groups = groups; a.dy_npg = npg; a.dy_relu = relu;
+    a.dy_y_bytes = (unsigned)((int64_t)a.g.n * a.g.ho * a.g.wo * ldy * 2);
+    a.lds_bytes = std::max(a.lds_bytes, 2 * (a.x_bytes + a.y_bytes) + groups * 5 * C * 4);
+}
+int launch_wgrad_group_dy(const WgradJob* jobs_dev, int njobs, int total_blocks, int lds_bytes, const char* base, float* grads, hipStream_t s) {
+    if (njobs <= 0 || total_blocks <= 0) return 0;
+    if (lds_bytes > 64 * 1024) return 1;
+    k_wgrad_group_dy<<<(unsigned)total_blocks, 256, (size_t)lds_bytes, s>>>(jobs_dev, njobs, base, grads);
+    return 0;
+}
+
+#define WG_DISPATCH(W_, N_, T_, WHAT)                                      \
     do {                                                                    \
         if ((W_) == 4 && (N_) == 4) { if (T_) { WHAT(4, 4, true); } else { WHAT(4, 4, false); } }   \
         else if ((W_) == 4) { if (T_) { WHAT(4, 2, true); } else { WHAT(4, 2, false); } }           \
diff --git a/stcd_amd/csrc/kernels_ew.hip b/stcd_amd/csrc/kernels_ew.hip
--- a/stcd_amd/csrc/kernels_ew.hip
+++ b/stcd_amd/csrc/kernels_ew.hip
@@ -327,30 +327,6 @@
 }
 
 
-__device__ __forceinline__ void bn_bwd_table(float* tab, const long long* __restrict__ bacc, const float* __restrict__ stat,
-                                             float* __restrict__ dgamma, float* __restrict__ dbeta, int C, int groups, int64_t ppg,
-                                             bool publish, int cbase = 0, int CS = 0, float* __restrict__ dbeta_copy = nullptr) {
-    if (CS == 0) CS = C;
-    const double inv_n = 1.0 / (double)ppg;
-    for (int cl = threadIdx.x; cl < CS; cl += blockDim.x) {
-        const int c = cbase + cl;
-        double tg = 0.0, tb = 0.0;
-        for (int g = 0; g < groups; ++g) {
-            const double s1 = bn_acc_get(bacc, groups, C, g, 0, c, BN_BS), s2 = bn_acc_get(bacc, groups, C, g, 1, c, BN_BS);
-            const float* st = stat + (int64_t)g * 4 * C;
-            const double mean = st[c], invstd = st[C + c], scale = st[2 * C + c];
-            const double k1 = s1 * inv_n, k2 = s2 * inv_n;
-            float* bw = tab + (int64_t)g * 5 * CS;
-            bw[cl] = (float)scale;
-            bw[CS + cl] = st[3 * C + c];
-            bw[2 * CS + cl] = (float)(-scale * k2 * invstd);
-            bw[3 * CS + cl] = (float)mean;
-            bw[4 * CS + cl] = (float)(-scale * k1);
-            tb += s1; tg += s2;
-        }
-        if (publish && dgamma) { dgamma[c] = (float)tg; dbeta[c] = (float)tb; if (dbeta_copy) dbeta_copy[c] = (float)tb; }
-    }
-}
 
 __global__ void k_bn_eval_prepare(int C, int groups, const float* __restrict__ gamma, const float* __restrict__ beta,
                                   const float* __restrict__ rmean, const float* __restrict__ rvar, float* __restrict__ stat,
@@ -943,12 +919,8 @@
         float o[8], dzv[8];
 #pragma unroll
         for (int j = 0; j < 8; ++j) {
-            float dz = MASK ? d[k][j] * mk[j] : d[k][j];
-            float z = y[k][j] * sc[j] + sh[j];
-            if constexpr (OPT == 1) z += rs[k][j];
-            if (relu && !(z > 0.f)) dz = 0.f;
-            dzv[j] = dz;
-            o[j] = sc[j] * dz + kb[j] * (y[k][j] - mu[j]) + kc[j];
+            o[j] = bn_bwd_dy1<MASK, OPT == 1>(d[k][j], MASK ? mk[j] : 1.f, y[k][j], OPT == 1 ? rs[k][j] : 0.f, sc[j], sh[j], kb[j], mu[j], kc[j],
+                                              relu, dzv[j]);
             if constexpr (OPT == 2) o[j] += ex[k][j];
         }
         if (dZout) store8<T>(dZout + (p0 + k) * lddz + c0, dzv);
diff --git a/stcd_amd/csrc/ops_abi.hip b/stcd_amd/csrc/ops_abi.hip
--- a/stcd_amd/csrc/ops_abi.hip
+++ b/stcd_amd/csrc/ops_abi.hip
@@ -94,6 +94,48 @@
     launch_bn_bwd_reduce(dtype, da, ldda, ppg * ldda, y, ldy, stat, mask, g->c, g->groups, npg, HW, relu ? 1 : 0, acc, s);
     launch_bn_bwd_apply(dtype, da, ldda, ppg * ldda, dy, lddy, y, ldy, stat, acc, dgamma, dbeta, mask, g->c, g->groups, npg, HW,
                         relu ? 1 : 0, s);
+    STCD_HIP(hipGetLastError());
+    return 0;
+}
+
+int stcd_op_bn_bwd_wgrad(const stcd_conv_geom* g, int groups, int gx, const void* in, const void* da, int ldda, const void* y, int ldy,
+                         const float* stat, const float* mask, int relu, float* dw, float* dgamma, float* dbeta, void* scratch,
+                         int64_t scratch_bytes, void* hip_stream) {
+    STCD_CHECK(g != nullptr, "geometry is null");
+    STCD_CHECK(in && da && y && stat && dw && dgamma && dbeta && scratch, "null pointer argument");
+    STCD_CHECK(g->ntaps == 9 && g->ci >= 8 && g->ci % 8 == 0 && g->ldi >= g->ci && g->ldi % 8 == 0 && g->n >= 1 && g->hm >= 1 && g->wm >= 1,
+               "bad geometry");
+    STCD_CHECK(g->co == 8 || g->co == 16, "the fused form handles 8 or 16 output channels (one 16-channel tile)");
+    STCD_CHECK((groups == 1 || groups == 2) && g->n % groups == 0, "groups must be 1 or 2 and divide n");
+    STCD_CHECK(ldda >= g->co && ldda % 8 == 0 && ldy >= g->co && ldy % 8 == 0, "bad pixel stride");
+    STCD_CHECK((int64_t)g->n * g->ho * g->wo * ldy * 2 < ((int64_t)1 << 31), "tensor too large for 32-bit indexing");
+    stcd_conv_geom gg = *g;
+    gg.ldo = ldda;
+    WgradMfmaPlan p = wgrad_mfma_plan(gg, g->ci, g->co);
+    STCD_CHECK(wgrad_dy_ok(gg, p), "geometry not taken by the fused form (3x3 stride 1 over the whole map, Ci <= 16, Co <= 16)");
+    const int64_t ntiles = (int64_t)g->n * ((g->wm + 15) / 16) * ((g->hm + 7) / 8);
+    STCD_CHECK(gx >= 0 && gx <= ntiles, "gx must be 0 (the planner's K split) or at most the number of 16 x 8 tiles");
+    if (gx > 0) { p.gx = gx; p.slab_floats = (int64_t)gx * g->ntaps * g->ci * g->co; }
+    stcd_map_geom mg;
+    memset(&mg, 0, sizeof(mg));
+    mg.n = g->n; mg.h = g->ho; mg.w = g->wo; mg.c = g->co; mg.groups = groups;
+    const int64_t acc_b = (acc_bytes(mg) + 255) & ~(int64_t)255, slab_b = (p.slab_floats * 4 + 255) & ~(int64_t)255;
+    STCD_CHECK(scratch_bytes >= acc_b + slab_b + (int64_t)sizeof(WgradJob), "scratch too small for the sums, the partial slabs and the job table");
+    hipStream_t s = (hipStream_t)hip_stream;
+    const int npg = g->n / groups;
+    const int64_t HW = (int64_t)g->ho * g->wo, ppg = npg * HW;
+    long long* acc = (long long*)scratch;
+    float* slab = (float*)((char*)scratch + acc_b);
+    WgradJob* table = (WgradJob*)((char*)scratch + acc_b + slab_b);
+    STCD_HIP(hipMemsetAsync(acc, 0, (size_t)acc_bytes(mg), s));
+    launch_bn_bwd_reduce(STCD_DTYPE_BF16, da, ldda, ppg * ldda, y, ldy, stat, mask, g->co, groups, npg, HW, relu ? 1 : 0, acc, s);
+    WgradJob j = wgrad_make_job(gg, p, (int64_t)(intptr_t)in, (int64_t)(intptr_t)da, (int64_t)(intptr_t)slab, g->ci, g->co);
+    wgrad_job_set_dy(j, (int64_t)(intptr_t)y, ldy, (int64_t)(intptr_t)stat, mask ? (int64_t)(intptr_t)mask : -1, (int64_t)(intptr_t)acc, 0,
+                     (int64_t)(dbeta - dgamma), g->co, groups, npg, relu ? 1 : 0);
+    STCD_HIP(hipMemcpyAsync(table, &j, sizeof(j), hipMemcpyHostToDevice, s));
+    STCD_HIP(hipStreamSynchronize(s));
+    STCD_CHECK(launch_wgrad_group_dy(table, 1, j.gx, j.lds_bytes, nullptr, dgamma, s) == 0, "LDS budget exceeded");
+    launch_reduce_dw(slab, p.gx, gg, g->ci, g->co, g->ci, g->co, nullptr, dw, s);
     STCD_HIP(hipGetLastError());
     return 0;
 }
```

Result: no change. 7946 image-pairs/sec (-0.0%).
